# probabilists/zuko

Measured on AMD Instinct MI355X. Metric: log_prob samples/sec, NSF d=64 K=8 bins=8 batch=2^20, higher is better.
Workload: dtype f32; 1 GPU; NSF(features=64, context=0, transforms=8, bins=8, hidden=[256]*3) log_prob, batch=2^20 per GPU, x~N(0,1), seed-0 init; batch_per_gpu=1048576, global_batch=1048576, parallelism=batch-sharded x1, one RCCL all-reduce of the scalar NLL

## Files before the change

include/zuko_amd.h:

```cpp
#ifndef ZUKO_AMD_H
#define ZUKO_AMD_H

#include <stdint.h>

#ifdef __cplusplus
extern "C" {
#endif

#define ZK_DTYPE_F32 0
#define ZK_DTYPE_F64 1
#define ZK_DTYPE_BF16 2

#define ZK_ACT_NONE 0
#define ZK_ACT_RELU 1
#define ZK_ACT_ELU 2
#define ZK_ACT_TANH 3
#define ZK_ACT_SILU 4
#define ZK_ACT_GELU 5
#define ZK_ACT_SIGMOID 6
#define ZK_ACT_LEAKY 7


int zk_rqs_forward(int dtype, int64_t N, int64_t D, int K, double bound, double slope, const void* x,
                   const void* widths, int64_t w_sN, int64_t w_sD, const void* heights, int64_t h_sN, int64_t h_sD,
                   const void* derivs, int64_t d_sN, int64_t d_sD, void* y, void* ladj, int ladj_reduced,
                   int32_t* bin_out, void* stream);

int zk_rqs_inverse(int dtype, int64_t N, int64_t D, int K, double bound, double slope, const void* y,
                   const void* widths, int64_t w_sN, int64_t w_sD, const void* heights, int64_t h_sN, int64_t h_sD,
                   const void* derivs, int64_t d_sN, int64_t d_sD, void* x, int32_t* bin_out, void* stream);

int zk_rqs_from_knots(int dtype, int inverse, int64_t N, int64_t D, int K, const void* in, const void* horizontal,
                      const void* vertical, const void* slopes, int64_t k_sN, int64_t k_sD, void* out, void* ladj,
                      int32_t* bin_out, void* stream);

int zk_rqs_diag(int inverse, int64_t N, int64_t D, int K, double bound, double slope, const void* in, const void* widths,
                int64_t w_sN, int64_t w_sD, const void* heights, int64_t h_sN, int64_t h_sD, const void* derivs, int64_t d_sN,
                int64_t d_sD, void* out, void* ladj, int32_t* bin_out, float* knots_out, void* stream);

int zk_affine_forward(int dtype, int64_t N, int64_t D, double slope, const void* x, const void* shift, int64_t s_sN,
                      int64_t s_sD, const void* scale, int64_t c_sN, int64_t c_sD, void* y, void* ladj, int ladj_reduced,
                      void* stream);
int zk_affine_inverse(int dtype, int64_t N, int64_t D, double slope, const void* y, const void* shift, int64_t s_sN,
                      int64_t s_sD, const void* scale, int64_t c_sN, int64_t c_sD, void* x, void* stream);

int zk_sos_forward(int dtype, int64_t N, int64_t D, int P, int L1, double slope, const double* gl_nodes01,
                   const double* gl_weights01, const void* x, const void* a_coef, int64_t a_sN, int64_t a_sD,
                   const void* constant, int64_t c_sN, int64_t c_sD, void* y, void* ladj, int ladj_reduced, void* stream);
int zk_sos_inverse(int dtype, int64_t N, int64_t D, int P, int L1, double slope, const double* gl_nodes01,
                   const double* gl_weights01, int n_bisect, const void* y, const void* a_coef, int64_t a_sN,
                   int64_t a_sD, const void* constant, int64_t c_sN, int64_t c_sD, void* x, void* stream);

int zk_bernstein_forward(int dtype, int64_t N, int64_t D, int M, int bounded, double bound, double eps, const void* x,
                         const void* theta, int64_t t_sN, int64_t t_sD, void* y, void* ladj, int ladj_reduced, void* stream);
int zk_bernstein_inverse(int dtype, int64_t N, int64_t D, int M, int bounded, double bound, double eps, int n_bisect, const void* y,
                         const void* theta, int64_t t_sN, int64_t t_sD, void* x, void* stream);

int zk_linear(int dtype, int64_t N, int in_features, int out_features, const void* x, int64_t ldx, const void* weight,
              const uint8_t* mask, const void* bias, int act, void* y, int64_t ldy, void* stream);

int zk_linear_bf16(int64_t N, int in_features, int out_features, const void* x, int64_t ldx, const void* weight, const uint64_t* tile_live_mask,
                   const void* bias, int act, void* y, int64_t ldy, void* stream);

int zk_linear_bf16_rqs(int64_t N, int in_features, int panels, const void* h, int64_t ldh, const void* weight_panels, const uint64_t* tile_live_mask,
                       const void* bias_panels, int K, int features, double bound, double slope, const void* x, int64_t ldx, void* y, int64_t ldy,
                       float* partial, float* ladj, void* stream);
int zk_linear_bf16_rqs_lanes(int64_t N, int in_features, int panels, const void* h, int64_t ldh, const void* weight_panels,
                             const uint64_t* tile_live_mask, const void* bias_panels, int K, int features, double bound, double slope, const void* x,
                             int64_t ldx, void* y, int64_t ldy, float* partial, float* ladj, void* stream);

typedef struct zk_ar_args_v1 {
  uint32_t struct_size;
  uint32_t version;
  int32_t uni_kind;
  int32_t D;
  int32_t DIN;
  int32_t n_layers;
  int32_t n_groups;
  int32_t n_chunks;
  int32_t act;
  int32_t bias_floats;
  int32_t accumulate;
  int32_t rev;
  int32_t n_sched;
  int32_t g0;
  int32_t g1;
  int32_t reserved;
  int64_t N;
  int64_t ldx;
  int64_t ldy;
  int64_t ldo;
  int64_t ldphi;
  double bound;
  double slope;
  const void* x;
  void* y;
  void* ladj;
  const void* y_in;
  void* x_out;
  const void* wstream;
  const void* bias;
  const uint32_t* skip;
  const int32_t* featmap;
  int32_t* bin_out;
  float* knots_out;
  const int32_t* sched;
  const int32_t* olim;
  const void* launcher;
  void* h1;
  void* h2;
  void* h3;
  void* phi;
  void* gh1;
  void* gh2;
  void* gh3;
  int32_t phi_packed;
  int32_t pad_;
  const double* gl_nodes01;
  const double* gl_weights01;
  double eps;
  double wdescale0;
  double wdescale1;
  double wdescale2;
  double wdescale3;
  uint32_t* amax0;
  uint32_t* amax1;
  uint32_t* amax2;
  uint32_t* amax3;
} zk_ar_args_v1;

int zk_ar_forward(const zk_ar_args_v1* args, void* stream);
int zk_ar_forward_split(const zk_ar_args_v1* args, void* stream);
int zk_ar_forward_diag(const zk_ar_args_v1* args, void* stream);
int zk_ar_dgrad_chain(const zk_ar_args_v1* args, void* stream);
int zk_ar_dgrad_full(const zk_ar_args_v1* args, void* stream);
int zk_ar_backward_full(const zk_ar_args_v1* args, void* stream);
int zk_ar_inverse_sweep(const zk_ar_args_v1* args, void* stream);
int zk_ar_inverse_partial(const zk_ar_args_v1* args, void* stream);
typedef struct zk_coupling_args_v1 {
  uint32_t struct_size;
  uint32_t version;
  int32_t D;
  int32_t C;
  int32_t nit;
  int32_t n_groups;
  int32_t n_layers;
  int32_t n_chunks;
  int32_t act;
  int32_t bias_floats;
  int32_t accumulate;
  int32_t static_ok;
  int64_t N;
  int64_t ldx;
  int64_t ldc;
  int64_t ldy;
  double slope;
  const void* in;
  const void* ctx;
  void* out;
  void* ladj;
  const void* wstream;
  const void* bias;
  const int32_t* bias_off;
  const int32_t* amap;
  const int32_t* fmap;
  const int32_t* tiles;
  const int32_t* widths;
  double wdescale0;
  double wdescale1;
  double wdescale2;
  double wdescale3;
} zk_coupling_args_v1;
int zk_coupling_forward(const zk_coupling_args_v1* args, void* stream);
int zk_coupling_inverse(const zk_coupling_args_v1* args, void* stream);
typedef struct zk_ar_inc_args_v1 {
  uint32_t struct_size;
  uint32_t version;
  int32_t uni_kind;
  int32_t n_hidden;
  int32_t D;
  int32_t C;
  int32_t n_groups;
  int32_t n_chunks;
  int32_t act;
  int32_t bias_floats;
  int64_t N;
  int64_t ldy;
  int64_t ldc;
  int64_t ldx;
  double bound;
  double slope;
  const void* y;
  const void* ctx;
  void* x;
  void* ladj;
  const void* wstream;
  const void* bias;
  const int32_t* bias_off;
  const int32_t* featmap;
  const int32_t* prog;
  int32_t half;
  int32_t pad_;
  double wdescale1;
  double wdescale2;
  double wdescale3;
  const double* gl_nodes01;
  const double* gl_weights01;
  double eps;
  int32_t n_bisect;
  int32_t pad2_;
} zk_ar_inc_args_v1;
int zk_ar_inverse_incremental(const zk_ar_inc_args_v1* args, void* stream);
int zk_ar_inc_lds_bytes(int bias_floats, int nit);
int zk_ar_lds_bytes(int variant, int bias_floats);
int zk_ar_forward_static(const zk_ar_args_v1* args, void* stream);
int zk_ar_forward_train(const zk_ar_args_v1* args, void* stream);
int zk_gather_f32(const void* src, const uint8_t* mask, const int32_t* idx, int64_t n, void* dst, void* stream);
int zk_gather_split_bf16(const void* src, const uint8_t* mask, const int32_t* idx, int64_t n_blocks, void* dst, void* stream);
int zk_gather_split_f16(const void* src, const uint8_t* mask, const int32_t* idx, int64_t n_blocks, void* dst, double scale, void* stream);
typedef struct zk_gather_desc_v1 {
  uint32_t struct_size;
  int32_t split;
  int64_t count;
  const void* src;
  const uint8_t* mask;
  const int32_t* idx;
  void* dst;
} zk_gather_desc_v1;
int zk_gather_multi(int n, const zk_gather_desc_v1* descs, void* stream);

int zk_univariate_backward(int kind, int64_t N, int64_t D, int K, double bound, double slope, const void* x, const void* phi,
                           const void* gy, const void* gl, int gl_reduced, void* gx, void* gphi, void* stream);
int zk_sos_backward(int64_t N, int64_t D, int P, int L1, double slope, const double* gl_nodes01, const double* gl_weights01,
                    int has_const, const void* x, const void* params, const void* gy, const void* gl, int gl_reduced, void* gx,
                    void* gparams, void* stream);
int zk_bernstein_backward(int64_t N, int64_t D, int M, int bounded, double bound, double eps, const void* x, const void* theta, const void* gy,
                          const void* gl, int gl_reduced, void* gx, void* gtheta, void* stream);
int zk_inverse_seed(int64_t n, const void* gx, const void* ladj, void* gy, void* seed, void* stream);
int zk_diag_normal_backward(int64_t N, int64_t D, const void* z, const void* loc, const void* scale, const void* g, void* gz,
                            void* stream);
int zk_act_backward(int64_t n, const void* y, const void* gout, int act, void* gin, void* stream);

int zk_gemm_f32_skip(int64_t N, int in_features, int out_features, const void* x, int64_t ldx, const void* w, const uint64_t* kskip,
                     const void* bias, int act, const void* gate, int64_t ldg, int gate_act, void* y, int64_t ldy, void* stream);
int zk_wgrad_slices(int64_t N, int npairs);
int zk_wgrad_f32(int64_t N, int out_features, int in_features, const void* g, int64_t ldg, const void* h, int64_t ldh,
                 const int32_t* pairs, int npairs, float* partial, const uint8_t* mask, void* dw, int accumulate, const int32_t* rows,
                 const int32_t* cols, void* stream);
int zk_wgrad_bias_f32(int64_t N, int out_features, int in_features, const void* g, int64_t ldg, const void* h, int64_t ldh,
                      const int32_t* pairs, int npairs, float* partial, const uint8_t* mask, void* dw, int accumulate,
                      const uint8_t* cs_flag, float* cs_partial, void* db, const int32_t* rows, const int32_t* cols, void* stream);
typedef struct zk_wgrad_layer_v1 {
  uint32_t struct_size;
  int32_t out_features;
  int32_t in_features;
  int32_t npairs;
  int64_t ldg;
  int64_t ldh;
  const void* g;
  const void* h;
  const int32_t* pairs;
  void* partial;
  const uint8_t* mask;
  void* dw;
  const uint8_t* cs_flag;
  void* cs_partial;
  void* db;
  const int32_t* rows;
  const int32_t* cols;
  const uint32_t* g_amax;
  const uint32_t* h_amax;
} zk_wgrad_layer_v1;
int zk_wgrad_multi(int n_layers, const zk_wgrad_layer_v1* layers, int64_t N, void* stream);
int zk_colsum_slices(int64_t N);
int zk_colsum_f32(int64_t N, int C, const void* x, int64_t ld, float* workspace, void* out, int accumulate, void* stream);

#define ZK_AMAX_WORDS 2048
typedef struct zk_amax_desc_v1 {
  uint32_t struct_size;
  int32_t cols;
  int64_t rows;
// ... 34 lines not shown
```

zuko_amd/csrc/fused_ar.hip:

```cpp
#include "../../include/zuko_amd.h"
#include "zk_ar_common.h"
#include <type_traits>

#ifndef ZK_AR_TIMING
#define ZK_AR_TIMING 0
#endif

namespace zk {

template <int CH, int NR> struct RingT {
  static constexpr int kChunk = CH, kSlots = NR;
  float* lds;
  const float* stream;
  int n_chunks, pos, slot, load_chunk, load_slot, wave, lane, dbg;
  const int* sched;

  template <int I> __device__ __forceinline__ void dma(const float* g, float* l) {
    if constexpr (I < CH / AR_WAVES) {
#ifndef ZK_AR_NO_RING_DMA
      __builtin_amdgcn_global_load_lds((const __attribute__((address_space(1))) void*)g, (__attribute__((address_space(3))) void*)l, 16, I * AR_TF * 4, 0);
#endif
      dma<I + 1>(g, l);
    }
  }
// ... 227 lines not shown
        printf("wave %d: L1 %llu  L2 %llu  L3 %llu  (+bias/act each)  last layer + 16 epilogues %llu   total %llu cycles\n", wave, tstamp[1] - tstamp[0],
               tstamp[2] - tstamp[1], tstamp[3] - tstamp[2], tstamp[5] - tstamp[3], tstamp[5] - tstamp[0]);
    }
    if (!INVERSE) ar_ladj_store(a, lacc, n, live, q);
  }
  ring.drain();
}

__device__ __forceinline__ float gather_one(const float* __restrict__ src, const uint8_t* __restrict__ mask, int32_t k) { return (k >= 0 && (!mask || mask[k])) ? src[k] : 0.f; }

__device__ __forceinline__ void gather_split_lane(const float* __restrict__ src, const uint8_t* __restrict__ mask, const int32_t* __restrict__ idx, int64_t i, uint4* __restrict__ dst) {
  typedef __bf16 bf16x8 __attribute__((ext_vector_type(8)));
  const int4 k0 = *reinterpret_cast<const int4*>(idx + i * 8), k1 = *reinterpret_cast<const int4*>(idx + i * 8 + 4);
  const int k[8] = {k0.x, k0.y, k0.z, k0.w, k1.x, k1.y, k1.z, k1.w};
  bf16x8 h, m, l;
#pragma unroll
  for (int e = 0; e < 8; ++e) {
    const float v = gather_one(src, mask, k[e]);
    const __bf16 hh = (__bf16)v;
    const float r1 = v - (float)hh;
    const __bf16 mm = (__bf16)r1;
    h[e] = hh; m[e] = mm; l[e] = (__bf16)(r1 - (float)mm);
  }
  const int64_t b = i >> 6;
  const int lane = (int)(i & 63);
  dst[(b * 3 + 0) * 64 + lane] = __builtin_bit_cast(uint4, h);
  dst[(b * 3 + 1) * 64 + lane] = __builtin_bit_cast(uint4, m);
  dst[(b * 3 + 2) * 64 + lane] = __builtin_bit_cast(uint4, l);
}

__global__ __launch_bounds__(256) void gather_kernel(const float* __restrict__ src, const uint8_t* __restrict__ mask, const int32_t* __restrict__ idx, int64_t n, float* __restrict__ dst) {
  for (int64_t i = (int64_t)blockIdx.x * 256 + threadIdx.x; i < n; i += (int64_t)gridDim.x * 256) {
    dst[i] = gather_one(src, mask, idx[i]);
  }
}

__global__ __launch_bounds__(256) void gather_split_kernel(const float* __restrict__ src, const uint8_t* __restrict__ mask, const int32_t* __restrict__ idx, int64_t n_lanes,
                                                           uint4* __restrict__ dst) {
  for (int64_t i = (int64_t)blockIdx.x * 256 + threadIdx.x; i < n_lanes; i += (int64_t)gridDim.x * 256) gather_split_lane(src, mask, idx, i, dst);
}

__global__ __launch_bounds__(256) void gather_split_f16_kernel(const float* __restrict__ src, const uint8_t* __restrict__ mask, const int32_t* __restrict__ idx, int64_t n_lanes,
                                                               uint4* __restrict__ dst, float scale) {
  typedef _Float16 f16x8 __attribute__((ext_vector_type(8)));
  for (int64_t i = (int64_t)blockIdx.x * 256 + threadIdx.x; i < n_lanes; i += (int64_t)gridDim.x * 256) {
    const int4 k0 = *reinterpret_cast<const int4*>(idx + i * 8), k1 = *reinterpret_cast<const int4*>(idx + i * 8 + 4);
    const int k[8] = {k0.x, k0.y, k0.z, k0.w, k1.x, k1.y, k1.z, k1.w};
    f16x8 h, l;
#pragma unroll
    for (int e = 0; e < 8; ++e) {
      const float v = gather_one(src, mask, k[e]) * scale;
      const _Float16 hh = (_Float16)v;
      h[e] = hh; l[e] = (_Float16)(v - (float)hh);
    }
    const int64_t b = i >> 6;
    const int lane = (int)(i & 63);
    dst[(b * 2 + 0) * 64 + lane] = __builtin_bit_cast(uint4, h);
    dst[(b * 2 + 1) * 64 + lane] = __builtin_bit_cast(uint4, l);
  }
}

struct GatherMulti {
  int n;
  int start[9];
  struct One { const float* src; const uint8_t* mask; const int32_t* idx; int64_t count; void* dst; int split; } g[8];
};
__global__ __launch_bounds__(256) void gather_multi_kernel(GatherMulti m) {
  const int b = (int)blockIdx.x;
  GatherMulti::One g = m.g[0];
  int base = 0;
#pragma unroll
  for (int k = 1; k < 8; ++k)
    if (k < m.n && b >= m.start[k]) { g = m.g[k]; base = m.start[k]; }
  const int64_t i = (int64_t)(b - base) * 256 + threadIdx.x;
  if (!g.split) {
    if (i < g.count) reinterpret_cast<float*>(g.dst)[i] = gather_one(g.src, g.mask, g.idx[i]);
  } else if (i < g.count * 64) {
    gather_split_lane(g.src, g.mask, g.idx, i, reinterpret_cast<uint4*>(g.dst));
  }
}

}

using namespace zk;

extern "C" {

int zk_gather_f32(const void* src, const uint8_t* mask, const int32_t* idx, int64_t n, void* dst, void* stream) {
  if (n <= 0) return 0;
  int64_t nb = (n + 255) / 256;
  hipLaunchKernelGGL(gather_kernel, dim3((unsigned)(nb > 2048 ? 2048 : nb)), dim3(256), 0, (hipStream_t)stream, (const float*)src, mask, idx, n, (float*)dst);
  return ZK_LAUNCH_CHECK();
}

int zk_gather_split_bf16(const void* src, const uint8_t* mask, const int32_t* idx, int64_t n_blocks, void* dst, void* stream) {
  if (n_blocks <= 0) return 0;
  if (!src || !idx || !dst || ((uintptr_t)idx % 16) || ((uintptr_t)dst % 16)) return ZK_EINVAL;
  const int64_t n_lanes = n_blocks * 64, nb = (n_lanes + 255) / 256;
  hipLaunchKernelGGL(gather_split_kernel, dim3((unsigned)(nb > 2048 ? 2048 : nb)), dim3(256), 0, (hipStream_t)stream, (const float*)src, mask, idx, n_lanes, (uint4*)dst);
  return ZK_LAUNCH_CHECK();
}

int zk_gather_split_f16(const void* src, const uint8_t* mask, const int32_t* idx, int64_t n_blocks, void* dst, double scale, void* stream) {
  if (n_blocks <= 0) return 0;
  if (!src || !idx || !dst || ((uintptr_t)idx % 16) || ((uintptr_t)dst % 16) || !(scale > 0.0) || !(scale < 1e38)) return ZK_EINVAL;
  const int64_t n_lanes = n_blocks * 64, nb = (n_lanes + 255) / 256;
  hipLaunchKernelGGL(gather_split_f16_kernel, dim3((unsigned)(nb > 2048 ? 2048 : nb)), dim3(256), 0, (hipStream_t)stream, (const float*)src, mask, idx, n_lanes, (uint4*)dst, (float)scale);
  return ZK_LAUNCH_CHECK();
}

int zk_gather_multi(int n, const zk_gather_desc_v1* descs, void* stream) {
  if (n < 1 || n > 8 || !descs) return ZK_EINVAL;
  GatherMulti m{};
  m.n = n;
  int blocks = 0;
  for (int k = 0; k < n; ++k) {
    const zk_gather_desc_v1& d = descs[k];
    if (d.struct_size != sizeof(zk_gather_desc_v1) || d.count < 0 || (d.count > 0 && (!d.src || !d.idx || !d.dst))) return ZK_EINVAL;
    if (d.split && (((uintptr_t)d.idx % 16) || ((uintptr_t)d.dst % 16))) return ZK_EINVAL;
    m.g[k] = {(const float*)d.src, d.mask, d.idx, d.count, d.dst, d.split};
    m.start[k] = blocks;
    const int64_t threads = d.split ? d.count * 64 : d.count;
    if (threads > (int64_t)0x7fffffff) return ZK_EINVAL;
    blocks += (int)((threads + 255) / 256);
  }
  m.start[n] = blocks;
  if (blocks == 0) return 0;
  hipLaunchKernelGGL(gather_multi_kernel, dim3((unsigned)blocks), dim3(256), 0, (hipStream_t)stream, m);
  return ZK_LAUNCH_CHECK();
}

#ifndef AR_CH
#define AR_CH 24
#define AR_NR 3
#endif
typedef RingT<AR_CH, AR_NR> Ring24x3;
static int ar_lds_bytes(int bias_floats, bool xlds, int xs) { return ArLds::bytes(AR_CH * AR_NR * AR_TF, bias_floats, xlds ? AR_WAVES : 0, xs); }
int zk_ar_lds_bytes(int variant, int bias_floats) { return ar_lds_bytes(bias_floats, true, 260); }

struct ArPartial {
  const void* static_fn = nullptr;
  int rev = 0;
  float* act_out[3] = {nullptr, nullptr, nullptr};
  float* phi_out = nullptr;
  int64_t ldphi = 0;
  int phi_packed = 0;
  const double* gl_nodes01 = nullptr;
  const double* gl_weights01 = nullptr;
  double eps = 0.0;
  int32_t* bin_out = nullptr;
  float* knots_out = nullptr;
  double wdescale[4] = {0.0, 0.0, 0.0, 0.0};
  unsigned* amax[4] = {nullptr, nullptr, nullptr, nullptr};
  const int* sched = nullptr;
  int n_sched = 0;
  const int* olim = nullptr;
  int g0 = 0, g1 = -1;
};

static int ar_launch(const ArPartial& part, bool inverse, int uni_kind, int64_t N, int D, int DIN, const void* x, int64_t ldx, const void* yin, int64_t ldyin, void* y, int64_t ldy,
                     void* ladj, int accumulate, const void* wstream, const void* bias, int bias_floats, const uint32_t* skip, const int32_t* featmap,
                     int n_layers, int n_groups, int n_chunks, int act, double bound, double slope, int variant, void* stream) {
  if (N <= 0) return 0;
  if (n_groups * 8 > ArLds::FMAP_WORDS || n_groups > ArLds::SKIP_WORDS) return ZK_EINVAL;
  if (n_layers < 2 || DIN > (part.static_fn ? 512 : 256) || DIN < D || DIN % 4 || ldx % 4 || ((uintptr_t)x % 16) || n_chunks < 1) return ZK_EINVAL;
  ArArgs a{};
  a.N = N; a.D = D; a.DIN = DIN;
  a.x = (const float*)x; a.ldx = ldx;
  a.yin = (const float*)yin; a.ldyin = ldyin;
  a.y = (float*)y; a.ldy = ldy; a.ladj = (float*)ladj; a.accumulate = accumulate;
  a.stream = (const float*)wstream; a.bias = (const float*)bias; a.skip = skip; a.featmap = featmap;
  a.L = n_layers; a.NG = n_groups; a.n_chunks = n_chunks; a.act = act; a.bias_floats = bias_floats;
  a.bound = (float)bound; a.ls = (float)log(slope);
  a.lc = rqs_lean_const(bound, log(slope));
  a.n_tiles = (N + 127) / 128;
  a.g0 = 0; a.g1 = n_groups;
  for (int l = 0; l < 8; ++l) a.olim[l] = 3;
  if (part.sched) {
    if (part.n_sched < 1 || part.g0 < 0 || part.g1 > n_groups || part.g0 >= part.g1 || n_layers - 1 > 8) return ZK_EINVAL;
    a.sched = part.sched; a.n_sched = part.n_sched; a.g0 = part.g0; a.g1 = part.g1;
    for (int l = 0; l < n_layers - 1; ++l) a.olim[l] = part.olim[l];
  }
#if ZK_AR_TIMING
  a.dbg = (variant >> 8) & 0xff;
  if ((variant & 0xff) != 0) return ZK_EINVAL;
#else
  if (variant != 0) return ZK_EINVAL;
#endif
  if (part.static_fn) {
    if (inverse || part.sched || ((part.bin_out != nullptr) != (part.knots_out != nullptr))) return ZK_EINVAL;
    a.bin_out = part.bin_out; a.knots_out = part.knots_out;
    a.l1rev = part.rev;
    for (int l = 0; l < 3; ++l) a.act_out[l] = part.act_out[l];
    a.phi_out = part.phi_out; a.ldphi = part.ldphi; a.phi_packed = part.phi_packed;
    if (uni_kind == 5) {
      const bool conditioner_only = part.phi_out != nullptr && y == nullptr;
      if ((!part.gl_nodes01 || !part.gl_weights01) && !conditioner_only) return ZK_EINVAL;
      a.sos.bound = (float)bound; a.sos.slope = (float)slope; a.sos.P = 3; a.sos.L1 = 5;
      if (part.gl_nodes01 && part.gl_weights01)
        for (int i = 0; i < 5; ++i) { a.sos.node[i] = (float)part.gl_nodes01[i]; a.sos.weight[i] = (float)part.gl_weights01[i]; }
    }
    a.eps = (float)(part.eps > 0.0 ? part.eps : 1e-6);
    for (int l = 0; l < 4; ++l) a.wdescale[l] = (float)part.wdescale[l];
    for (int l = 0; l < 4; ++l) a.amax[l] = part.amax[l];
    return ((ars_launch_fn)part.static_fn)(&a, ARS_ABI, (int)sizeof(ArArgs), part.phi_out != nullptr, stream);
  }
  a.xs = ((D + 3) / 4) * 4 + 4;
  const bool vec_ok = (D % 4 == 0) && (ldy % 4 == 0) && ((uintptr_t)y % 16 == 0) && (!inverse || ((ldyin % 4 == 0) && ((uintptr_t)yin % 16 == 0)));
  a.xlds = vec_ok && ar_lds_bytes(bias_floats, true, a.xs) <= 160 * 1024;
  const int lds = ar_lds_bytes(bias_floats, a.xlds, a.xs);
  if (lds > 160 * 1024) return ZK_EINVAL;
  const void* fn = nullptr;
#define ZK_AR_PICK(UNI)                                                                                                                     \
  (inverse ? (a.xlds ? (const void*)ar_kernel<UNI, true, Ring24x3, true> : (const void*)ar_kernel<UNI, true, Ring24x3, false>)            \
           : (a.xlds ? (const void*)ar_kernel<UNI, false, Ring24x3, true> : (const void*)ar_kernel<UNI, false, Ring24x3, false>))
#define ZK_AR_PICK_X(UNI) (inverse ? (const void*)ar_kernel<UNI, true, Ring24x3, true> : (const void*)ar_kernel<UNI, false, Ring24x3, true>)
  if (uni_kind == 0) fn = ZK_AR_PICK(UniAffine);
  else if (uni_kind == 1) fn = ZK_AR_PICK(UniRqs8);
  else if (uni_kind >= 2 && uni_kind <= 4 && !a.xlds) return ZK_EINVAL;
  else if (uni_kind == 2) fn = ZK_AR_PICK_X(UniRqs4);
  else if (uni_kind == 3) fn = ZK_AR_PICK_X(UniRqs16);
  else if (uni_kind == 4) fn = ZK_AR_PICK_X(UniCircRqs8);
  else return ZK_EINVAL;
  if (part.bin_out || part.knots_out) {
    if (inverse || part.sched || !a.xlds || !part.bin_out || !part.knots_out) return ZK_EINVAL;
    a.bin_out = part.bin_out; a.knots_out = part.knots_out;
    if (uni_kind == 1) fn = (const void*)ar_kernel<UniRqs8, false, Ring24x3, true, true>;
    else if (uni_kind == 2) fn = (const void*)ar_kernel<UniRqs4, false, Ring24x3, true, true>;
    else if (uni_kind == 3) fn = (const void*)ar_kernel<UniRqs16, false, Ring24x3, true, true>;
    else return ZK_EINVAL;
  }
  return ar_launch_dyn_lds(fn, 256, 512, lds, a, stream);
}

#define AR_ARGS_OK(args) (ar_args_norm(args, &args##_norm_) ? ((args) = &args##_norm_, true) : false)

static int ar_launch_v1(const ArPartial& part, bool inverse, const zk_ar_args_v1& p, void* stream) {
  return ar_launch(part, inverse, p.uni_kind, p.N, p.D, p.DIN, p.x, p.ldx, inverse ? p.y_in : nullptr, inverse ? p.ldy : 0, inverse ? p.x_out : p.y, inverse ? p.ldo : p.ldy,
                   inverse ? nullptr : p.ladj, p.accumulate, p.wstream, p.bias, p.bias_floats, p.skip, p.featmap, p.n_layers, p.n_groups, p.n_chunks, p.act, p.bound, p.slope, 0,
                   stream);
}

int zk_ar_forward(const zk_ar_args_v1* args, void* stream) {
  zk_ar_args_v1 args_norm_;
  if (!AR_ARGS_OK(args)) return ZK_EINVAL;
  return ar_launch_v1(ArPartial{}, false, *args, stream);
}

int zk_ar_forward_diag(const zk_ar_args_v1* args, void* stream) {
  zk_ar_args_v1 args_norm_;
  if (!AR_ARGS_OK(args)) return ZK_EINVAL;
  ArPartial part;
  part.bin_out = args->bin_out; part.knots_out = args->knots_out;
  zk_ar_args_v1 p = *args;
  p.accumulate = 0;
  return ar_launch_v1(part, false, p, stream);
}

int zk_ar_forward_static(const zk_ar_args_v1* args, void* stream) {
  zk_ar_args_v1 args_norm_;
  if (!AR_ARGS_OK(args) || !args->launcher) return ZK_EINVAL;
  ArPartial part;
  part.static_fn = args->launcher; part.rev = args->rev;
  part.gl_nodes01 = args->gl_nodes01; part.gl_weights01 = args->gl_weights01; part.eps = args->eps;
  part.bin_out = args->bin_out; part.knots_out = args->knots_out;
  part.wdescale[0] = args->wdescale0; part.wdescale[1] = args->wdescale1; part.wdescale[2] = args->wdescale2; part.wdescale[3] = args->wdescale3;
  zk_ar_args_v1 p = *args;
  p.skip = nullptr;
  return ar_launch_v1(part, false, p, stream);
}

int zk_ar_forward_train(const zk_ar_args_v1* args, void* stream) {
  zk_ar_args_v1 args_norm_;
  if (!AR_ARGS_OK(args) || !args->launcher || !args->phi || !args->h1) return ZK_EINVAL;
  const int n_layers = args->n_layers;
  if (n_layers < 2 || n_layers > 4 || (n_layers > 2 && !args->h2) || (n_layers > 3 && !args->h3)) return ZK_EINVAL;
  if (((uintptr_t)args->h1 % 16) || ((uintptr_t)args->h2 % 16) || ((uintptr_t)args->h3 % 16)) return ZK_EINVAL;
  ArPartial part;
  part.static_fn = args->launcher; part.rev = args->rev;
  part.act_out[0] = (float*)args->h1; part.act_out[1] = (float*)args->h2; part.act_out[2] = (float*)args->h3; part.phi_out = (float*)args->phi; part.ldphi = args->ldphi;
  part.phi_packed = args->phi_packed;
  part.amax[0] = args->amax0; part.amax[1] = args->amax1; part.amax[2] = args->amax2; part.amax[3] = args->amax3;
  zk_ar_args_v1 p = *args;
  p.act = 1; p.skip = nullptr;
  if (!p.y) {
    p.ldy = 0; p.ladj = nullptr; p.accumulate = 0; p.bound = 1.0; p.slope = 1e-3;
  }
  return ar_launch_v1(part, false, p, stream);
}

typedef int (*ars_dgrad_fn)(const ArArgs* a, int abi, int args_bytes, void* stream);
static bool ar_chain_args_ok(const zk_ar_args_v1* args) {
  return args->launcher && args->x && args->y && args->wstream && args->n_layers >= 2 && args->n_layers <= 4 && args->N >= 0 && args->N <= 0x7fffffff;
}
static ArArgs ar_chain_args(const zk_ar_args_v1* args, int chain_layers, int gated) {
  const void* hs[3] = {args->h1, args->h2, args->h3};
  void* gs[3] = {args->gh1, args->gh2, args->gh3};
  ArArgs a{};
  a.x = (const float*)args->x; a.ldx = args->ldx; a.N = args->N; a.D = args->D; a.DIN = args->DIN; a.L = chain_layers; a.n_chunks = args->n_chunks;
  a.stream = (const float*)args->wstream;
  a.phi_out = (float*)args->y; a.ldphi = args->ldy;
  for (int c = 0; c < gated; ++c) {
    a.gate[c] = (const float*)hs[gated - 1 - c];
    a.act_out[c] = (float*)gs[gated - 1 - c];
  }
  return a;
}
static int ar_chain_launch(const zk_ar_args_v1* args, const ArArgs& a, void* stream) { return ((ars_dgrad_fn)args->launcher)(&a, ARS_ABI, (int)sizeof(ArArgs), stream); }

int zk_ar_dgrad_chain(const zk_ar_args_v1* args, void* stream) {
  zk_ar_args_v1 args_norm_;
  if (!AR_ARGS_OK(args) || !ar_chain_args_ok(args)) return ZK_EINVAL;
  if (args->N == 0) return 0;
  return ar_chain_launch(args, ar_chain_args(args, args->n_layers - 1, args->n_layers - 2), stream);
}

int zk_ar_dgrad_full(const zk_ar_args_v1* args, void* stream) {
  zk_ar_args_v1 args_norm_;
  if (!AR_ARGS_OK(args) || !ar_chain_args_ok(args)) return ZK_EINVAL;
  if (args->N == 0) return 0;
  ArArgs a = ar_chain_args(args, args->n_layers, args->n_layers - 1);
  a.accumulate = args->accumulate;
  return ar_chain_launch(args, a, stream);
}

int zk_ar_backward_full(const zk_ar_args_v1* args, void* stream) {
  zk_ar_args_v1 args_norm_;
  if (!AR_ARGS_OK(args) || !ar_chain_args_ok(args) || !args->phi || !args->x_out || !args->y_in || !args->ladj || !args->featmap) return ZK_EINVAL;
  if (args->uni_kind < 0 || args->uni_kind > 1 || args->DIN < args->D || args->D < 1) return ZK_EINVAL;
  if (args->N == 0) return 0;
  ArArgs a = ar_chain_args(args, args->n_layers, args->n_layers - 1);
  a.NG = args->n_groups; a.featmap = args->featmap; a.accumulate = args->accumulate;
  a.gy = (const float*)args->y_in; a.ldgy = args->ldo; a.gl = (const float*)args->ladj;
  a.phi_in = (const float*)args->phi; a.gphi_out = (float*)args->x_out; a.ldpin = args->ldphi; a.phi_packed = 1;
  a.bound = (float)args->bound; a.ls = (float)log(args->slope);
  a.amax[0] = args->amax0; a.amax[1] = args->amax1; a.amax[2] = args->amax2; a.amax[3] = args->amax3;
  return ar_chain_launch(args, a, stream);
}

int zk_ar_inverse_sweep(const zk_ar_args_v1* args, void* stream) {
  zk_ar_args_v1 args_norm_;
  if (!AR_ARGS_OK(args)) return ZK_EINVAL;
  return ar_launch_v1(ArPartial{}, true, *args, stream);
}

int zk_ar_inverse_partial(const zk_ar_args_v1* args, void* stream) {
  zk_ar_args_v1 args_norm_;
  if (!AR_ARGS_OK(args) || !args->sched || !args->olim) return ZK_EINVAL;
  ArPartial part;
  part.sched = args->sched; part.n_sched = args->n_sched; part.olim = args->olim; part.g0 = args->g0; part.g1 = args->g1;
  return ar_launch_v1(part, true, *args, stream);
}

}
```

zuko_amd/csrc/fused_ar_half_impl.h:

```cpp
#pragma once
#include "fused_ar_split_impl.h"

#ifndef ARH_LOOK
#define ARH_LOOK 1
#endif
#ifndef ARH_RELU_INT
#define ARH_RELU_INT 0
#endif
#ifndef ARH_EPI_PINNED
#define ARH_EPI_PINNED 1
#endif
#ifndef ARH_DESCALE_PK
#define ARH_DESCALE_PK 1
#endif
#ifndef ARH_PREFETCH
#define ARH_PREFETCH 1
#endif

namespace zk {

typedef _Float16 f16x8 __attribute__((ext_vector_type(8)));

struct ArhB {
  f16x8 h, l;
// ... 26 lines not shown
  for (int e = 0; e < 4; ++e) asm("v_fma_mixlo_f16 %0, %1, %2, %3" : "=v"(h[e]) : "v"(e < 2 ? lo[2 * e] : hi[2 * e - 4]), "v"(s), "s"(nz));
#pragma unroll
  for (int e = 0; e < 4; ++e) asm("v_fma_mixhi_f16 %0, %1, %2, %3" : "+v"(h[e]) : "v"(e < 2 ? lo[2 * e + 1] : hi[2 * e - 3]), "v"(s), "s"(nz));
#pragma unroll
  for (int e = 0; e < 4; ++e) asm("v_fma_mixlo_f16 %0, %1, %2, -%3 op_sel:[0,0,0] op_sel_hi:[0,0,1]" : "=v"(l[e]) : "v"(e < 2 ? lo[2 * e] : hi[2 * e - 4]), "v"(s), "v"(h[e]));
#pragma unroll
  for (int e = 0; e < 4; ++e) asm("v_fma_mixhi_f16 %0, %1, %2, -%3 op_sel:[0,0,1] op_sel_hi:[0,0,1]" : "+v"(l[e]) : "v"(e < 2 ? lo[2 * e + 1] : hi[2 * e - 3]), "v"(s), "v"(h[e]));
  b.h = __builtin_bit_cast(f16x8, h); b.l = __builtin_bit_cast(f16x8, l);
  return;
#endif
#pragma unroll
  for (int e = 0; e < 8; ++e) {
    const float v = (e < 4 ? lo[e] : hi[e - 4]) * s;
    const _Float16 h = (_Float16)v;
    const float r = v - (float)h;
    b.h[e] = h;
    b.l[e] = (_Float16)r;
  }
}

#define ARH_MFMA(A, B, C) C = __builtin_amdgcn_mfma_f32_16x16x32_f16(__builtin_bit_cast(f16x8, A), B, C, 0, 0, 0)
__device__ __forceinline__ void arh_block(const f32x4 (&a)[2], const ArhB& b, f32x4& c) {
  if (ARX_ABL == 2) {
    asm volatile("" ::"v"(a[0]), "v"(a[1]));
    return;
  }
  ARH_MFMA(a[1], b.h, c);
  ARH_MFMA(a[0], b.l, c);
  ARH_MFMA(a[0], b.h, c);
}

__device__ __forceinline__ void arh_touch(f32x4& v) { asm volatile("" : "+v"(v)); }
template <int N> __device__ __forceinline__ void arh_settle(f32x4& a0, f32x4& a1) { asm volatile("s_waitcnt lgkmcnt(%2)" : "+v"(a0), "+v"(a1) : "n"(N)); }
template <int N> __device__ __forceinline__ void arh_settle(f32x4& a0, f32x4& a1, f32x4& a2) { asm volatile("s_waitcnt lgkmcnt(%3)" : "+v"(a0), "+v"(a1), "+v"(a2) : "n"(N)); }

template <int WAVES, int CH, int NR> struct ArhRing : ArRingS<WAVES, CH, NR> {
  typedef ArRingS<WAVES, CH, NR> B;
  template <int XV> __device__ __forceinline__ void advance_x() {
    asm volatile("s_waitcnt vmcnt(%0) lgkmcnt(0)" ::"n"((NR - 2) * B::PER + XV) : "memory");
    if (ARX_ABL != 4) __builtin_amdgcn_s_barrier();
    asm volatile("" ::: "memory");
    this->issue();
    this->slot = (this->slot + 1 == NR) ? 0 : this->slot + 1;
    this->cur_off = this->lds_off + (unsigned)(this->slot * CH * AR_TF * 4 + this->lane * 16);
  }
  template <int S, int XV = 0> __device__ __forceinline__ f32x4 read() {
    if constexpr (XV != 0 && S % CH == 0) {
      advance_x<XV>();
      f32x4 v;
      if (ARX_ABL == 5) {
        asm volatile("v_mov_b32 %0, %1" : "=v"(v[0]) : "v"(this->cur_off));
        v[1] = v[2] = v[3] = v[0];
        return v;
      }
      asm volatile("ds_read_b128 %0, %1 offset:%2" : "=v"(v) : "v"(this->cur_off), "n"((S % CH) * AR_TF * 4));
      return v;
    } else {
      return B::template read<S>();
    }
  }
};

template <class S, int L, class Ring> __device__ __forceinline__ void arh_hidden(Ring& ring, const float* bias_q, const ArhB (&in)[S::TMAX / 2], f32x4 (&out)[S::TMAX], float d) {
  typedef ArxPat<S> P;
  constexpr int NB = S::NB[L], BASE = S::BASE[L], HTL = S::HT[L];
  ars_for<HTL>([&](auto t_) ARS_ALWAYS_INLINE {
    constexpr int t = t_;
    if constexpr (!P::tile_has_blocks(L, t)) out[t] = *reinterpret_cast<const f32x4*>(bias_q + t * 16);
  });
  if constexpr (NB > 0) {
    constexpr int LOOK = ARH_LOOK < NB ? ARH_LOOK : NB;
    f32x4 a[LOOK + 1][2];
    f32x4 bs;
    f32x4 acc;
    const unsigned bias_addr = arx_lds_addr(bias_q);
    ars_for<LOOK>([&](auto b_) ARS_ALWAYS_INLINE {
      constexpr int b = b_;
      ars_for<2>([&](auto p) ARS_ALWAYS_INLINE { a[b][p] = ring.template read<BASE + 2 * b + decltype(p)::value>(); });
    });
    ars_for<NB>([&](auto s_) ARS_ALWAYS_INLINE {
      constexpr int s = s_, ot = P::ot(L, s), ip = P::ip(L, s), cur = s % (LOOK + 1);
      constexpr bool first_of_tile = (s == 0 || P::ot(L, s - 1) != ot), last_of_tile = (s + 1 == NB || P::ot(L, s + 1) != ot);
      if constexpr (first_of_tile) acc = f32x4{0.f, 0.f, 0.f, 0.f};
      if constexpr (last_of_tile) bs = arx_lds_raw<ot * 64>(bias_addr);
      if constexpr (s + LOOK < NB) {
        constexpr int nx = (s + LOOK) % (LOOK + 1);
        ars_for<2>([&](auto p) ARS_ALWAYS_INLINE { a[nx][p] = ring.template read<BASE + 2 * (s + LOOK) + decltype(p)::value>(); });
      }
      constexpr int ahead = (s + LOOK < NB ? LOOK : NB - 1 - s);
      if constexpr (last_of_tile) arh_settle<(s + LOOK < NB ? 2 : 0)>(a[cur][0], a[cur][1], bs);
      else arh_settle<2 * ahead>(a[cur][0], a[cur][1]);
      if (ARX_FENCE) __builtin_amdgcn_sched_barrier(0);
      arh_block(a[cur], in[ip], acc);
      if (ARX_FENCE) __builtin_amdgcn_sched_barrier(0);
      if constexpr (last_of_tile) {
        if (ARH_DESCALE_PK) {
#pragma unroll
          for (int r = 0; r < 4; r += 2) {
            const arh_f32x2 o = __builtin_elementwise_fma(arh_f32x2{acc[r], acc[r + 1]}, arh_f32x2{d, d}, arh_f32x2{bs[r], bs[r + 1]});
            out[ot][r] = o[0]; out[ot][r + 1] = o[1];
          }
        } else {
#pragma unroll
          for (int r = 0; r < 4; ++r) out[ot][r] = __builtin_fmaf(acc[r], d, bs[r]);
        }
      }
    });
  }
}

template <class S, int L, class Ring> __device__ __forceinline__ void arh_hidden_stack(Ring& ring, const float* bias_lds, int q, ArhB (&in)[S::TMAX / 2], f32x4 (&out)[S::TMAX], const ArArgs& a,
                                                                                       float& inv_s, float& poison) {
  if constexpr (L < S::NH) {
    arh_hidden<S, L>(ring, bias_lds + L * S::BIAS_STRIDE + 4 * q, in, out, a.wdescale[L] * inv_s);
    constexpr int HTL = S::HT[L];
    float amax = 0.f;
    if constexpr (S::ACT == 1 && ARH_EPI_PINNED) {
#pragma unroll
      for (int t = 0; t < HTL; ++t)
#pragma unroll
        for (int r = 0; r < 4; r += 2) {
          asm("v_max_f32 %0, 0, %0" : "+v"(out[t][r]));
          asm("v_max_f32 %0, 0, %0" : "+v"(out[t][r + 1]));
          asm("v_max3_f32 %0, %0, %1, %2" : "+v"(amax) : "v"(out[t][r]), "v"(out[t][r + 1]));
        }
    } else if constexpr (S::ACT == 1) {
#pragma unroll
      for (int t = 0; t < HTL; ++t)
#pragma unroll
        for (int r = 0; r < 4; ++r) {
          if (ARH_RELU_INT) out[t][r] = __builtin_bit_cast(float, max(__builtin_bit_cast(int, out[t][r]), 0));
          else out[t][r] = out[t][r] < 0.f ? 0.f : out[t][r];
          amax = fmaxf(amax, out[t][r]);
        }
    } else {
      ar_activate<S::ACT, HTL>(out, out);
#pragma unroll
      for (int t = 0; t < HTL; ++t)
#pragma unroll
        for (int r = 0; r < 4; ++r) amax = fmaxf(amax, fabsf(out[t][r]));
    }
    float s;
    arh_scale(amax, s, inv_s);
    if constexpr (S::ACT == 1 && ARH_EPI_PINNED) {
      if (!(amax < ARH_AMAX_OVERFLOW)) poison = __builtin_nanf("");
    }
    const f32x4 zero = {0.f, 0.f, 0.f, 0.f};
#pragma unroll
    for (int p = 0; p < (HTL + 1) / 2; ++p) arh_split(out[2 * p], 2 * p + 1 < HTL ? out[2 * p + 1] : zero, s, in[p]);
    arh_hidden_stack<S, L + 1, Ring>(ring, bias_lds, q, in, out, a, inv_s, poison);
  }
}

template <class S, typename Uni, bool DIAG = false> __global__ __launch_bounds__(64 * S::WAVES, S::OCC) void arh_kernel(ArArgs a) {
  typedef ArhRing<S::WAVES, S::CH, S::NR> Ring;
  static_assert(S::WAVES == 8 && S::NR == 3 && S::TMAX <= 16 && S::TMAX % 2 == 0 && S::OCC == 2, "two-part split kernels: widths <= 256, two wavefronts per SIMD");
  constexpr int NT = Uni::NT, FPL = Uni::FPL, TOTAL = Uni::TOTAL, WAVES = S::WAVES;
  constexpr int NG = S::NG;
  constexpr int NSTEP = S::GOFF[NG];
  constexpr bool XLDS = S::XLDS;
  const ArLane ln;
  const int tid = ln.tid, lane = ln.lane, wave = ln.wave, j = ln.j, q = ln.q;

  Ring ring;
  ring.lds = ars_lds; ring.stream = a.stream; ring.n_chunks = a.n_chunks; ring.wave = wave; ring.lane = lane;
  ring.load_chunk = 0; ring.load_slot = 0;
#pragma unroll
  for (int i = 0; i < S::NR - 1; ++i) ring.issue();
  ring.slot = S::NR - 1;
  ring.lds_off = (unsigned)(size_t)((__attribute__((address_space(3))) float*)ars_lds);
  ring.cur_off = ring.lds_off;

  auto x_request = [&](int64_t tile, f32x4 (&xv)[S::NIT]) ARS_ALWAYS_INLINE {
    const int64_t n = tile * (16 * WAVES) + wave * 16 + j;
    const float* row = a.x + (n < a.N ? n : a.N - 1) * a.ldx;
#pragma unroll
    for (int it = 0; it < S::NIT; ++it) {
      const int col = it * 16 + 4 * q;
      xv[it] = *reinterpret_cast<const f32x4*>(row + ((it + 1) * 16 <= S::DIN || col < S::DIN ? col : S::DIN - 4));
    }
  };
  f32x4 xnext[S::NIT];
  if (ARH_PREFETCH) x_request(blockIdx.x, xnext);

  float* const bias_lds = ars_lds + S::NR * S::CH * AR_TF;
  int* const fmap_lds = ArLds::fmap(bias_lds, a.bias_floats);
  float* const xr = ArLds::row(fmap_lds, wave, j, a.xs);
  ArLds::stage<64 * WAVES>(a, tid, bias_lds, fmap_lds, NG * 4 * FPL);
  const float* bias_last = bias_lds + S::NH * S::BIAS_STRIDE;
  const unsigned bias_last_addr = arx_lds_addr(bias_last + 4 * q);
  const ArFids<NG, FPL, (NG * FPL <= 32)> fids(fmap_lds, q);

  for (int64_t tile = blockIdx.x; tile < a.n_tiles; tile += gridDim.x) {
    const int64_t n = tile * (16 * WAVES) + wave * 16 + j;
    const bool live = n < a.N;
    const int64_t nc = live ? n : a.N - 1;
    const float* xrow = a.x + nc * a.ldx;

    ArhB in[S::TMAX / 2];
    f32x4 out[S::TMAX];
    float poison;
    float inv_s;
    {
      f32x4 xin[S::NIT + 1];
#pragma unroll
      for (int it = 0; it < S::NIT; ++it) {
        f32x4 v = {0.f, 0.f, 0.f, 0.f};
        if (ARH_PREFETCH) {
          if ((it + 1) * 16 <= S::DIN || it * 16 + 4 * q < S::DIN) v = xnext[it];
        } else {
          if ((it + 1) * 16 <= S::DIN || it * 16 + 4 * q < S::DIN) v = *reinterpret_cast<const f32x4*>(xrow + it * 16 + 4 * q);
        }
        xin[it] = v;
      }
      xin[S::NIT] = f32x4{0.f, 0.f, 0.f, 0.f};
      poison = ar_poison_of<S::NIT>(xin);
      float amax = 0.f;
#pragma unroll
      for (int it = 0; it < S::NIT; ++it)
#pragma unroll
        for (int r = 0; r < 4; ++r) amax = fmaxf(amax, fabsf(xin[it][r]));
      if constexpr (XLDS) ar_rows_in<S::D>(xr, q, xin);
      float s;
      arh_scale(amax, s, inv_s);
      if constexpr (S::ACT == 1 && ARH_EPI_PINNED) {
        if (!(amax < ARH_AMAX_OVERFLOW)) poison = __builtin_nanf("");
      }
#pragma unroll
      for (int p = 0; p < (S::NIT + 1) / 2; ++p) arh_split(xin[2 * p], xin[2 * p + 1], s, in[p]);
    }

    float ladj_in = 0.f;
    if (ARH_PREFETCH && a.ladj && a.accumulate && live && q == 0) ladj_in = a.ladj[n];

    arh_hidden_stack<S, 0, Ring>(ring, bias_lds, q, in, out, a, inv_s, poison);

    const float dl = a.wdescale[S::NH] * inv_s;
    float lacc = 0.f;
    constexpr int NBL = NSTEP * NT;
    constexpr int LOOKL = ARH_LOOK < NBL ? ARH_LOOK : NBL;
    f32x4 w[LOOKL + 1][2];
    constexpr int XPOS = ARH_PREFETCH ? (S::LAST_BASE + S::CH - 1) / S::CH * S::CH : -1;
    if (ARH_PREFETCH) {
      asm volatile("" ::: "memory");
      x_request(tile + gridDim.x < a.n_tiles ? tile + gridDim.x : tile, xnext);
      asm volatile("" ::: "memory");
    }
#define ARH_READ_LAST(POS) ring.template read<(POS), ((POS) == XPOS ? S::NIT : 0)>()
    ars_for<LOOKL>([&](auto b_) ARS_ALWAYS_INLINE {
      constexpr int b = b_;
      ars_for<2>([&](auto p) ARS_ALWAYS_INLINE { w[b][p] = ARH_READ_LAST(S::LAST_BASE + 2 * b + decltype(p)::value); });
    });
    ars_for<NG>([&](auto g_) ARS_ALWAYS_INLINE {
      constexpr int g = g_, ST0 = S::GOFF[g], GN = S::GOFF[g + 1] - S::GOFF[g];
      int fid[FPL];
      float xin[FPL];
      fids.template fetch<XLDS>(g, xr, xrow, fid, xin);
      f32x4 acc[NT], bs[NT];
      if constexpr (GN == 0) {
        const float* bg = bias_last + (g * NT) * 16 + 4 * q;
        ars_for<NT>([&](auto t) ARS_ALWAYS_INLINE { bs[t] = *reinterpret_cast<const f32x4*>(bg + t * 16); });
      }
      ars_for<NT>([&](auto t) ARS_ALWAYS_INLINE { acc[t] = f32x4{0.f, 0.f, 0.f, 0.f}; });
      ars_for<GN>([&](auto i_) ARS_ALWAYS_INLINE {
        constexpr int st = ST0 + decltype(i_)::value, ip = S::G_IP[st];
        ars_for<NT>([&](auto t_) ARS_ALWAYS_INLINE {
          constexpr int t = t_, blk = st * NT + t, cur = blk % (LOOKL + 1);
          constexpr bool last_of_group = (decltype(i_)::value == GN - 1 && t == NT - 1);
          if constexpr (last_of_group) {
            ars_for<NT>([&](auto u) ARS_ALWAYS_INLINE { bs[u] = arx_lds_raw<(g * NT + decltype(u)::value) * 64>(bias_last_addr); });
          }
          if constexpr (blk + LOOKL < NBL) {
            constexpr int nx = (blk + LOOKL) % (LOOKL + 1);
            ars_for<2>([&](auto p) ARS_ALWAYS_INLINE { w[nx][p] = ARH_READ_LAST(S::LAST_BASE + 2 * (blk + LOOKL) + decltype(p)::value); });
          }
          constexpr int ahead = (blk + LOOKL < NBL ? LOOKL : NBL - 1 - blk);
          if constexpr (last_of_group) arh_settle<(blk + LOOKL < NBL ? 2 : 0)>(w[cur][0], w[cur][1]);
          else arh_settle<2 * ahead>(w[cur][0], w[cur][1]);
          if constexpr (last_of_group) {
#pragma unroll
            for (int u = 0; u < NT; ++u) arh_touch(bs[u]);
          }
          if (ARX_FENCE) __builtin_amdgcn_sched_barrier(0);
          arh_block(w[cur], in[ip], acc[t]);
          if (ARX_FENCE) __builtin_amdgcn_sched_barrier(0);
        });
      });
      float p[4 * NT];
      ars_for<NT>([&](auto t) ARS_ALWAYS_INLINE {
#pragma unroll
        for (int r = 0; r < 4; ++r) {
          p[4 * t + r] = __builtin_fmaf(acc[t][r], dl, bs[t][r]);
          if (ARH_POISON_ONE) asm("" : "+v"(p[4 * t + r]));
        }
      });
      ar_uni_epilogue<Uni, DIAG, XLDS>(p, a, fid, xin, poison, xr, n, live, S::D, lacc);
    });
#undef ARH_READ_LAST
    if (ARH_PREFETCH) ar_ladj_store<true>(a, lacc, n, live, q, ladj_in);
    if constexpr (XLDS) ar_rows_out<S::D>(xr, q, a.y + n * a.ldy, live);
    if (!ARH_PREFETCH) ar_ladj_store(a, lacc, n, live, q);
  }
  asm volatile("s_waitcnt vmcnt(0)" ::: "memory");
}

template <class S, typename Uni> static int arh_launch(const ArArgs* in, int abi, int args_bytes, int train, void* stream) {
  if (abi != ARS_ABI || args_bytes != (int)sizeof(ArArgs)) return ZK_EINVAL;
  ArArgs a = *in;
  if (train || a.D != S::D || a.DIN != S::DIN || a.L != S::NH + 1 || a.act != S::ACT || a.sched || a.NG != S::NG || a.n_chunks != S::NCHUNK || a.l1rev) return ZK_EINVAL;
  for (int l = 0; l <= S::NH; ++l)
    if (!(a.wdescale[l] > 0.f) || !(a.wdescale[l] < __builtin_inff())) return ZK_EINVAL;
  a.n_tiles = (a.N + 16 * S::WAVES - 1) / (16 * S::WAVES);
  a.xs = ((S::D + 3) / 4) * 4 + 4;
  const bool vec_ok = (S::D % 4 == 0) && (a.ldy % 4 == 0) && ((uintptr_t)a.y % 16 == 0);
  if (S::XLDS != 0 && !vec_ok) return ZK_EINVAL;
  a.xlds = S::XLDS;
  const int lds = ArLds::bytes(S::NR * S::CH * AR_TF, a.bias_floats, S::XLDS ? S::WAVES : 0, a.xs);
  if (lds > 160 * 1024) return ZK_EINVAL;
  const void* fn = nullptr;
  if ((a.bin_out != nullptr) != (a.knots_out != nullptr)) return ZK_EINVAL;
  if (a.bin_out) {
    if constexpr (Uni::NKNOT > 1) fn = (const void*)arh_kernel<S, Uni, true>;
  } else {
    fn = (const void*)arh_kernel<S, Uni, false>;
  }
  if (!fn) return ZK_EINVAL;
  return ar_launch_dyn_lds(fn, 256, 64 * S::WAVES, lds, a, stream);
}

}
```

zuko_amd/csrc/fused_ar_split_impl.h:

```cpp
#pragma once
#include "fused_ar_static_impl.h"
#include "zk_half.h"
#include "zk_univariate_bwd.h"

#ifndef ARX_LOOK
#define ARX_LOOK 1
#endif
#ifndef ARX_FENCE
#define ARX_FENCE 1
#endif

namespace zk {

typedef __bf16 bf16x8 __attribute__((ext_vector_type(8)));

struct ArxB {
  bf16x8 h, m, l;
};

__device__ __forceinline__ void arx_split(const f32x4& lo, const f32x4& hi, ArxB& b) {
  if (ARX_ABL == 6) {
    b.h = __builtin_bit_cast(bf16x8, lo); b.m = __builtin_bit_cast(bf16x8, hi); b.l = b.h;
    return;
  }
#pragma unroll
  for (int e = 0; e < 8; ++e) {
    const float v = e < 4 ? lo[e] : hi[e - 4];
    const __bf16 h = (__bf16)v;
    const float r1 = v - (float)h;
    const __bf16 m = (__bf16)r1;
    const float r2 = r1 - (float)m;
    b.h[e] = h;
    b.m[e] = m;
    b.l[e] = (__bf16)r2;
  }
}

#define ARX_MFMA(A, B, C) C = __builtin_amdgcn_mfma_f32_16x16x32_bf16(__builtin_bit_cast(bf16x8, A), B, C, 0, 0, 0)
__device__ __forceinline__ void arx_block(const f32x4 (&a)[3], const ArxB& b, f32x4& c) {
  if (ARX_ABL == 2) {
    asm volatile("" ::"v"(a[0]), "v"(a[1]), "v"(a[2]));
    return;
  }
  ARX_MFMA(a[2], b.h, c);
  ARX_MFMA(a[0], b.l, c);
  ARX_MFMA(a[1], b.m, c);
  ARX_MFMA(a[1], b.h, c);
  ARX_MFMA(a[0], b.m, c);
  ARX_MFMA(a[0], b.h, c);
}

template <int OFF> __device__ __forceinline__ f32x4 arx_lds_raw(unsigned addr) {
  f32x4 v;
  asm volatile("ds_read_b128 %0, %1 offset:%2" : "=v"(v) : "v"(addr), "n"(OFF));
  return v;
}
__device__ __forceinline__ unsigned arx_lds_addr(const float* p) { return (unsigned)(size_t)((const __attribute__((address_space(3))) float*)p); }

template <bool ON> __device__ __forceinline__ void arx_mfma_guard(f32x4& acc) {
  if constexpr (ON) asm volatile("s_nop 15" : "+v"(acc));
}
template <class S, class = void> struct ArxOneWave : std::false_type {};
template <class S> struct ArxOneWave<S, std::void_t<decltype(S::OCC)>> : std::integral_constant<bool, S::OCC == 1> {};

template <class S> struct ArxPat {
  static constexpr int ot(int l, int s) { return S::B_OT[S::BOFF[l] + s]; }
  static constexpr int ip(int l, int s) { return S::B_IP[S::BOFF[l] + s]; }
  static constexpr bool tile_has_blocks(int l, int t) {
    for (int s = 0; s < S::NB[l]; ++s)
      if (ot(l, s) == t) return true;
    return false;
  }
};

template <class S, int L, class Ring> __device__ __forceinline__ void arx_hidden(Ring& ring, const float* bias_q, const ArxB (&in)[S::TMAX / 2], f32x4 (&out)[S::TMAX]) {
  typedef ArxPat<S> P;
  constexpr int NB = S::NB[L], BASE = S::BASE[L], HTL = S::HT[L];
  ars_for<HTL>([&](auto t_) ARS_ALWAYS_INLINE {
    constexpr int t = t_;
    if constexpr (!P::tile_has_blocks(L, t)) out[t] = *reinterpret_cast<const f32x4*>(bias_q + t * 16);
  });
  if constexpr (NB > 0) {
    constexpr int LOOK = ARX_LOOK < NB ? ARX_LOOK : NB;
    f32x4 a[LOOK + 1][3];
    const unsigned bias_addr = arx_lds_addr(bias_q);
    ars_for<LOOK>([&](auto b_) ARS_ALWAYS_INLINE {
      constexpr int b = b_;
      ars_for<3>([&](auto p) ARS_ALWAYS_INLINE { a[b][p] = ring.template read<BASE + 3 * b + decltype(p)::value>(); });
    });
    ars_for<NB>([&](auto s_) ARS_ALWAYS_INLINE {
      constexpr int s = s_, ot = P::ot(L, s), ip = P::ip(L, s), cur = s % (LOOK + 1);
      constexpr bool first_of_tile = (s == 0 || P::ot(L, s - 1) != ot);
      if constexpr (first_of_tile) out[ot] = arx_lds_raw<ot * 64>(bias_addr);
      if constexpr (s + LOOK < NB) {
        constexpr int nx = (s + LOOK) % (LOOK + 1);
        ars_for<3>([&](auto p) ARS_ALWAYS_INLINE { a[nx][p] = ring.template read<BASE + 3 * (s + LOOK) + decltype(p)::value>(); });
      }
      constexpr int ahead = (s + LOOK < NB ? LOOK : NB - 1 - s);
      if constexpr (first_of_tile) ars_settle<(s + LOOK < NB ? 3 : 0)>(a[cur][0], a[cur][1], a[cur][2], out[ot]);
      else ars_settle<3 * ahead>(a[cur][0], a[cur][1], a[cur][2]);
      if (ARX_FENCE) __builtin_amdgcn_sched_barrier(0);
      arx_block(a[cur], in[ip], out[ot]);
      if (ARX_FENCE) __builtin_amdgcn_sched_barrier(0);
    });
    arx_mfma_guard<ArxOneWave<S>::value>(out[P::ot(L, NB - 1)]);
  }
}

__device__ __forceinline__ void arx_amax_flush(const ArArgs& a, const float (&mx)[4], unsigned which, int lane) {
#pragma unroll
  for (int l = 0; l < 4; ++l)
    if (a.amax[l]) {
      const float m = gh_wave_max(mx[l]);
      if (lane == 0) gh_amax_put(a.amax[l], which, m);
    }
}
template <class S, int L, class Ring, bool TRAIN> __device__ __forceinline__ void arx_hidden_stack(Ring& ring, const float* bias_lds, int q, ArxB (&in)[S::TMAX / 2], f32x4 (&out)[S::TMAX],
                                                                                                 const ArArgs& a, int64_t n, bool live, float (&mx)[4]) {
  if constexpr (L < S::NH) {
    arx_hidden<S, L>(ring, bias_lds + L * S::BIAS_STRIDE + 4 * q, in, out);
    constexpr int HTL = S::HT[L];
    ar_activate<S::ACT, HTL>(out, out);
    if constexpr (TRAIN) {
      if (live) {
#pragma unroll
        for (int t = 0; t < HTL; ++t) *reinterpret_cast<f32x4*>(a.act_out[L < 3 ? L : 2] + n * (HTL * 16) + t * 16 + 4 * q) = out[t];
        if (a.amax[L < 3 ? L : 2]) {
#pragma unroll
          for (int t = 0; t < HTL; ++t)
#pragma unroll
            for (int r = 0; r < 4; ++r) mx[L < 3 ? L : 2] = fmaxf(mx[L < 3 ? L : 2], fabsf(out[t][r]));
        }
      }
    }
    const f32x4 zero = {0.f, 0.f, 0.f, 0.f};
#pragma unroll
    for (int p = 0; p < (HTL + 1) / 2; ++p) arx_split(out[2 * p], 2 * p + 1 < HTL ? out[2 * p + 1] : zero, in[p]);
    arx_hidden_stack<S, L + 1, Ring, TRAIN>(ring, bias_lds, q, in, out, a, n, live, mx);
  }
}

template <class S, typename Uni, bool TRAIN, bool DIAG = false> __global__ __launch_bounds__(64 * S::WAVES, S::OCC) void arx_kernel(ArArgs a) {
  typedef ArRingS<S::WAVES, S::CH, S::NR> Ring;
  static_assert((S::WAVES == 8 || S::WAVES == 4) && (S::NR == 2 || S::NR == 3) && (S::TMAX <= 16 || (S::TMAX <= 32 && S::OCC == 1 && S::WAVES == 4)) && S::TMAX % 2 == 0,
                "operand-split kernels: widths <= 256 with two wavefronts per SIMD, <= 512 with one");
  constexpr int NT = Uni::NT, FPL = Uni::FPL, TOTAL = Uni::TOTAL, WAVES = S::WAVES;
  constexpr int NG = S::NG;
  constexpr int NSTEP = S::GOFF[NG];
  constexpr bool XLDS = S::XLDS;
  const ArLane ln;
  const int tid = ln.tid, lane = ln.lane, wave = ln.wave, j = ln.j, q = ln.q;

  Ring ring;
  ring.start(ars_lds, a.stream, a.n_chunks, wave, lane);
  float* const bias_lds = ars_lds + S::NR * S::CH * AR_TF;
  int* const fmap_lds = ArLds::fmap(bias_lds, a.bias_floats);
  float* const xr = ArLds::row(fmap_lds, wave, j, a.xs);
  ArLds::stage<64 * WAVES>(a, tid, bias_lds, fmap_lds, NG * 4 * FPL);
  const float* bias_last = bias_lds + S::NH * S::BIAS_STRIDE;
  const unsigned bias_last_addr = arx_lds_addr(bias_last + 4 * q);
  const ArFids<NG, FPL, (NG * FPL <= 32 && !TRAIN)> fids(fmap_lds, q);

  const bool uni_on = !TRAIN || a.y != nullptr;
  float mx[4] = {0.f, 0.f, 0.f, 0.f};
  for (int64_t tile = blockIdx.x; tile < a.n_tiles; tile += gridDim.x) {
    const int64_t n = tile * (16 * WAVES) + wave * 16 + j;
    const bool live = n < a.N;
    const int64_t nc = live ? n : a.N - 1;
    const float* xrow = a.x + nc * a.ldx;

    ArxB in[S::TMAX / 2];
    f32x4 out[S::TMAX];
    float poison;
    {
      f32x4 xin[S::NIT + 1];
#pragma unroll
      for (int it = 0; it < S::NIT; ++it) {
        f32x4 v = {0.f, 0.f, 0.f, 0.f};
        if ((it + 1) * 16 <= S::DIN || it * 16 + 4 * q < S::DIN) v = *reinterpret_cast<const f32x4*>(xrow + it * 16 + 4 * q);
        xin[it] = v;
        if constexpr (TRAIN) {
          if (live && a.amax[3]) {
#pragma unroll
            for (int r = 0; r < 4; ++r) mx[3] = fmaxf(mx[3], fabsf(v[r]));
          }
        }
      }
      xin[S::NIT] = f32x4{0.f, 0.f, 0.f, 0.f};
      poison = 0.f;
      int bad = 0;
#pragma unroll
      for (int it = 0; it < S::NIT; ++it)
#pragma unroll
        for (int r = 0; r < 4; ++r) bad |= !(fabsf(xin[it][r]) < __builtin_inff());
      bad |= __shfl_xor(bad, 16, 64);
      bad |= __shfl_xor(bad, 32, 64);
      if (bad) poison = __builtin_nanf("");
      if constexpr (XLDS) ar_rows_in<S::D>(xr, q, xin);
#pragma unroll
      for (int p = 0; p < (S::NIT + 1) / 2; ++p) arx_split(xin[2 * p], xin[2 * p + 1], in[p]);
    }

    arx_hidden_stack<S, 0, Ring, TRAIN>(ring, bias_lds, q, in, out, a, n, live, mx);

    float lacc = 0.f;
    constexpr int NBL = NSTEP * NT;
    constexpr int LOOKL = ARX_LOOK < NBL ? ARX_LOOK : NBL;
    f32x4 w[LOOKL + 1][3];
    ars_for<LOOKL>([&](auto b_) ARS_ALWAYS_INLINE {
      constexpr int b = b_;
      ars_for<3>([&](auto p) ARS_ALWAYS_INLINE { w[b][p] = ring.template read<S::LAST_BASE + 3 * b + decltype(p)::value>(); });
    });
    ars_for<NG>([&](auto g_) ARS_ALWAYS_INLINE {
      constexpr int g = g_, ST0 = S::GOFF[g], GN = S::GOFF[g + 1] - S::GOFF[g];
      int fid[FPL];
      float xin[FPL];
      fids.template fetch<XLDS>(g, xr, xrow, fid, xin);
      f32x4 acc[NT];
      if constexpr (GN > 0) {
        ars_for<NT>([&](auto t) ARS_ALWAYS_INLINE { acc[t] = arx_lds_raw<(g * NT + decltype(t)::value) * 64>(bias_last_addr); });
      } else {
        const float* bg = bias_last + (g * NT) * 16 + 4 * q;
        ars_for<NT>([&](auto t) ARS_ALWAYS_INLINE { acc[t] = *reinterpret_cast<const f32x4*>(bg + t * 16); });
      }
      ars_for<GN>([&](auto i_) ARS_ALWAYS_INLINE {
        constexpr int st = ST0 + decltype(i_)::value, ip = S::G_IP[st];
        ars_for<NT>([&](auto t_) ARS_ALWAYS_INLINE {
          constexpr int t = t_, blk = st * NT + t, cur = blk % (LOOKL + 1);
          if constexpr (blk + LOOKL < NBL) {
            constexpr int nx = (blk + LOOKL) % (LOOKL + 1);
            ars_for<3>([&](auto p) ARS_ALWAYS_INLINE { w[nx][p] = ring.template read<S::LAST_BASE + 3 * (blk + LOOKL) + decltype(p)::value>(); });
          }
          constexpr int ahead = (blk + LOOKL < NBL ? LOOKL : NBL - 1 - blk);
          if constexpr (decltype(i_)::value == 0 && t == 0) ars_settle<(blk + LOOKL < NBL ? 3 : 0)>(w[cur][0], w[cur][1], w[cur][2], acc[t]);
          else if constexpr (decltype(i_)::value == 0) ars_settle<3 * ahead>(w[cur][0], w[cur][1], w[cur][2], acc[t]);
          else ars_settle<3 * ahead>(w[cur][0], w[cur][1], w[cur][2]);
          if (ARX_FENCE) __builtin_amdgcn_sched_barrier(0);
          arx_block(w[cur], in[ip], acc[t]);
          if (ARX_FENCE) __builtin_amdgcn_sched_barrier(0);
        });
      });
      float p[4 * NT];
      if constexpr (GN > 0) arx_mfma_guard<ArxOneWave<S>::value>(acc[NT - 1]);
      ars_for<NT>([&](auto t) ARS_ALWAYS_INLINE {
#pragma unroll
        for (int r = 0; r < 4; ++r) p[4 * t + r] = acc[t][r];
      });
      if constexpr (TRAIN) {
        if (a.phi_packed) {
          if (live) {
            float* dst = a.phi_out + n * a.ldphi + (g * NT) * 16 + 4 * q;
            ars_for<NT>([&](auto t) ARS_ALWAYS_INLINE {
              *reinterpret_cast<f32x4*>(dst + decltype(t)::value * 16) = f32x4{p[4 * t] + poison, p[4 * t + 1] + poison, p[4 * t + 2] + poison, p[4 * t + 3] + poison};
            });
          }
        } else {
#pragma unroll
          for (int fi = 0; fi < FPL; ++fi) {
            const int f = fid[fi];
            if (f >= 0 && live) {
              float* dst = a.phi_out + n * a.ldphi + f * TOTAL;
#pragma unroll
              for (int i = 0; i < TOTAL; ++i) dst[i] = p[fi * TOTAL + i] + poison;
            }
          }
        }
      }
      if (uni_on) ar_uni_epilogue<Uni, DIAG, XLDS>(p, a, fid, xin, poison, xr, n, live, S::D, lacc);
    });
    if constexpr (XLDS) ar_rows_out<S::D>(xr, q, a.y + n * a.ldy, live && uni_on);
    if (uni_on) ar_ladj_store(a, lacc, n, live, q);
  }
  if constexpr (TRAIN) arx_amax_flush(a, mx, blockIdx.x * WAVES + wave, lane);
  asm volatile("s_waitcnt vmcnt(0)" ::: "memory");
}

#ifndef ARXB_AHEAD
#define ARXB_AHEAD 1
#endif
#ifndef ARXB_ABL
#define ARXB_ABL 0
#endif
template <class S> struct ArxdPat {
  static constexpr int pair_index(int s) {
    int n = 0;
    for (int i = 1; i <= s; ++i) n += S::B_IP[i] != S::B_IP[i - 1];
    return n;
  }
};

template <class S, class Ring> __device__ __forceinline__ void arxd_first(Ring& ring, const float* grow_q, int q, f32x4 (&out)[S::TMAX]) {
  typedef ArxdPat<S> P;
  constexpr int NB = S::NB[0], BASE = S::BASE[0], HTL = S::HT[0], NP = S::NP0, DEPTH = NP < 6 ? NP : 6;
  const f32x4 zero = {0.f, 0.f, 0.f, 0.f};
#pragma unroll
  for (int t = 0; t < HTL; ++t) out[t] = zero;
  f32x4 pf[DEPTH][2];
  auto fetch = [&](auto j_) ARS_ALWAYS_INLINE {
    constexpr int j = decltype(j_)::value, ip = S::P0[j];
    ars_for<2>([&](auto h_) ARS_ALWAYS_INLINE {
      constexpr int it = 2 * ip + decltype(h_)::value;
      f32x4 v = zero;
      if constexpr ((it + 1) * 16 <= S::DIN0) v = *reinterpret_cast<const f32x4*>(grow_q + it * 16);
      else if constexpr (it * 16 < S::DIN0) {
        if (it * 16 + 4 * q < S::DIN0) v = *reinterpret_cast<const f32x4*>(grow_q + it * 16);
      }
      pf[j % DEPTH][h_] = v;
    });
  };
  ars_for<DEPTH>([&](auto j_) ARS_ALWAYS_INLINE { fetch(j_); });
  ArxB b;
  f32x4 a[2][3];
  ars_for<3>([&](auto p) ARS_ALWAYS_INLINE { a[0][p] = ring.template read<BASE + decltype(p)::value>(); });
  ars_for<NB>([&](auto s_) ARS_ALWAYS_INLINE {
    constexpr int s = s_, ot = S::B_OT[s], j = P::pair_index(s);
    if constexpr (s == 0 || S::B_IP[s - 1] != S::B_IP[s]) {
      arx_split(pf[j % DEPTH][0], pf[j % DEPTH][1], b);
      if constexpr (j + DEPTH < NP) fetch(std::integral_constant<int, j + DEPTH>{});
    }
    if constexpr (s + 1 < NB) {
      ars_for<3>([&](auto p) ARS_ALWAYS_INLINE { a[(s + 1) & 1][p] = ring.template read<BASE + 3 * (s + 1) + decltype(p)::value>(); });
      ars_settle<3>(a[s & 1][0], a[s & 1][1], a[s & 1][2]);
    } else {
      ars_settle<0>(a[s & 1][0], a[s & 1][1], a[s & 1][2]);
    }
    __builtin_amdgcn_sched_barrier(0);
    arx_block(a[s & 1], b, out[ot]);
    __builtin_amdgcn_sched_barrier(0);
  });
}

template <class S, int L, class Ring> __device__ __forceinline__ void arxd_stack(Ring& ring, const float* zero_q, int q, ArxB (&in)[S::TMAX / 2], f32x4 (&out)[S::TMAX], const ArArgs& a,
                                                                                 int64_t n, int64_t nc, bool live, float (&mx)[4], const float* xadd_q = nullptr) {
  if constexpr (L < S::NH) {
    if constexpr (L > 0) arx_hidden<S, L>(ring, zero_q, in, out);
    constexpr int HTL = S::HT[L];
    if constexpr (L + 1 < S::NH) {
      const float* grow = a.gate[L] + nc * (HTL * 16) + 4 * q;
#pragma unroll
      for (int t = 0; t < HTL; ++t) {
        const f32x4 h = (ARXB_ABL == 6 || ARXB_ABL == 7 || ARXB_ABL == 8) ? f32x4{1.f, -1.f, 1.f, 1.f} : *reinterpret_cast<const f32x4*>(grow + t * 16);
#pragma unroll
        for (int r = 0; r < 4; ++r) out[t][r] = out[t][r] * (h[r] > 0.f ? 1.f : 0.f);
      }
      if (live && ARXB_ABL != 5 && ARXB_ABL != 7 && ARXB_ABL != 8) {
#pragma unroll
        for (int t = 0; t < HTL; ++t) *reinterpret_cast<f32x4*>(a.act_out[L] + n * (HTL * 16) + t * 16 + 4 * q) = out[t];
        if (a.amax[L < 3 ? L : 2]) {
#pragma unroll
          for (int t = 0; t < HTL; ++t)
#pragma unroll
            for (int r = 0; r < 4; ++r) mx[L < 3 ? L : 2] = fmaxf(mx[L < 3 ? L : 2], fabsf(out[t][r]));
        }
      }
      const f32x4 zero = {0.f, 0.f, 0.f, 0.f};
#pragma unroll
      for (int p = 0; p < (HTL + 1) / 2; ++p) arx_split(out[2 * p], 2 * p + 1 < HTL ? out[2 * p + 1] : zero, in[p]);
      arxd_stack<S, L + 1, Ring>(ring, zero_q, q, in, out, a, n, nc, live, mx, xadd_q);
    } else if (live) {
#pragma unroll
      for (int t = 0; t < HTL; ++t)
        if ((t + 1) * 16 <= S::DOUT || t * 16 + 4 * q < S::DOUT) {
          f32x4* dst = reinterpret_cast<f32x4*>(a.phi_out + n * a.ldphi + t * 16 + 4 * q);
          if (xadd_q) out[t] += *reinterpret_cast<const f32x4*>(xadd_q + t * 16);
          *dst = a.accumulate ? *dst + out[t] : out[t];
        }
    }
  }
}

template <class S> __global__ __launch_bounds__(512, 2) void arxd_kernel(ArArgs a) {
  typedef ArRingS<8, S::CH> Ring;
  static_assert(S::NH >= 2 && S::NH <= 4 && S::TMAX <= 16 && S::TMAX % 2 == 0 && S::WAVES == 8, "dgrad chain: the last layer + up to three gated layers, widths <= 256");
  const ArLane ln;
  const int lane = ln.lane, wave = ln.wave, j = ln.j, q = ln.q;
  Ring ring;
  ring.start(ars_lds, a.stream, a.n_chunks, wave, lane);
  float* zero_lds = ArChainLds<S::CH, S::TMAX>::template zero_fill<512>(ars_lds, ln.tid);
  __syncthreads();
  float mx[4] = {0.f, 0.f, 0.f, 0.f};
  for (int64_t tile = blockIdx.x; tile < a.n_tiles; tile += gridDim.x) {
    const int64_t n = tile * 128 + wave * 16 + j;
    const bool live = n < a.N;
    const int64_t nc = live ? n : a.N - 1;
    ArxB in[S::TMAX / 2];
    f32x4 out[S::TMAX];
    arxd_first<S>(ring, a.x + nc * a.ldx + 4 * q, q, out);
    arxd_stack<S, 0, Ring>(ring, zero_lds + 4 * q, q, in, out, a, n, nc, live, mx);
  }
  arx_amax_flush(a, mx, blockIdx.x * 8 + wave, lane);
  asm volatile("s_waitcnt vmcnt(0)" ::: "memory");
}

template <typename Uni, typename A> __device__ __forceinline__ void arxb_adjoint(const float* p, const A& a, float x, float gy, float gl, float& gx, float* g) {
  if constexpr (Uni::TOTAL == 2) affine_backward_element(p, x, gy, gl, a.ls, gx, g);
  else rqs_backward_element<(Uni::TOTAL + 1) / 3>(p, x, gy, gl, a.bound, a.ls, gx, g);
}

template <class S, typename Uni, class Ring>
__device__ __forceinline__ void arxb_first(Ring& ring, const ArArgs& a, const int* fmap_lds, float* xr, int q, int64_t n, int64_t nc, bool live, f32x4 (&out)[S::TMAX], float (&mx)[4]) {
  constexpr int NT = Uni::NT, FPL = Uni::FPL, TOTAL = Uni::TOTAL;
  constexpr int SG = (NT % 2) ? 2 : 1;
  constexpr int NSTEP = S::NG / SG, PPS = SG * NT / 2, NF = SG * FPL;
  constexpr int NB = S::NB[0], BASE = S::BASE[0], HTL = S::HT[0];
  static_assert(S::NG % SG == 0 && FPL * TOTAL <= 4 * NT, "packed order: whole pairs per step");
  const f32x4 zero = {0.f, 0.f, 0.f, 0.f};
#pragma unroll
  for (int t = 0; t < HTL; ++t) out[t] = zero;
  const float glv = a.gl[nc];
  const float* phirow = a.phi_in + nc * a.ldpin + 4 * q;
  float* gphirow = a.gphi_out + n * a.ldpin + 4 * q;
  const float* xrow = a.x + nc * a.ldx;
  const float* gyrow = a.gy + nc * a.ldgy;
  f32x4 ph4[ARXB_AHEAD][SG * NT];
  float xv[ARXB_AHEAD][NF], gyv[ARXB_AHEAD][NF];
  int fid[ARXB_AHEAD][NF];
  auto fetch = [&](auto s_) ARS_ALWAYS_INLINE {
    constexpr int s = decltype(s_)::value, bf = s % ARXB_AHEAD;
#pragma unroll
    for (int t = 0; t < SG * NT; ++t)
      ph4[bf][t] = (ARXB_ABL == 2 || ARXB_ABL == 3 || ARXB_ABL == 8) ? f32x4{0.01f, 0.02f, 0.03f, 0.04f} : *reinterpret_cast<const f32x4*>(phirow + (s * SG * NT + t) * 16);
#pragma unroll
    for (int i = 0; i < NF; ++i) {
      const int f = fmap_lds[((s * SG + i / FPL) * 4 + q) * FPL + i % FPL];
      const int fc = f < 0 ? 0 : f;
      fid[bf][i] = f;
      xv[bf][i] = xrow[fc];
      gyv[bf][i] = gyrow[fc];
    }
  };
  ars_for<(ARXB_AHEAD < NSTEP ? ARXB_AHEAD : NSTEP)>([&](auto s_) ARS_ALWAYS_INLINE { fetch(s_); });
  f32x4 w[2][3];
  if constexpr (NB > 0) {
    ars_for<3>([&](auto p) ARS_ALWAYS_INLINE { w[0][p] = ring.template read<BASE + decltype(p)::value>(); });
  }
  ars_for<NSTEP>([&](auto s_) ARS_ALWAYS_INLINE {
    constexpr int s = s_, bf = s % ARXB_AHEAD;
    float gq[SG * NT * 4];
#pragma unroll
    for (int i = 0; i < SG * NT * 4; ++i) gq[i] = 0.f;
#pragma unroll
    for (int i = 0; i < NF; ++i) {
      const int f = fid[bf][i];
      float ph[TOTAL], g[TOTAL], gxv;
#pragma unroll
      for (int k = 0; k < TOTAL; ++k) ph[k] = ph4[bf][(i / FPL) * NT + ((i % FPL) * TOTAL + k) / 4][((i % FPL) * TOTAL + k) % 4];
      if (ARXB_ABL == 4) {
        gxv = xv[bf][i] + gyv[bf][i];
#pragma unroll
        for (int k = 0; k < TOTAL; ++k) g[k] = ph[k] + glv;
      } else
      arxb_adjoint<Uni>(ph, a, xv[bf][i], gyv[bf][i], glv, gxv, g);
      if (f >= 0) xr[f] = gxv;
#pragma unroll
      for (int k = 0; k < TOTAL; ++k) gq[(i / FPL) * NT * 4 + (i % FPL) * TOTAL + k] = f >= 0 ? g[k] : 0.f;
    }
    if constexpr (s + ARXB_AHEAD < NSTEP) fetch(std::integral_constant<int, s + ARXB_AHEAD>{});
    if (live && ARXB_ABL != 1 && ARXB_ABL != 3 && ARXB_ABL != 8) {
#pragma unroll
      for (int t = 0; t < SG * NT; ++t) *reinterpret_cast<f32x4*>(gphirow + (s * SG * NT + t) * 16) = f32x4{gq[4 * t], gq[4 * t + 1], gq[4 * t + 2], gq[4 * t + 3]};
      if (a.amax[3]) {
#pragma unroll
        for (int t = 0; t < 4 * SG * NT; ++t) mx[3] = fmaxf(mx[3], fabsf(gq[t]));
      }
    }
    ars_for<PPS>([&](auto pl_) ARS_ALWAYS_INLINE {
      constexpr int pl = pl_, pp = s * PPS + pl, B0 = S::PB[pp], B1 = S::PB[pp + 1];
      if constexpr (B1 > B0) {
        ArxB b;
        arx_split(f32x4{gq[8 * pl], gq[8 * pl + 1], gq[8 * pl + 2], gq[8 * pl + 3]}, f32x4{gq[8 * pl + 4], gq[8 * pl + 5], gq[8 * pl + 6], gq[8 * pl + 7]}, b);
        ars_for<B1 - B0>([&](auto i_) ARS_ALWAYS_INLINE {
          constexpr int blk = B0 + decltype(i_)::value, ot = S::B_OT[blk];
          if constexpr (blk + 1 < NB) {
            ars_for<3>([&](auto p) ARS_ALWAYS_INLINE { w[(blk + 1) & 1][p] = ring.template read<BASE + 3 * (blk + 1) + decltype(p)::value>(); });
            ars_settle<3>(w[blk & 1][0], w[blk & 1][1], w[blk & 1][2]);
          } else {
            ars_settle<0>(w[blk & 1][0], w[blk & 1][1], w[blk & 1][2]);
          }
          __builtin_amdgcn_sched_barrier(0);
          arx_block(w[blk & 1], b, out[ot]);
          __builtin_amdgcn_sched_barrier(0);
        });
      }
    });
  });
}

template <class S, typename Uni> using ArxbLds = ArChainLds<S::CH, S::TMAX, ((S::NG * 4 * Uni::FPL + 3) / 4) * 4>;

template <class S, typename Uni> __global__ __launch_bounds__(512, 2) void arxb_kernel(ArArgs a) {
  typedef ArRingS<8, S::CH> Ring;
  static_assert(S::NH >= 2 && S::NH <= 4 && S::TMAX <= 16 && S::TMAX % 2 == 0 && S::WAVES == 8, "dgrad chain: the last layer + up to three gated layers, widths <= 256");
  typedef ArxbLds<S, Uni> Lds;
  const ArLane ln;
  const int tid = ln.tid, lane = ln.lane, wave = ln.wave, j = ln.j, q = ln.q;
  Ring ring;
  ring.start(ars_lds, a.stream, a.n_chunks, wave, lane);
  int* fmap_lds = Lds::fmap(ars_lds);
  float* xr = Lds::rows(ars_lds) + (wave * 16 + j) * a.xs;
  float* zero_lds = Lds::template zero_fill<512>(ars_lds, tid);
  for (int i = tid; i < S::NG * 4 * Uni::FPL; i += 512) fmap_lds[i] = a.featmap[i];
  __syncthreads();
  float mx[4] = {0.f, 0.f, 0.f, 0.f};
  for (int64_t tile = blockIdx.x; tile < a.n_tiles; tile += gridDim.x) {
    const int64_t n = tile * 128 + wave * 16 + j;
    const bool live = n < a.N;
    const int64_t nc = live ? n : a.N - 1;
    ArxB in[S::TMAX / 2];
    f32x4 out[S::TMAX];
    if (a.D < S::DOUT) {
#pragma unroll 1
      for (int i = a.D + q; i < a.xs - 4; i += 4) xr[i] = 0.f;
    }
    arxb_first<S, Uni>(ring, a, fmap_lds, xr, q, n, nc, live, out, mx);
    asm volatile("" ::: "memory");
    __builtin_amdgcn_wave_barrier();
    arxd_stack<S, 0, Ring>(ring, zero_lds + 4 * q, q, in, out, a, n, nc, live, mx, xr + 4 * q);
    asm volatile("" ::: "memory");
    __builtin_amdgcn_wave_barrier();
  }
  arx_amax_flush(a, mx, blockIdx.x * 8 + wave, lane);
  asm volatile("s_waitcnt vmcnt(0)" ::: "memory");
}

template <class S, typename Uni> static int arxb_launch(const ArArgs* in, int abi, int args_bytes, void* stream) {
  if (abi != ARS_ABI || args_bytes != (int)sizeof(ArArgs)) return ZK_EINVAL;
  ArArgs a = *in;
  if (a.DIN != S::DOUT || a.D < 1 || a.D > S::DOUT || a.D > S::NG * 4 * Uni::FPL || a.L != S::NH || a.NG != S::NG || a.n_chunks != S::NCHUNK || !a.x || !a.phi_out || !a.phi_in || !a.gphi_out || !a.gy || !a.gl || !a.featmap ||
      a.ldx % 4 || a.ldphi % 4 || a.ldpin < (int64_t)S::NG * Uni::NT * 16 || ((uintptr_t)a.x % 16) || ((uintptr_t)a.phi_out % 16))
    return ZK_EINVAL;
  for (int l = 0; l + 1 < S::NH; ++l)
    if (!a.gate[l] || !a.act_out[l] || ((uintptr_t)a.gate[l] % 16) || ((uintptr_t)a.act_out[l] % 16)) return ZK_EINVAL;
  a.n_tiles = (a.N + 127) / 128;
  a.xs = ((S::DOUT + 3) / 4) * 4 + 4;
  const int lds = ArxbLds<S, Uni>::bytes(8 * 16 * a.xs);
  if (lds > 160 * 1024 || a.ldpin % 4 || ((uintptr_t)a.phi_in % 16) || ((uintptr_t)a.gphi_out % 16)) return ZK_EINVAL;
  return ar_launch_dyn_lds((const void*)arxb_kernel<S, Uni>, 256, 512, lds, a, stream);
}

template <class S> static int arxd_launch(const ArArgs* in, int abi, int args_bytes, void* stream) {
  if (abi != ARS_ABI || args_bytes != (int)sizeof(ArArgs)) return ZK_EINVAL;
  ArArgs a = *in;
  if (a.DIN != S::DIN0 || a.D != S::DOUT || a.L != S::NH || a.n_chunks != S::NCHUNK || !a.x || !a.phi_out || a.ldx % 4 || a.ldphi % 4 || ((uintptr_t)a.x % 16) ||
      ((uintptr_t)a.phi_out % 16))
    return ZK_EINVAL;
  for (int l = 0; l + 1 < S::NH; ++l)
    if (!a.gate[l] || !a.act_out[l] || ((uintptr_t)a.gate[l] % 16) || ((uintptr_t)a.act_out[l] % 16)) return ZK_EINVAL;
  a.n_tiles = (a.N + 127) / 128;
  return ar_launch_dyn_lds((const void*)arxd_kernel<S>, 256, 512, ArChainLds<S::CH, S::TMAX>::bytes(0), a, stream);
}

template <class S, typename Uni> static int arx_launch(const ArArgs* in, int abi, int args_bytes, int train, void* stream) {
  if (abi != ARS_ABI || args_bytes != (int)sizeof(ArArgs)) return ZK_EINVAL;
  ArArgs a = *in;
  if (a.D != S::D || a.DIN != S::DIN || a.L != S::NH + 1 || a.act != S::ACT || a.sched || a.NG != S::NG || a.n_chunks != S::NCHUNK || a.l1rev) return ZK_EINVAL;
  if (train && (!S::TRAIN_OK || !a.phi_out || (a.phi_packed && (a.ldphi % 4 || a.ldphi < (int64_t)S::NG * Uni::NT * 16 || ((uintptr_t)a.phi_out % 16))))) return ZK_EINVAL;
  a.n_tiles = (a.N + 16 * S::WAVES - 1) / (16 * S::WAVES);
  a.xs = ((S::D + 3) / 4) * 4 + 4;
  const bool vec_ok = (S::D % 4 == 0) && ((train && !a.y) || ((a.ldy % 4 == 0) && ((uintptr_t)a.y % 16 == 0)));
  if (S::XLDS != 0 && !vec_ok) return ZK_EINVAL;
  a.xlds = S::XLDS;
  const int lds = ArLds::bytes(S::NR * S::CH * AR_TF, a.bias_floats, S::XLDS ? S::WAVES : 0, a.xs);
  if (lds > 160 * 1024) return ZK_EINVAL;
  const void* fn = nullptr;
  if ((a.bin_out != nullptr) != (a.knots_out != nullptr) || (a.bin_out && train)) return ZK_EINVAL;
  if (train) {
    if constexpr (S::TRAIN_OK) fn = (const void*)arx_kernel<S, Uni, true>;
  } else if (a.bin_out) {
    if constexpr (Uni::NKNOT > 1) fn = (const void*)arx_kernel<S, Uni, false, true>;
  } else {
    fn = (const void*)arx_kernel<S, Uni, false>;
  }
  if (!fn) return ZK_EINVAL;
  constexpr int MAXG = (S::WAVES == 4 && S::OCC == 2) ? 512 : 256;
  return ar_launch_dyn_lds(fn, MAXG, 64 * S::WAVES, lds, a, stream);
}

}
```

zuko_amd/csrc/fused_ar_static_impl.h:

```cpp
#pragma once
#include "zk_ar_common.h"
#include <type_traits>
#include <utility>

namespace zk {

#define ARS_CH 24
#define ARS_NR 3
#define ARS_ALWAYS_INLINE __attribute__((always_inline))

template <class F, int... I> __device__ __forceinline__ void ars_for_impl(F&& f, std::integer_sequence<int, I...>) { (f(std::integral_constant<int, I>{}), ...); }
template <int N, class F> __device__ __forceinline__ void ars_for(F&& f) {
  if constexpr (N > 0) ars_for_impl(f, std::make_integer_sequence<int, N>{});
}

__host__ __device__ constexpr int ars_popc(unsigned m) { return (int)((m & 1u) + ((m >> 1) & 1u) + ((m >> 2) & 1u) + ((m >> 3) & 1u)); }

template <class S> struct ArsPat {
  static constexpr int otg(int l, int s) { return S::S_OTG[S::SOFF[l] + s]; }
  static constexpr int it(int l, int s) { return S::S_IT[S::SOFF[l] + s]; }
  static constexpr int alt(int l, int s) { return S::S_ALT[S::SOFF[l] + s]; }
  static constexpr unsigned mask(int l, int s) { return S::S_MASK[S::SOFF[l] + s]; }
  static constexpr bool first_of_group(int l, int s) { return s == 0 || otg(l, s - 1) != otg(l, s); }
  static constexpr bool group_has_steps(int l, int g) {
// ... 188 lines not shown
  if constexpr (FID_REGS) {
#pragma unroll
    for (int i = 0; i < NG; ++i)
#pragma unroll
      for (int fi = 0; fi < FPL; ++fi) fids[i * FPL + fi] = fmap_lds[(i * 4 + q) * FPL + fi];
  }

  for (int64_t tile = blockIdx.x; tile < a.n_tiles; tile += gridDim.x) {
    const int64_t n = tile * (16 * WAVES) + wave * 16 + j;
    const bool live = n < a.N;
    const int64_t nc = live ? n : a.N - 1;
    const float* xrow = a.x + nc * a.ldx;

    f32x4 in[S::TMAX], out[S::TMAX];
#pragma unroll
    for (int it = 0; it < S::NIT; ++it) {
      f32x4 v = {0.f, 0.f, 0.f, 0.f};
      if ((it + 1) * 16 <= S::DIN || it * 16 + 4 * q < S::DIN) v = *reinterpret_cast<const f32x4*>(xrow + it * 16 + 4 * q);
      in[it] = v;
    }
    const float poison = ar_poison_of<S::NIT>(in);
    if constexpr (XLDS) ar_rows_in<S::D>(xr, q, in);

    ars_hidden_stack<S, 0, Ring, TRAIN>(ring, bias_lds, q, in, out, rev, a, n, live);

    float lacc = 0.f;
    f32x4 w[2][NT];
    if constexpr (NSTEP > 0) {
      ars_for<NT>([&](auto t) ARS_ALWAYS_INLINE { w[0][t] = ring.template read<S::LAST_BASE + decltype(t)::value>(); });
    }
    ars_for<NG>([&](auto g_) ARS_ALWAYS_INLINE {
      constexpr int g = g_, ST0 = S::GOFF[g], GN = S::GOFF[g + 1] - S::GOFF[g];
      int fid[FPL];
      float xin[FPL];
#pragma unroll
      for (int fi = 0; fi < FPL; ++fi) {
        if constexpr (FID_REGS) fid[fi] = fids[g * FPL + fi];
        else fid[fi] = fmap_lds[(g * 4 + q) * FPL + fi];
        const int fc = fid[fi] < 0 ? 0 : fid[fi];
        if constexpr (XLDS) xin[fi] = xr[fc];
        else xin[fi] = xrow[fc];
      }
      f32x4 acc[NT];
      {
        const float* bg = bias_last + (g * NT) * 16 + 4 * q;
        ars_for<NT>([&](auto t) ARS_ALWAYS_INLINE { acc[t] = *reinterpret_cast<const f32x4*>(bg + t * 16); });
      }
      ars_for<GN>([&](auto i_) ARS_ALWAYS_INLINE {
        constexpr int st = ST0 + decltype(i_)::value, it = S::G_IT[st];
        if constexpr (st + 1 < NSTEP) {
          ars_for<NT>([&](auto t) ARS_ALWAYS_INLINE { w[(st + 1) & 1][t] = ring.template read<S::LAST_BASE + (st + 1) * NT + decltype(t)::value>(); });
          ars_settle_tiles<NT, NT>(w[st & 1]);
        } else {
          ars_settle_tiles<0, NT>(w[st & 1]);
        }
        __builtin_amdgcn_sched_barrier(0);
        ars_for<4>([&](auto r) ARS_ALWAYS_INLINE {
          ars_for<NT>([&](auto t) ARS_ALWAYS_INLINE { acc[t] = __builtin_amdgcn_mfma_f32_16x16x4f32(w[st & 1][t][(int)r], in[it][(int)r], acc[t], 0, 0, 0); });
        });
        __builtin_amdgcn_sched_barrier(0);
      });
      float p[4 * NT];
      ars_for<NT>([&](auto t) ARS_ALWAYS_INLINE {
#pragma unroll
        for (int r = 0; r < 4; ++r) p[4 * t + r] = acc[t][r];
      });
      if constexpr (TRAIN) {
#pragma unroll
        for (int fi = 0; fi < FPL; ++fi) {
          const int f = fid[fi];
          if (f >= 0 && live) {
            float* dst = a.phi_out + n * a.ldphi + f * TOTAL;
#pragma unroll
            for (int i = 0; i < TOTAL; ++i) dst[i] = p[fi * TOTAL + i] + poison;
          }
        }
      } else {
        ar_uni_epilogue<Uni, false, XLDS, false>(p, a, fid, xin, poison, xr, n, live, S::D, lacc);
      }
    });
    if constexpr (XLDS && !TRAIN) ar_rows_out<S::D>(xr, q, a.y + n * a.ldy, live);
    if constexpr (!TRAIN) ar_ladj_store(a, lacc, n, live, q);
  }
  asm volatile("s_waitcnt vmcnt(0)" ::: "memory");
}

template <class S, int L, class Ring> __device__ __forceinline__ void ars_dgrad_stack(Ring& ring, const float* zero_q, int q, f32x4 (&in)[S::TMAX], f32x4 (&out)[S::TMAX], const ArArgs& a,
                                                                                      int64_t n, int64_t nc, bool live) {
  if constexpr (L < S::NH) {
    ars_hidden<S, L>(ring, zero_q, in, out, false);
    constexpr int HTL = S::HT[L];
    if constexpr (L + 1 < S::NH) {
      const float* grow = a.gate[L] + nc * (HTL * 16) + 4 * q;
#pragma unroll
      for (int t = 0; t < HTL; ++t) {
        const f32x4 h = *reinterpret_cast<const f32x4*>(grow + t * 16);
#pragma unroll
        for (int r = 0; r < 4; ++r) in[t][r] = out[t][r] * (h[r] > 0.f ? 1.f : 0.f);
      }
      if (live) {
#pragma unroll
        for (int t = 0; t < HTL; ++t) *reinterpret_cast<f32x4*>(a.act_out[L] + n * (HTL * 16) + t * 16 + 4 * q) = in[t];
      }
      ars_dgrad_stack<S, L + 1, Ring>(ring, zero_q, q, in, out, a, n, nc, live);
    } else if (live) {
#pragma unroll
      for (int t = 0; t < HTL; ++t)
        if ((t + 1) * 16 <= S::DOUT || t * 16 + 4 * q < S::DOUT) *reinterpret_cast<f32x4*>(a.phi_out + n * a.ldphi + t * 16 + 4 * q) = out[t];
    }
  }
}

template <class S> __global__ __launch_bounds__(512, 2) void ars_dgrad_kernel(ArArgs a) {
  typedef ArRingS<8> Ring;
  static_assert(S::NH >= 1 && S::NH <= 4 && S::TMAX <= 16, "dgrad chain: up to three gated layers + the input layer, widths <= 256");
  typedef ArChainLds<ARS_CH, S::TMAX> Lds;
  const ArLane ln;
  const int wave = ln.wave, j = ln.j, q = ln.q;
  Ring ring;
  ring.start(ars_lds, a.stream, a.n_chunks, wave, ln.lane);
  float* zero_lds = Lds::template zero_fill<512>(ars_lds, ln.tid);
  __syncthreads();
  for (int64_t tile = blockIdx.x; tile < a.n_tiles; tile += gridDim.x) {
    const int64_t n = tile * 128 + wave * 16 + j;
    const bool live = n < a.N;
    const int64_t nc = live ? n : a.N - 1;
    const float* grow = a.x + nc * a.ldx;
    f32x4 in[S::TMAX], out[S::TMAX];
#pragma unroll
    for (int it = 0; it < S::NIT; ++it) in[it] = *reinterpret_cast<const f32x4*>(grow + it * 16 + 4 * q);
    ars_dgrad_stack<S, 0, Ring>(ring, zero_lds + 4 * q, q, in, out, a, n, nc, live);
  }
  asm volatile("s_waitcnt vmcnt(0)" ::: "memory");
}

template <class S> static int ars_dgrad_launch(const ArArgs* in, int abi, int args_bytes, void* stream) {
  if (abi != ARS_ABI || args_bytes != (int)sizeof(ArArgs)) return ZK_EINVAL;
  ArArgs a = *in;
  if (a.DIN != S::DIN || a.D != S::DOUT || a.L != S::NH || a.n_chunks != S::NCHUNK || !a.x || !a.phi_out || a.ldx % 4 || a.ldphi % 4 || ((uintptr_t)a.x % 16) ||
      ((uintptr_t)a.phi_out % 16))
    return ZK_EINVAL;
  for (int l = 0; l + 1 < S::NH; ++l)
    if (!a.gate[l] || !a.act_out[l] || ((uintptr_t)a.gate[l] % 16) || ((uintptr_t)a.act_out[l] % 16)) return ZK_EINVAL;
  a.n_tiles = (a.N + 127) / 128;
  return ar_launch_dyn_lds((const void*)ars_dgrad_kernel<S>, 256, 512, ArChainLds<ARS_CH, S::TMAX>::bytes(0), a, stream);
}

template <class S, typename Uni> static int ars_launch(const ArArgs* in, int abi, int args_bytes, int train, void* stream) {
  if (abi != ARS_ABI || args_bytes != (int)sizeof(ArArgs)) return ZK_EINVAL;
  ArArgs a = *in;
  if (a.D != S::D || a.DIN != S::DIN || a.L != S::NH + 1 || a.act != S::ACT || a.sched || a.NG != S::NG || a.n_chunks != S::NCHUNK) return ZK_EINVAL;
  if (a.l1rev && !S::HAS_ALT) return ZK_EINVAL;
  if (a.bin_out || a.knots_out) return ZK_EINVAL;
  if (train && (!S::TRAIN_OK || !a.phi_out)) return ZK_EINVAL;
  a.n_tiles = (a.N + 16 * S::WAVES - 1) / (16 * S::WAVES);
  a.xs = ((S::D + 3) / 4) * 4 + 4;
  const bool vec_ok = (S::D % 4 == 0) && (train || ((a.ldy % 4 == 0) && ((uintptr_t)a.y % 16 == 0)));
  if (S::XLDS != 0 && !vec_ok) return ZK_EINVAL;
  a.xlds = S::XLDS;
  const int lds = ArLds::bytes(ARS_NR * ARS_CH * AR_TF, a.bias_floats, S::XLDS ? S::WAVES : 0, a.xs);
  if (lds > 160 * 1024) return ZK_EINVAL;
  const void* fn = nullptr;
  if (train) {
    if constexpr (S::TRAIN_OK) fn = (const void*)ars_kernel<S, Uni, true>;
  } else {
    fn = (const void*)ars_kernel<S, Uni, false>;
  }
  if (!fn) return ZK_EINVAL;
  return ar_launch_dyn_lds(fn, 256, 64 * S::WAVES, lds, a, stream);
}

}
```

zuko_amd/csrc/zk_ar_common.h:

```cpp
#pragma once
#include "zk_univariate.h"
#include <cstddef>
#include <cstring>
#include <mutex>
#include <unordered_map>

namespace zk {

typedef float f32x4 __attribute__((ext_vector_type(4)));

#define AR_TF 256
#define AR_WAVES 8
#define AR_T 16
#define ARS_ABI 9
#ifndef ARX_ABL
#define ARX_ABL 0
#endif
#ifndef ARH_POISON_ONE
#define ARH_POISON_ONE 1
#endif

struct ArArgs {
  int64_t N;
  int D, DIN;
  const float* x; int64_t ldx;
  float* y; int64_t ldy;
  const float* yin; int64_t ldyin;
  float* ladj; int accumulate;
  const float* stream;
  const float* bias;
  const uint32_t* skip;
  const int32_t* featmap;
  int L, NG, n_chunks, act, bias_floats, dbg;
  const int* sched;
  int n_sched;
  int olim[8];
  int g0, g1;
  int xlds;
  int xs;
  float bound, ls;
  RqsLeanConst lc;
  int64_t n_tiles;
  int32_t* bin_out;
  float* knots_out;
  int l1rev;
  float* act_out[3];
  float* phi_out;
  int64_t ldphi;
  const float* gate[3];
  const float* phi_in;
  float* gphi_out;
  int64_t ldpin;
  const float* gy; int64_t ldgy;
  const float* gl;
  int phi_packed;
  SosConst<float> sos;
  float eps;
  float wdescale[4];
  unsigned* amax[4];
};

__device__ __forceinline__ float act_f32(float v, int act) {
  switch (act) {
    case 1: return v < 0.f ? 0.f : v;
    case 2: return v > 0.f ? v : expm1f(v);
    case 3: return tanhf(v);
    case 4: return v / (1.f + expf(-v));
    case 5: return 0.5f * v * (1.f + erff(v * 0.70710678118654752440f));
    case 6: return 1.f / (1.f + expf(-v));
    case 7: return v > 0.f ? v : 0.01f * v;
    default: return v;
  }
}


struct UniAffine {
  static constexpr int TOTAL = 2, FPL = 2, NT = 1;
  template <bool INV> static __device__ __forceinline__ void poison(float* p, int base, float nan_or_zero) {
    p[base + 0] += nan_or_zero;
    p[base + 1] += nan_or_zero;
  }
  static constexpr int NKNOT = 1;
  template <typename P, typename A> static __device__ __forceinline__ void fwd(const P& p, int base, const A& a, float x, float& y, float& lj, int* k = nullptr, float* ks = nullptr) {
    affine_fwd<float, MathFast>(p(base + 0), p(base + 1), a.ls, x, y, lj);
  }
  template <typename P, typename A> static __device__ __forceinline__ float inv(const P& p, int base, const A& a, float y) {
    return affine_inv<float, MathFast>(p(base + 0), p(base + 1), a.ls, y);
  }
};

template <int K, bool CIRC> struct UniRqs {
  static constexpr int TOTAL = 3 * K - 1, FPL = 1, NT = (TOTAL + 3) / 4;
  static __device__ __forceinline__ float shift(float v, float bound) {
    const float period = 2.f * bound;
    float r = fmodf(v, period);
    r = (r < 0.f) ? r + period : r;
    return r - bound;
  }
  template <bool INV> static __device__ __forceinline__ void poison(float* p, int base, float nan_or_zero) {
#if ARH_POISON_ONE
    p[base + (INV ? K : 0)] += nan_or_zero;
#else
#pragma unroll
    for (int j = 0; j < K; ++j) p[base + (INV ? K : 0) + j] += nan_or_zero;
#endif
  }
  static constexpr int NKNOT = K + 1;
  template <typename P, typename A> static __device__ __forceinline__ void fwd(const P& p, int base, const A& a, float x, float& y, float& lj, int* k = nullptr, float* ks = nullptr) {
    int kk;
    rqs_lean<K, false>([&](int j) { return p(base + j); }, [&](int j) { return p(base + K + j); }, [&](int j) { return p(base + 2 * K + j); }, a.lc,
                       CIRC ? shift(x, a.bound) : x, y, lj, kk, ks);
    if (k) *k = kk;
  }
  template <typename P, typename A> static __device__ __forceinline__ float inv(const P& p, int base, const A& a, float y) {
    float x, lj;
    rqs_lean<K, true>([&](int j) { return p(base + j); }, [&](int j) { return p(base + K + j); }, [&](int j) { return p(base + 2 * K + j); }, a.lc, y, x, lj);
    return CIRC ? shift(x, a.bound) : x;
  }
};
template <int P, int L1> struct UniSos {
  static constexpr int TOTAL = P * L1 + 1, FPL = 1, NT = (TOTAL + 3) / 4, NKNOT = 1;
  template <bool INV> static __device__ __forceinline__ void poison(float* p, int base, float nan_or_zero) {
    p[base] += nan_or_zero;
    p[base + P * L1] += nan_or_zero;
  }
  template <typename Pa, typename A> static __device__ __forceinline__ void fwd(const Pa& p, int base, const A& a, float x, float& y, float& lj, int* k = nullptr, float* ks = nullptr) {
    auto ld = [&](int j) { return p(base + j); };
    y = sos_f_static<float, P, L1>(a.sos, ld, x) + p(base + P * L1);
    lj = t_log(sos_g_static<float, P, L1>(a.sos, ld, x));
  }
};
template <int NC> struct UniBernBounded {
  static constexpr int TOTAL = NC - 5, FPL = 1, NT = (TOTAL + 3) / 4, NKNOT = 1;
  template <bool INV> static __device__ __forceinline__ void poison(float* p, int base, float nan_or_zero) { p[base] += nan_or_zero; }
  template <typename Pa, typename A> static __device__ __forceinline__ void fwd(const Pa& p, int base, const A& a, float x, float& y, float& lj, int* k = nullptr, float* ks = nullptr) {
    float th[NC];
    bern_theta_bounded<float, NC>([&](int j) { return p(base + j); }, a.bound, th);
    const BernTails<float> t = bern_tails<float, NC>(th, true, a.bound, a.eps);
    float d;
    bern_fwd<float, NC>(th, t, a.bound, x, y, d, a.eps);
    lj = t_log(d);
  }
};
typedef UniSos<3, 5> UniSos3x5;
typedef UniBernBounded<22> UniBern17;
typedef UniRqs<8, false> UniRqs8;
typedef UniRqs<4, false> UniRqs4;
typedef UniRqs<16, false> UniRqs16;
typedef UniRqs<8, true> UniCircRqs8;


struct ArLds {
  static constexpr int FMAP_WORDS = 1024, SKIP_WORDS = 256;
  static constexpr int bytes(int ring_floats, int bias_floats, int row_waves, int xs) {
    return (ring_floats + bias_floats + FMAP_WORDS + SKIP_WORDS + row_waves * 16 * xs) * (int)sizeof(float);
  }
  static __device__ __forceinline__ int* fmap(float* bias, int bias_floats) { return reinterpret_cast<int*>(bias + bias_floats); }
  static __device__ __forceinline__ int* skip(int* fmap_) { return fmap_ + FMAP_WORDS; }
  static __device__ __forceinline__ float* row(int* fmap_, int wave, int j, int xs) {
    return reinterpret_cast<float*>(fmap_ + FMAP_WORDS + SKIP_WORDS) + wave * 16 * xs + j * xs;
  }
  template <int THREADS> static __device__ __forceinline__ void stage(const ArArgs& a, int tid, float* bias, int* fmap_, int n_fmap, int skip0 = 0, int n_skip = 0) {
    for (int i = tid; i < a.bias_floats; i += THREADS) bias[i] = a.bias[i];
    for (int i = tid; i < n_fmap; i += THREADS) fmap_[i] = a.featmap[i];
    for (int i = tid; i < n_skip; i += THREADS) skip(fmap_)[i] = (int)a.skip[skip0 + i];
    __syncthreads();
  }
};

struct ArLane {
  int tid, lane, wave, j, q;
  __device__ __forceinline__ ArLane() : tid(threadIdx.x), lane(tid & 63), wave(__builtin_amdgcn_readfirstlane(tid >> 6)), j(lane & 15), q(lane >> 4) {}
};

template <int NIT, int M> __device__ __forceinline__ float ar_poison_of(const f32x4 (&v)[M]) {
  int bad = 0;
#pragma unroll
  for (int it = 0; it < NIT; ++it)
#pragma unroll
    for (int r = 0; r < 4; ++r) bad |= !(fabsf(v[it][r]) < __builtin_inff());
  bad |= __shfl_xor(bad, 16, 64);
  bad |= __shfl_xor(bad, 32, 64);
  return bad ? __builtin_nanf("") : 0.f;
}

template <int D, int M> __device__ __forceinline__ void ar_rows_in(float* xr, int q, const f32x4 (&v)[M]) {
#pragma unroll
  for (int it = 0; it < (D + 15) / 16; ++it)
    if ((it + 1) * 16 <= D || it * 16 + 4 * q < D) *reinterpret_cast<f32x4*>(xr + it * 16 + 4 * q) = v[it];
  asm volatile("" ::: "memory");
  __builtin_amdgcn_wave_barrier();
}
template <int D> __device__ __forceinline__ void ar_rows_out(const float* xr, int q, float* yrow, bool live) {
  asm volatile("" ::: "memory");
  __builtin_amdgcn_wave_barrier();
  if (live) {
#pragma unroll
    for (int it = 0; it < (D + 15) / 16; ++it)
      if ((it + 1) * 16 <= D || it * 16 + 4 * q < D) *reinterpret_cast<f32x4*>(yrow + it * 16 + 4 * q) = *reinterpret_cast<const f32x4*>(xr + it * 16 + 4 * q);
  }
}
template <int ACT, int N, int M> __device__ __forceinline__ void ar_activate(f32x4 (&dst)[M], const f32x4 (&src)[M]) {
  if constexpr (ACT == 1) {
#pragma unroll
    for (int t = 0; t < N; ++t)
#pragma unroll
      for (int r = 0; r < 4; ++r) dst[t][r] = src[t][r] < 0.f ? 0.f : src[t][r];
  } else if constexpr (ACT == 0) {
#pragma unroll
    for (int t = 0; t < N; ++t) dst[t] = src[t];
  } else {
#pragma unroll 1
    for (int rep = 0; rep < 1; ++rep) {
#pragma unroll
      for (int t = 0; t < N; ++t)
#pragma unroll
        for (int r = 0; r < 4; ++r) dst[t][r] = act_f32(src[t][r], ACT);
    }
  }
}
template <int NG, int FPL, bool REGS> struct ArFids {
  int r[REGS ? NG * FPL : 1];
  const int* fmap;
  int q;
  __device__ __forceinline__ ArFids(const int* fmap_lds, int q_) : fmap(fmap_lds), q(q_) {
    if constexpr (REGS) {
#pragma unroll
      for (int i = 0; i < NG; ++i)
#pragma unroll
        for (int fi = 0; fi < FPL; ++fi) r[i * FPL + fi] = fmap[(i * 4 + q) * FPL + fi];
    }
  }
  template <bool XLDS> __device__ __forceinline__ void fetch(int g, const float* xr, const float* xrow, int (&fid)[FPL], float (&xin)[FPL]) const {
#pragma unroll
    for (int fi = 0; fi < FPL; ++fi) {
      if constexpr (REGS) fid[fi] = r[g * FPL + fi];
      else fid[fi] = fmap[(g * 4 + q) * FPL + fi];
      const int fc = fid[fi] < 0 ? 0 : fid[fi];
      if constexpr (XLDS) xin[fi] = xr[fc];
      else xin[fi] = xrow[fc];
    }
  }
};

template <typename Uni, bool DIAG, bool XLDS, bool ABL = true>
__device__ __forceinline__ void ar_uni_epilogue(float (&p)[4 * Uni::NT], const ArArgs& a, const int (&fid)[Uni::FPL], const float (&xin)[Uni::FPL], float poison, float* xr, int64_t n,
                                                bool live, int D, float& lacc) {
  constexpr int FPL = Uni::FPL, TOTAL = Uni::TOTAL;
#pragma unroll
  for (int fi = 0; fi < FPL; ++fi) Uni::template poison<false>(p, fi * TOTAL, poison);
  auto ld = [&](int i) { return p[i]; };
#pragma unroll
  for (int fi = 0; fi < FPL; ++fi) {
    const int f = fid[fi];
    if (f >= 0) {
      float yv, lj;
      if (ABL && ARX_ABL == 3) {
        yv = p[fi * TOTAL] + xin[fi]; lj = p[fi * TOTAL + 1];
#pragma unroll
        for (int i = 2; i < TOTAL; ++i) lj += p[fi * TOTAL + i];
      } else if constexpr (DIAG) {
        int kb = 0;
        float ks[Uni::NKNOT];
        Uni::fwd(ld, fi * TOTAL, a, xin[fi], yv, lj, &kb, ks);
        if (live) {
          a.bin_out[n * D + f] = kb;
#pragma unroll
          for (int jj = 0; jj < Uni::NKNOT; ++jj) a.knots_out[(n * D + f) * Uni::NKNOT + jj] = ks[jj];
        }
      } else Uni::fwd(ld, fi * TOTAL, a, xin[fi], yv, lj);
      if constexpr (XLDS) xr[f] = yv;
      else if (live) a.y[n * a.ldy + f] = yv;
      lacc += lj;
    }
  }
}

template <bool PREFETCHED = false> __device__ __forceinline__ void ar_ladj_store(const ArArgs& a, float lacc, int64_t n, bool live, int q, float ladj_in = 0.f) {
  if (a.ladj) {
    lacc += __shfl_xor(lacc, 16, 64);
    lacc += __shfl_xor(lacc, 32, 64);
    if (live && q == 0) a.ladj[n] = a.accumulate ? (PREFETCHED ? ladj_in : a.ladj[n]) + lacc : lacc;
  }
}

static inline int ar_launch_dyn_lds(const void* fn, int max_grid, int block, int lds_bytes, ArArgs& a, void* stream) {
  hipError_t e = hipSuccess;
  {
    static std::mutex mu;
    static std::unordered_map<const void*, int> granted;
    std::lock_guard<std::mutex> lock(mu);
    int& g = granted[fn];
    if (g < lds_bytes) {
      e = hipFuncSetAttribute(fn, hipFuncAttributeMaxDynamicSharedMemorySize, lds_bytes);
      if (e != hipSuccess) return (int)e;
      g = lds_bytes;
    }
  }
  const unsigned grid = (unsigned)(a.n_tiles < max_grid ? a.n_tiles : max_grid);
  void* kargs[] = {&a};
  e = hipLaunchKernel(fn, dim3(grid), dim3((unsigned)block), kargs, lds_bytes, (hipStream_t)stream);
  if (e != hipSuccess) return (int)e;
  return ZK_LAUNCH_CHECK();
}

template <class Args> static inline bool ar_args_norm(const Args* p, Args* out) {
  if (!p || p->version != 1 || p->struct_size < offsetof(Args, phi_packed) || p->struct_size > sizeof(Args)) return false;
  std::memset(out, 0, sizeof(*out));
  std::memcpy(out, p, p->struct_size);
  out->struct_size = sizeof(Args);
  return true;
}

}
```

zuko_amd/distributions.py:

```python

from __future__ import annotations

import torch
from torch import Size, Tensor
from torch.distributions import Distribution, Independent, Normal, Transform, Uniform
from torch.distributions.utils import _sum_rightmost

from . import ops

__all__ = ["BoxUniform", "DiagNormal", "NormalizingFlow"]

Distribution._validate_args = False
Distribution.arg_constraints = {}


class DiagNormal(Independent):

    def __init__(self, loc: Tensor, scale: Tensor, ndims: int = 1) -> None:
        super().__init__(Normal(torch.as_tensor(loc), torch.as_tensor(scale)), ndims)

    def __repr__(self) -> str:
        return "Diag" + repr(self.base_dist)

    def expand(self, batch_shape: Size, new: Distribution | None = None) -> Distribution:
        new = self._get_checked_instance(DiagNormal, new)
        return super().expand(batch_shape, new)


class BoxUniform(Independent):

    def __init__(self, lower: Tensor, upper: Tensor, ndims: int = 1) -> None:
        super().__init__(Uniform(torch.as_tensor(lower), torch.as_tensor(upper)), ndims)

    def __repr__(self) -> str:
        return "Box" + repr(self.base_dist)

    def expand(self, batch_shape: Size, new: Distribution | None = None) -> Distribution:
        new = self._get_checked_instance(BoxUniform, new)
        return super().expand(batch_shape, new)


class NormalizingFlow(Distribution):

    has_rsample = True

    def __init__(self, transform: Transform, base: Distribution) -> None:
        super().__init__()
        extra = transform.codomain.event_dim - len(base.event_shape)
        if extra > 0:
            base = Independent(base, extra)
        self.transform = transform
        self.base = base
        self.reinterpreted = max(-extra, 0)

    def __repr__(self) -> str:
        inner = f"(transform): {self.transform}\n(base): {self.base}".replace("\n", "\n  ")
        return f"{type(self).__name__}(\n  {inner}\n)"

    @property
    def batch_shape(self) -> Size:
        return self.base.batch_shape

    @property
    def event_shape(self) -> Size:
        return self.transform.inverse_shape(self.base.event_shape)

    def expand(self, batch_shape: Size, new: Distribution | None = None) -> Distribution:
        new = self._get_checked_instance(NormalizingFlow, new)
        new.transform = self.transform
        new.base = self.base.expand(batch_shape)
        new.reinterpreted = self.reinterpreted
        Distribution.__init__(new, validate_args=False)
        return new

    def _fusable_base(self):
        b = self.base
        if isinstance(b, DiagNormal) and b.reinterpreted_batch_ndims == 1 and self.reinterpreted == 0:
            n = b.base_dist
            loc, scale = n.loc, n.scale
            D = loc.shape[-1]
            if loc.dim() > 1:
                if any(s != 0 for s in loc.stride()[:-1]) or any(s != 0 for s in scale.stride()[:-1]):
                    return None
                loc = loc.as_strided((D,), (loc.stride(-1),))
                scale = scale.as_strided((D,), (scale.stride(-1),))
            return loc, scale
        return None

    def log_prob(self, x: Tensor) -> Tensor:
        z, ladj = self.transform.call_and_ladj(x)
        ladj = _sum_rightmost(ladj, self.reinterpreted)
        fused = self._fusable_base()
        if fused is not None and torch.is_grad_enabled() and (fused[0].requires_grad or fused[1].requires_grad):
            fused = None
        if fused is not None and z.is_cuda and torch.is_tensor(ladj) and ladj.shape == z.shape[:-1]:
            return ops.diag_normal_log_prob(z, fused[0], fused[1], ladj)
        return self.base.log_prob(z) + ladj

    def rsample(self, shape: Size = ()) -> Tensor:
        z = self.base.rsample(shape) if self.base.has_rsample else self.base.sample(shape)
        return self.transform.inv(z)

    def rsample_and_log_prob(self, shape: Size = ()):
        z = self.base.rsample(shape) if self.base.has_rsample else self.base.sample(shape)
        x, ladj = self.transform.inv.call_and_ladj(z)
        ladj = _sum_rightmost(ladj, self.reinterpreted)
        return x, self.base.log_prob(z) - ladj
```

zuko_amd/flows/autoregressive.py:

```python

from __future__ import annotations

from functools import partial
import math
import os
from math import ceil, prod
from typing import Callable, Sequence

import torch
from torch import BoolTensor, LongTensor, Size, Tensor
from torch.distributions import Transform

import weakref

import torch.nn as nn

from .. import fused
from ..distributions import DiagNormal
from ..lazy import Flow, LazyTransform, UnconditionalDistribution
from ..nn import MaskedLinear, MaskedMLP, _act_code
from ..transforms import AutoregressiveTransform, DependentTransform, MonotonicAffineTransform, MonotonicRQSTransform
from ..utils import broadcast, unpack
from .elementwise import ElementWiseTransform

# ... 228 lines not shown
            del cache[key]
        if key not in cache:
            state = None
            lay = self._fusable_layout()
            mods = list(self.hyper)
            simple = all(isinstance(a, MaskedLinear) != (i % 2 == 1) for i, a in enumerate(mods))
            codes = {_act_code(a) for a in mods if not isinstance(a, MaskedLinear)}
            if lay is not None and lay[0].kind in (0, 1, 2, 3, 5, 6) and simple and len(codes) == 1 and None not in codes and all(l.weight.dtype == torch.float32 for l in lins):
                layout = fused.UniLayout(lay[0].kind, lay[0].total, 1, (lay[0].total + 3) // 4, lay[0].bins)
                plan = inc.build_inc_plan([l.mask for l in lins], self.features, self.order.cpu().numpy(), layout)
                if plan is not None:
                    state = inc.IncAR(plan, lins, device, codes.pop(), lay[1], 1e-3 if lay[0].kind == 6 else lay[2], eps=lay[2] if lay[0].kind == 6 else None)
            cache[key] = (structure, state)
        return cache[key][1]

    def fused_state(self, device: torch.device, inverse: bool = False):
        cache = _FUSED_CACHE.setdefault(self, {})
        key = str(device) + ("/inv" if inverse else "")
        if inverse and self.order is None:
            return None
        lins_all = [m for m in self.hyper if isinstance(m, MaskedLinear)]
        structure = tuple((l.mask._version, l.mask.data_ptr()) for l in lins_all) + ((self.order._version, self.order.data_ptr()) if self.order is not None else ())
        if key in cache and cache[key][0] != structure:
            del cache[key]
        if key not in cache:
            state = None
            lay = self._fusable_layout()
            mods = list(self.hyper)
            lins = [m for m in mods if isinstance(m, MaskedLinear)]
            acts = [m for m in mods if not isinstance(m, MaskedLinear)]
            simple = all(isinstance(a, MaskedLinear) != (i % 2 == 1) for i, a in enumerate(mods))
            codes = {_act_code(a) for a in acts}
            if lay is not None and simple and len(codes) == 1 and None not in codes and all(l.weight.dtype == torch.float32 for l in lins):
                variant = fused.default_variant()
                wide = max([l.weight.shape[0] for l in lins[:-1]] + [lins[0].weight.shape[1]]) > fused.MAX_WIDTH
                poly = lay[0].kind in (5, 6)
                plan = None if ((wide or poly) and inverse) else fused.build_plan([l.mask for l in lins], self.features, lay[0], fused.chunk_of(variant), align_groups=inverse,
                                                                        max_width=fused.MAX_WIDTH_WIDE if wide else fused.MAX_WIDTH)
                if plan is not None:
                    state = fused.FusedAR(plan, device, codes.pop(), lay[1], 1e-3 if lay[0].kind == 6 else lay[2], variant)
                    if lay[0].kind == 6:
                        state.eps = lay[2]
                    if inverse:
                        state.set_sweeps(self.order.cpu().numpy(), self.passes)
            cache[key] = (structure, state)
        return cache[key][1]


_FUSED_CACHE: "weakref.WeakKeyDictionary" = weakref.WeakKeyDictionary()


def _incremental_enabled() -> bool:
    return os.environ.get("ZUKO_AMD_NO_INCREMENTAL", "0") != "1"


def _partial_inverse_enabled() -> bool:
    import os

    return os.environ.get("ZUKO_AMD_FULL_SWEEPS", "0") != "1"


class FusedAutoregressiveTransform(AutoregressiveTransform):

    def __init__(self, lazy: MaskedAutoregressiveTransform, c: Tensor | None) -> None:
        super().__init__(partial(lazy.meta, c), lazy.passes)
        self.lazy = lazy
        self.c = c

    def _fused(self, x: Tensor, need_generic: bool = False):
        if not (x.is_cuda and x.dtype == torch.float32 and x.dim() >= 1):
            return None
        if torch.is_grad_enabled() and (x.requires_grad or (self.c is not None and self.c.requires_grad) or any(p.requires_grad for p in self.lazy.hyper.parameters())):
            return None
        st = self.lazy.fused_state(x.device)
        if st is None:
            return None
        rows = x.numel() // max(x.shape[-1], 1)
        if self.c is not None and self.c.dim() > 1:
            rows = max(rows, self.c.numel() // max(self.c.shape[-1], 1))
        if not st.ready(rows) or (need_generic and not st.generic_ok):
            return None
        return st

    def _check_widths(self, x: Tensor, st) -> None:
        D = self.lazy.features
        C = 0 if self.c is None else self.c.shape[-1]
        din = getattr(getattr(st, "plan", None), "din", None)
        if x.shape[-1] != D or (din is not None and D + C != din):
            raise RuntimeError(f"zuko_amd: input of {x.shape[-1]} features + {C} context columns given to a conditioner built for "
                               f"{D} features + {(din - D) if din is not None else '?'} context columns")

    def _bf16_spline(self, x: Tensor):
        lazy = self.lazy
        if not (x.is_cuda and x.dtype == torch.bfloat16 and x.dim() >= 1) or os.environ.get("ZUKO_AMD_BF16_UNFUSED", "0") == "1":
            return None
        if torch.is_grad_enabled() and (x.requires_grad or any(p.requires_grad for p in lazy.hyper.parameters())):
            return None
        spec = lazy._rqs_spec()
        if spec is None or spec[0] not in (8, 16) or not hasattr(lazy.hyper, "bf16_rqs"):
            return None
        c = self.c
        if c is not None:
            xb, cb = broadcast(x, c, ignore=1)
            inp = torch.cat((xb, cb), dim=-1)
        else:
            xb, inp = x, x
        D = lazy.features
        batch = xb.shape[:-1]
        out = lazy.hyper.bf16_rqs(inp.reshape(-1, inp.shape[-1]), xb.reshape(-1, D), *spec)
        if out is None:
            return None
        return out[0].reshape(batch + (D,)), out[1].reshape(batch)

    def call_and_ladj(self, x: Tensor):
        st = self._fused(x)
        if st is None:
            out = self._bf16_spline(x)
            if out is None:
                out = self._train_fused(x)
            return out if out is not None else super().call_and_ladj(x)
        return self._run_fused(st, x, None)

    def _train_fused(self, x: Tensor):
        lazy, c = self.lazy, self.c
        D = lazy.features
        if not (torch.is_grad_enabled() and x.is_cuda and x.dtype == torch.float32 and x.dim() >= 1 and x.shape[-1] == D):
            return None
        if c is not None and not (c.is_cuda and c.dtype == torch.float32 and (D + c.shape[-1]) % 4 == 0):
            return None
        lay = lazy._fusable_layout()
        if lay is None or lay[0].kind not in (0, 1):
            return None
        from .. import train

        sizes = (1, 1) if lay[0].kind == 0 else (lay[0].bins, lay[0].bins, lay[0].bins - 1)
        if c is not None:
            xb, cb = broadcast(x, c, ignore=1)
            inp = torch.cat((xb, cb), dim=-1)
        else:
            xb, inp = x, x
        batch = xb.shape[:-1]
        out = train.autoregressive(lazy.hyper, (lay[0].kind, float(lay[1]), float(lay[2]), sizes), inp.reshape(-1, inp.shape[-1]), features=D)
        return None if out is None else (out[0].reshape(batch + (D,)), out[1].reshape(batch))

    def call_and_accumulate_ladj(self, x: Tensor, total: Tensor):
        if torch.is_grad_enabled() and (x.requires_grad or total.requires_grad):
            return None
        st = self._fused(x)
        batch = x.shape[:-1] if self.c is None else torch.broadcast_shapes(x.shape[:-1], self.c.shape[:-1])
        if st is None or total.dtype != x.dtype or total.device != x.device or tuple(total.shape) != tuple(batch) or not total.is_contiguous():
            return None
        return self._run_fused(st, x, total)[0]

    def _run_fused(self, st, x: Tensor, total):
        self._check_widths(x, st)
        lazy, c = self.lazy, self.c
        D = lazy.features
        if c is not None:
            xb, cb = broadcast(x, c, ignore=1)
        else:
            xb, cb = x, None
        batch = xb.shape[:-1]
        x2 = xb.reshape(-1, D)
        din = D + (0 if cb is None else cb.shape[-1])
        dinp = -(-din // 4) * 4
        if cb is None and dinp == D and x2.stride(-1) == 1 and x2.stride(0) % 4 == 0 and x2.data_ptr() % 16 == 0:
            inp = x2
        else:
            inp = x2.new_zeros((x2.shape[0], dinp))
            inp[:, :D] = x2
            if cb is not None:
                inp[:, D:din] = cb.reshape(-1, cb.shape[-1])
        y = torch.empty((x2.shape[0], D), dtype=x.dtype, device=x.device)
        ladj = torch.empty(x2.shape[0], dtype=x.dtype, device=x.device) if total is None else total.view(-1)
        st.refresh([m for m in lazy.hyper if isinstance(m, MaskedLinear)])
        st.run(inp, y, ladj, total is not None)
        return y.reshape(batch + (D,)), ladj.reshape(batch)

    def _call(self, x: Tensor) -> Tensor:
        return self.call_and_ladj(x)[0]

    def log_abs_det_jacobian(self, x: Tensor, y: Tensor) -> Tensor:
        return self.call_and_ladj(x)[1]

    @property
    def inv(self) -> Transform:
        return _FusedInverse(self)

    def inverse_and_ladj(self, y: Tensor):
        out = self._inverse_impl(y, True)
        if isinstance(out, tuple):
            return out
        return out, self.log_abs_det_jacobian(out, y)

    def _inverse(self, y: Tensor) -> Tensor:
        return self._inverse_impl(y, False)

    def _inverse_impl(self, y: Tensor, want_ladj: bool):
        st = self._fused(y, need_generic=True)
        if st is None:
            out = self._poly_incremental(y, want_ladj)
            return out if out is not None else self._ordered_inverse(y)
        self._check_widths(y, st)
        lazy, c = self.lazy, self.c
        D = lazy.features
        if c is not None:
            yb, cb = broadcast(y, c, ignore=1)
        else:
            yb, cb = y, None
        batch = yb.shape[:-1]
        y2 = yb.reshape(-1, D).contiguous()
        inc_state = lazy.incremental_state(y.device) if _incremental_enabled() and _partial_inverse_enabled() else None
        if inc_state is not None:
            inc_state.refresh([m for m in lazy.hyper if isinstance(m, MaskedLinear)])
            c2 = None if cb is None else cb.reshape(-1, cb.shape[-1]).contiguous()
            x2, l2 = inc_state.run(y2, c2, want_ladj)
            return (x2.reshape(batch + (D,)), l2.reshape(batch)) if want_ladj else x2.reshape(batch + (D,))
        din = D + (0 if cb is None else cb.shape[-1])
        buf = y2.new_zeros((y2.shape[0], -(-din // 4) * 4))
        if cb is not None:
            buf[:, D:din] = cb.reshape(-1, cb.shape[-1])
        lins = [m for m in lazy.hyper if isinstance(m, MaskedLinear)]
        part = lazy.fused_state(y.device, inverse=True) if _partial_inverse_enabled() else None
        if part is not None:
            part.refresh(lins)
            for s_ in range(self.passes):
                part.run_inverse_partial(buf, y2, s_)
        else:
            st.refresh(lins)
            for _ in range(self.passes):
                st.run_inverse_sweep(buf, y2)
        return buf[:, :D].reshape(batch + (D,)).contiguous() if buf.shape[1] != D else buf.reshape(batch + (D,))


    def _poly_incremental(self, y: Tensor, want_ladj: bool):
        lazy, c = self.lazy, self.c
        if not (y.is_cuda and y.dtype == torch.float32 and y.dim() >= 1 and _incremental_enabled() and _partial_inverse_enabled()) or want_ladj:
            return None
        if torch.is_grad_enabled() and (y.requires_grad or (c is not None and c.requires_grad) or any(p.requires_grad for p in lazy.hyper.parameters())):
            return None
        lay = lazy._fusable_layout()
        if lay is None or lay[0].kind not in (5, 6) or os.environ.get("ZUKO_AMD_FULL_SWEEPS", "0") == "1":
            return None
        inc_state = lazy.incremental_state(y.device)
        if inc_state is None:
            return None
        D = lazy.features
        if y.shape[-1] != D:
            return None
        if c is not None:
            yb, cb = broadcast(y, c, ignore=1)
        else:
            yb, cb = y, None
        batch = yb.shape[:-1]
        inc_state.refresh([m for m in lazy.hyper if isinstance(m, MaskedLinear)])
        c2 = None if cb is None else cb.reshape(-1, cb.shape[-1]).contiguous()
        x2, _ = inc_state.run(yb.reshape(-1, D).contiguous(), c2, False)
        return x2.reshape(batch + (D,))

    def _ordered_inverse(self, y: Tensor) -> Tensor:
        lazy, c = self.lazy, self.c
        mods = list(lazy.hyper) if isinstance(lazy.hyper, torch.nn.Sequential) else []
        grad = torch.is_grad_enabled() and (y.requires_grad or (c is not None and c.requires_grad) or any(p.requires_grad for p in lazy.hyper.parameters()))
        if lazy.order is None or grad or not mods or type(mods[-1]) is not MaskedLinear or not y.is_cuda or y.dtype not in (torch.float32, torch.float64) or os.environ.get("ZUKO_AMD_FULL_SWEEPS", "0") == "1":
            return super()._inverse(y)
        from .. import ops

        if c is not None:
            yb, cb = broadcast(y, c, ignore=1)
        else:
            yb, cb = y, None
        batch = yb.shape[:-1]
        y2 = yb.reshape(-1, lazy.features)
        c2 = None if cb is None else cb.reshape(-1, cb.shape[-1])

        def linear(h, w, b, m, act_module):
            code = None if act_module is None else _act_code(act_module)
            if act_module is None or code is not None:
                return ops.linear(h, w, b, m, code or 0)
            return act_module(ops.linear(h, w, b, m))

        x2 = wavefront_inverse(lazy, y2, c2, self.passes, linear, lambda phi, ys: lazy.univariate(*unpack(phi, lazy.shapes)).inv(ys))
        return x2.reshape(batch + (lazy.features,))


def wavefront_inverse(lazy: "MaskedAutoregressiveTransform", y2: Tensor, c2: Tensor | None, passes: int, linear, inverse_of, stack=None) -> Tensor:
    from ..nn import apply_stack

    stack = apply_stack if stack is None else stack

    mods = list(lazy.hyper)
    D, total, last = lazy.features, lazy.total, mods[-1]
    dev = y2.device
    x2 = torch.zeros_like(y2)
    units = lazy._sweep_units(dev, passes)
    if units is not None:
        hbuf = [y2.new_zeros((y2.shape[0], m.weight.shape[0])) for m in mods[0:-1:2]]
        urows = lazy._sweep_unit_rows(dev, passes) if y2.dtype == mods[0].weight.dtype else None
    sweep_no = {}
    for s_, idx in lazy._sweep_features(dev, passes):
        if units is None:
            h = stack(mods[:-1], x2 if c2 is None else torch.cat((x2, c2), dim=-1))
        else:
            h = x2 if c2 is None else torch.cat((x2, c2), dim=-1)
            for l, lin in enumerate(mods[0:-1:2]):
                first_t = sweep_no.get(l, 0)
                todo = [units[l][t] for t in range(first_t, s_ + 1) if units[l][t] is not None]
                sweep_no[l] = s_ + 1
                if todo:
                    u_ = todo[0] if len(todo) == 1 else torch.cat(todo)
                    if urows is not None:
                        wr, mr, br, starts = urows[l]
                        r0, r1 = starts[first_t], starts[s_ + 1]
                        w_, m_, bias = wr[r0:r1], mr[r0:r1], None if br is None else br[r0:r1]
                    else:
                        w_, m_, bias = lin.weight.index_select(0, u_), lin.mask.index_select(0, u_), None if lin.bias is None else lin.bias.index_select(0, u_)
                    hbuf[l].index_copy_(1, u_, linear(h, w_, bias, m_, mods[2 * l + 1]))
                h = hbuf[l]
        if isinstance(idx, tuple):
            lo, hi = idx
            rows, k = slice(lo * total, hi * total), hi - lo
            w, b, m, ys = last.weight[rows], None if last.bias is None else last.bias[rows], last.mask[rows], y2[:, lo:hi]
        else:
            rows, k = (idx[:, None] * total + torch.arange(total, device=dev)[None, :]).reshape(-1), idx.numel()
            w, b, m, ys = last.weight.index_select(0, rows), None if last.bias is None else last.bias.index_select(0, rows), last.mask.index_select(0, rows), y2.index_select(1, idx)
        xs = inverse_of(linear(h, w, b, m, None).unflatten(-1, (k, total)), ys)
        if isinstance(idx, tuple):
            x2[:, idx[0] : idx[1]] = xs
# ... 50 lines not shown
```

zuko_amd/fused.py:

```python

from __future__ import annotations

from dataclasses import dataclass

import ctypes
import math
import os

import numpy as np
import torch
from torch import Tensor

TILE = 16
CHUNK = 24
GROUP_HIDDEN = 4
MAX_WIDTH = 256
MAX_WIDTH_WIDE = 512


@dataclass
class UniLayout:

    kind: int
    total: int
# ... 349 lines not shown
        raise ValueError(f"zuko_amd.set_matmul_precision: unknown mode '{mode}' (one of {sorted(_PRECISIONS)})")
    _precision = _PRECISIONS[mode.lower()]


HALF_SPREAD_LOG2 = 14
HALF_SMALL_FRACTION = 0.01
HALF_ROW_LOG2 = 12
HALF_MIN_LOG2, HALF_MAX_LOG2 = -20, 40


def half_scales(linears):
    stats = []
    for m in linears:
        w = m.weight.detach()
        a = (w * m.mask).abs() if getattr(m, "mask", None) is not None else w.abs()
        big = a.amax()
        nz = a > 0
        small = (nz & (a < big * 2.0 ** -HALF_SPREAD_LOG2)).sum() / nz.sum().clamp_min(1)
        rowmax = a.amax(dim=1)
        minrow = torch.where(rowmax > 0, rowmax, big).amin()
        bias = getattr(m, "bias", None)
        bfin = torch.isfinite(bias.detach()).all() if bias is not None else torch.ones((), dtype=torch.bool, device=w.device)
        stats.append(torch.stack([big.float(), small.float(), minrow.float(), bfin.float()]))
    out = []
    for big, small, minrow, bfin in torch.stack(stats).tolist():
        if big == 0.0:
            out.append((bfin == 1.0, 0))
            continue
        ok = bfin == 1.0 and math.isfinite(big) and 2.0 ** HALF_MIN_LOG2 <= big <= 2.0 ** HALF_MAX_LOG2 and small <= HALF_SMALL_FRACTION and minrow >= big * 2.0 ** -HALF_ROW_LOG2
        out.append((bool(ok), 15 - math.frexp(big)[1] if math.isfinite(big) else 0))
    return out


def chunk_of(variant: int = 0) -> int:
    return CHUNK


def default_variant() -> int:
    return 0


class FusedAR:

    def __init__(self, plan: ArPlan, device: torch.device, act: int, bound: float, slope: float, variant: int = 0) -> None:
        self.plan = plan
        self.variant = variant
        self.device = device
        self.act = act
        self.bound = bound
        self.slope = slope
        self.skip = torch.from_numpy(plan.skip.view(np.int32).copy()).to(device)
        self.featmap = torch.from_numpy(plan.featmap.copy()).to(device)
        self.gather = [torch.from_numpy(g).to(device) for g in plan.gather]
        self.bias_gather = [torch.from_numpy(g).to(device) for g in plan.bias_gather]
        self.stream = torch.empty(plan.n_blocks * 256, dtype=torch.float32, device=device)
        self.bias_floats = plan.bias_off[-1] + len(plan.bias_gather[-1])
        self.bias = torch.empty(self.bias_floats, dtype=torch.float32, device=device)
        self._stamp = None
        self._fine_stamp = None
        self.generic_ok = plan.max_width <= MAX_WIDTH and plan.layout.kind <= 4
        self.eps = 1e-6
        self._gl = None
        self.static = None
        self._static_tried_rows = -1
        self.fine_gather = self.fine_stream = self.fine_offsets = None
        self.fine_n_chunks = 0
        self.half = None
        self.half_gather = self.half_stream = self.half_offsets = None
        self.half_n_chunks = 0
        self.half_ok = False
        self.half_descale = None
        self._half_stamp = None
        self._acquire_static(None)
        self.gs_mode = os.environ.get("ZUKO_AMD_GSPLIT", "1")
        self.gs = None
        self._gs_stamp = self._seen_stamp = None

    @property
    def static_variant(self) -> int:
        return 0 if self.static is None else 1 + self.static[1]

    def _acquire_static(self, rows) -> None:
        from . import static_ar

        upgradable = self.static is not None and not self.static[0].meta.get("split") and static_ar.split_enabled() and rows is not None
        self._acquire_half(rows)
        if (self.static is not None and not upgradable) or self.plan.fine_gather is None or (rows is not None and rows <= self._static_tried_rows):
            return
        if rows is not None:
            self._static_tried_rows = rows if rows < static_ar.jit_min_rows() else 1 << 62
        found = static_ar.lookup(self.plan, self.plan.layout.kind, self.act, rows)
        if found is not None and (self.static is None or found[0] is not self.static[0]):
            self.static = found
            if found[0].meta.get("split"):
                t, gathers = static_ar.split_tables(self.plan, self.plan.layout.kind, self.act)
                self.fine_gather = [torch.from_numpy(g).to(self.device) for g in gathers]
                self.fine_offsets = [b * 256 for b in t["BASE"]] + [t["LAST_BASE"] * 256]
                self.fine_n_chunks = t["NCHUNK"]
                stream_images = t["STREAM_IMAGES"]
            else:
                self.fine_gather = [torch.from_numpy(g).to(self.device) for g in self.plan.fine_gather]
                self.fine_offsets = [b * 256 for b in self.plan.fine_layer_block0]
                self.fine_n_chunks = self.plan.fine_n_chunks
                stream_images = self.fine_n_chunks * 24
            self.fine_stream = torch.zeros(stream_images * 256, dtype=torch.float32, device=self.device)
            self._fine_stamp = None

    def _acquire_half(self, rows) -> None:
        from . import static_ar

        if self.half is not None or self.plan.fine_gather is None or not static_ar.half_enabled() or (rows is not None and rows <= getattr(self, "_half_tried_rows", -1)):
            return
        if rows is not None:
            self._half_tried_rows = rows if rows < static_ar.jit_min_rows() else 1 << 62
        kern = static_ar.lookup_half(self.plan, self.plan.layout.kind, self.act, rows)
        if kern is not None:
            t, gathers = static_ar.half_tables(self.plan, self.plan.layout.kind, self.act)
            self.half = kern
            self.half_gather = [torch.from_numpy(g).to(self.device) for g in gathers]
            self.half_offsets = [b * 256 for b in t["BASE"]] + [t["LAST_BASE"] * 256]
            self.half_n_chunks = t["NCHUNK"]
            self.half_stream = torch.zeros(t["STREAM_IMAGES"] * 256, dtype=torch.float32, device=self.device)
            self._half_stamp = None

    def _refresh_half(self, linears, stamp) -> None:
        from . import _C
        from .ops import _ptr, _stream

        scales = half_scales(linears)
        self._half_stamp = stamp
        self.half_ok = all(ok for ok, _ in scales)
        if not self.half_ok:
            return
        self.half_descale = [2.0 ** -e for _, e in scales]
        for l, (m, (_, e)) in enumerate(zip(linears, scales)):
            w = m.weight.detach()
            if not w.is_contiguous():
                w = w.contiguous()
            nb = self.half_gather[l].numel() // 512
            if nb:
                _C.check(_C.lib().zk_gather_split_f16(_ptr(w), _ptr(m.mask.contiguous().view(torch.uint8)), _ptr(self.half_gather[l]), nb, _ptr(self.half_stream[self.half_offsets[l] :]), 2.0 ** e,
                                                      _stream()), "zk_gather_split_f16")

    def _half_args(self, **io):
        p = self.plan
        from . import _C
        from .ops import _ptr

        d = list(self.half_descale) + [1.0] * (4 - len(self.half_descale))
        return _C.args("zk_ar_args_v1", launcher=self.half.launcher, rev=0, uni_kind=p.layout.kind, D=p.features, wstream=_ptr(self.half_stream), bias=_ptr(self.bias),
                       bias_floats=self.bias_floats, featmap=_ptr(self.featmap), n_layers=p.n_layers, n_groups=p.n_groups, n_chunks=self.half_n_chunks, act=self.act,
                       bound=self.bound, slope=self.slope, wdescale0=d[0], wdescale1=d[1], wdescale2=d[2], wdescale3=d[3], **io)

    def _half_serves(self, y: Tensor) -> bool:
        return (self.half is not None and self.half_ok and self._half_stamp is not None and self._half_stamp == self._seen_stamp and matmul_precision() == "f16x2"
                and self.gs_mode != "force" and (not self.half.meta["XLDS"] or (y.stride(0) % 4 == 0 and y.data_ptr() % 16 == 0)))

    def ready(self, rows: int) -> bool:
        from . import static_ar

        self._acquire_static(static_ar.effective_rows(self, rows))
        return self.generic_ok or self.static is not None

    def _gsplit(self):
        from . import static_ar

        if self.gs_mode == "0" or (self.static is not None and self.gs_mode != "force") or not self.generic_ok or not static_ar.split_enabled():
            return None
        if self.gs is None:
            t = gsplit_gather(self.plan)
            if t is None:
                self.gs = False
            else:
                gathers, offsets, n_chunks = t
                self.gs = ([torch.from_numpy(g).to(self.device) for g in gathers], offsets, n_chunks,
                           torch.zeros(n_chunks * GS_BLOCKS_PER_CHUNK * 768, dtype=torch.float32, device=self.device))
        return self.gs or None

    def refresh(self, linears, fine_only: bool = False) -> None:
        from . import _C
        from .ops import _ptr, _stream

        from .nn import _param_stamp

        stamp = _param_stamp(linears)
        self._seen_stamp = stamp
        want_generic = self.generic_ok and not (fine_only and self.static is not None) and stamp != self._stamp
        want_fine = self.static is not None and stamp != self._fine_stamp
        gs = self._gsplit()
        want_gs = gs is not None and stamp != self._gs_stamp
        if self.half is not None and not fine_only and stamp != self._half_stamp and matmul_precision() == "f16x2":
            self._refresh_half(linears, stamp)
        if not (want_generic or want_fine or want_gs):
            return
        items = []
        for l, m in enumerate(linears):
            w = m.weight.detach()
            if not w.is_contiguous():
                w = w.contiguous()
            mask = m.mask.contiguous().view(torch.uint8)
            if want_generic:
                items.append((w, mask, self.gather[l], self.gather[l].numel(), self.stream[self.plan.layer_block0[l] * 256 :], 0))
            if want_fine:
                fdst = self.fine_stream[self.fine_offsets[l] :]
                if self.static[0].meta.get("split"):
                    items.append((w, mask, self.fine_gather[l], self.fine_gather[l].numel() // 512, fdst, 1))
                else:
                    items.append((w, mask, self.fine_gather[l], self.fine_gather[l].numel(), fdst, 0))
            if want_gs and gs[0][l].numel():
                items.append((w, mask, gs[0][l], gs[0][l].numel() // 512, gs[3][gs[1][l] :], 1))
            nb = self.bias_gather[l].numel()
            bdst = self.bias[self.plan.bias_off[l] :]
            if m.bias is None:
                bdst[:nb].zero_()
            else:
                items.append((m.bias.detach().contiguous(), None, self.bias_gather[l], nb, bdst, 0))
        _C.gather_multi(items, _stream())
        if want_generic:
            self._stamp = stamp
        if want_fine:
            self._fine_stamp = stamp
        if want_gs:
            self._gs_stamp = stamp

    def run(self, inp: Tensor, y: Tensor, ladj: Tensor | None, accumulate: bool) -> None:
        from . import _C
        from .ops import _ptr, _stream

        p = self.plan
        N = inp.shape[0]
        if self._half_serves(y):
            a = self._half_args(N=N, DIN=inp.shape[1], x=_ptr(inp), ldx=inp.stride(0), y=_ptr(y), ldy=y.stride(0), ladj=_ptr(ladj), accumulate=int(accumulate))
            _C.check(_C.lib().zk_ar_forward_static(a, _stream()), "zk_ar_forward_static")
            return
        gs = self._gsplit()
        if gs is not None and self._gs_stamp is not None and self._gs_stamp == self._seen_stamp and (p.layout.kind <= 1 or (p.features % 4 == 0 and y.stride(0) % 4 == 0 and y.data_ptr() % 16 == 0)):
            a = self._generic_args(N=N, DIN=inp.shape[1], x=_ptr(inp), ldx=inp.stride(0), y=_ptr(y), ldy=y.stride(0), ladj=_ptr(ladj), accumulate=int(accumulate))
            a.wstream, a.n_chunks = gs[3].data_ptr(), gs[2]
            _C.check(_C.lib().zk_ar_forward_split(a, _stream()), "zk_ar_forward_split")
            return
        if self.static is not None:
            kern, rev = self.static
            if not kern.meta["XLDS"] or (y.stride(0) % 4 == 0 and y.data_ptr() % 16 == 0):
                extra = {}
                if p.layout.kind == 5:
                    if self._gl is None:
                        from .ops import _leggauss01

                        self._gl = _leggauss01(5)
                    extra = dict(gl_nodes01=ctypes.cast(self._gl[0], ctypes.c_void_p), gl_weights01=ctypes.cast(self._gl[1], ctypes.c_void_p))
                elif p.layout.kind == 6:
                    extra = dict(eps=float(self.eps))
                a = _C.args("zk_ar_args_v1", launcher=kern.launcher, rev=rev, uni_kind=p.layout.kind, N=N, D=p.features, DIN=inp.shape[1], x=_ptr(inp), ldx=inp.stride(0),
                            y=_ptr(y), ldy=y.stride(0), ladj=_ptr(ladj), accumulate=int(accumulate), wstream=_ptr(self.fine_stream), bias=_ptr(self.bias),
                            bias_floats=self.bias_floats, featmap=_ptr(self.featmap), n_layers=p.n_layers, n_groups=p.n_groups, n_chunks=self.fine_n_chunks, act=self.act,
                            bound=self.bound, slope=self.slope, **extra)
                _C.check(_C.lib().zk_ar_forward_static(a, _stream()), "zk_ar_forward_static")
                return
        if not self.generic_ok:
            raise RuntimeError("zuko_amd: this conditioner is wider than the generic fused kernel covers and has no static-shape kernel (FusedAR.ready() was not consulted)")
        a = self._generic_args(N=N, DIN=inp.shape[1], x=_ptr(inp), ldx=inp.stride(0), y=_ptr(y), ldy=y.stride(0), ladj=_ptr(ladj), accumulate=int(accumulate))
        _C.check(_C.lib().zk_ar_forward(a, _stream()), "zk_ar_forward")

    def _generic_args(self, **io):
        from . import _C
        from .ops import _ptr

        p = self.plan
        return _C.args("zk_ar_args_v1", uni_kind=p.layout.kind, D=p.features, wstream=_ptr(self.stream), bias=_ptr(self.bias), bias_floats=self.bias_floats, skip=_ptr(self.skip),
                       featmap=_ptr(self.featmap), n_layers=p.n_layers, n_groups=p.n_groups, n_chunks=p.n_chunks, act=self.act, bound=self.bound, slope=self.slope, **io)

    def run_diag(self, inp: Tensor, y: Tensor, ladj: Tensor, bins: Tensor, knots: Tensor) -> None:
        from . import _C
        from .ops import _ptr, _stream

        p = self.plan
        if self._half_serves(y) and p.layout.kind in (1, 2, 3) and y.stride(0) % 4 == 0 and y.data_ptr() % 16 == 0:
            a = self._half_args(N=inp.shape[0], DIN=inp.shape[1], x=_ptr(inp), ldx=inp.stride(0), y=_ptr(y), ldy=y.stride(0), ladj=_ptr(ladj), accumulate=0, bin_out=_ptr(bins), knots_out=_ptr(knots))
            _C.check(_C.lib().zk_ar_forward_static(a, _stream()), "zk_ar_forward_static")
            return
        if self.static is not None and self.static[0].meta.get("split") and y.stride(0) % 4 == 0 and y.data_ptr() % 16 == 0:
            kern, rev = self.static
            a = _C.args("zk_ar_args_v1", launcher=kern.launcher, rev=rev, uni_kind=p.layout.kind, N=inp.shape[0], D=p.features, DIN=inp.shape[1], x=_ptr(inp), ldx=inp.stride(0),
                        y=_ptr(y), ldy=y.stride(0), ladj=_ptr(ladj), accumulate=0, wstream=_ptr(self.fine_stream), bias=_ptr(self.bias), bias_floats=self.bias_floats,
                        featmap=_ptr(self.featmap), n_layers=p.n_layers, n_groups=p.n_groups, n_chunks=self.fine_n_chunks, act=self.act, bound=self.bound, slope=self.slope,
                        bin_out=_ptr(bins), knots_out=_ptr(knots))
            _C.check(_C.lib().zk_ar_forward_static(a, _stream()), "zk_ar_forward_static")
            return
        a = self._generic_args(N=inp.shape[0], DIN=inp.shape[1], x=_ptr(inp), ldx=inp.stride(0), y=_ptr(y), ldy=y.stride(0), ladj=_ptr(ladj), bin_out=_ptr(bins), knots_out=_ptr(knots))
        gs = self._gsplit()
        if gs is not None and self._gs_stamp is not None and self._gs_stamp == self._seen_stamp and p.features % 4 == 0 and y.stride(0) % 4 == 0 and y.data_ptr() % 16 == 0:
            a.wstream, a.n_chunks = gs[3].data_ptr(), gs[2]
            _C.check(_C.lib().zk_ar_forward_split(a, _stream()), "zk_ar_forward_split")
            return
        err = _C.lib().zk_ar_forward_diag(a, _stream())
        _C.check(err, "zk_ar_forward_diag")

    def run_inverse_sweep(self, buf: Tensor, y: Tensor) -> None:
        from . import _C
        from .ops import _ptr, _stream

        a = self._generic_args(N=buf.shape[0], DIN=buf.shape[1], x=_ptr(buf), ldx=buf.stride(0), y_in=_ptr(y), ldy=y.stride(0), x_out=_ptr(buf), ldo=buf.stride(0))
        err = _C.lib().zk_ar_inverse_sweep(a, _stream())
        _C.check(err, "zk_ar_inverse_sweep")


    def set_sweeps(self, order: np.ndarray, passes: int) -> None:
        import ctypes

        p = self.plan
        per_group = 4 * p.layout.fpl
        slot_order = np.where(p.featmap >= 0, order[np.maximum(p.featmap, 0)], -1)
        self.sweeps = []
        flat: list[int] = []
        for s_ in range(passes):
            slots = np.nonzero(slot_order == s_)[0]
            if slots.size == 0:
                self.sweeps.append(None)
                continue
            g0, g1 = int(slots.min() // per_group), int(slots.max() // per_group) + 1
            sched, olim = partial_schedule(p, g0, g1)
            if not sched:
                sched = [0]
            self.sweeps.append((len(flat), len(sched), (ctypes.c_int * len(olim))(*olim), g0, g1))
            flat += sched
        self.sched_dev = torch.tensor(flat, dtype=torch.int32, device=self.device)

    def run_inverse_partial(self, buf: Tensor, y: Tensor, sweep: int) -> None:
        from . import _C
        from .ops import _ptr, _stream
        import ctypes

        entry = self.sweeps[sweep]
        if entry is None:
            return
        off, n_sched, olim, g0, g1 = entry
        sched_ptr = ctypes.c_void_p(self.sched_dev.data_ptr() + 4 * off)
        a = self._generic_args(N=buf.shape[0], DIN=buf.shape[1], x=_ptr(buf), ldx=buf.stride(0), y_in=_ptr(y), ldy=y.stride(0), x_out=_ptr(buf), ldo=buf.stride(0),
                               sched=sched_ptr, n_sched=n_sched, olim=olim, g0=g0, g1=g1)
        err = _C.lib().zk_ar_inverse_partial(a, _stream())
        _C.check(err, "zk_ar_inverse_partial")
```

zuko_amd/static_ar.py:

```python

from __future__ import annotations

import ctypes
import fcntl
import hashlib
import json
import math
import os
import shutil
import subprocess
import sys
import threading

import numpy as np

HERE = os.path.dirname(os.path.abspath(__file__))
CSRC = os.path.join(HERE, "csrc")
ARS_DIR = os.path.join(HERE, "lib", "ars")
ARS_ABI = 9
UNI_TYPES = {0: "zk::UniAffine", 1: "zk::UniRqs8", 2: "zk::UniRqs4", 3: "zk::UniRqs16", 4: "zk::UniCircRqs8", 5: "zk::UniSos3x5", 6: "zk::UniBern17"}
SPLIT_ONLY_KINDS = {3, 5, 6}
_HEADERS = ("fused_ar_static_impl.h", "fused_ar_split_impl.h", "zk_ar_common.h", "zk_univariate.h", "zk_univariate_bwd.h", "zk_common.h", "zk_half.h")


def _hipcc() -> str | None:
    for cand in (os.environ.get("HIPCC"), "/opt/rocm/bin/hipcc", shutil.which("hipcc")):
        if cand and os.path.exists(cand):
            return cand
    return None


def _arch() -> str:
    from . import _build

    return _build.ARCH


def _jit_dir() -> str:
    d = os.environ.get("ZUKO_AMD_CACHE_DIR")
    return os.path.join(d, "ars") if d else ARS_DIR


def _dirs() -> list[str]:
    d = _jit_dir()
    return [ARS_DIR] if d == ARS_DIR else [d, ARS_DIR]


def _find(name: str) -> str | None:
    for d in _dirs():
        path = os.path.join(d, name)
        if os.path.exists(path):
            return path
    return None


_WARNED: set = set()


def _warn_once(key: str, msg: str) -> None:
    if key not in _WARNED:
        _WARNED.add(key)
        sys.stderr.write(f"[zuko_amd static_ar] {msg}\n")


def _build_so(stem: str, source, meta: dict | None, verbose: bool, out_dir: str | None = None) -> str | None:
    have = _find(stem + ".so")
    if have is not None and (meta is None or os.path.exists(have[: -len(".so")] + ".json")):
        return have
    hipcc = _hipcc()
    if hipcc is None:
        _warn_once("nohipcc", f"no hipcc on this machine: the static-shape kernel {stem} cannot be compiled; this conditioner runs on the generic operand-split kernel "
                              "(same results; 1.1-1.6x the generated kernel's time; conditioners wider than 256 run layer by layer).  Build it where a ROCm compiler is installed (zuko_amd.static_ar.prebuild, or one call at the "
                              "target batch size) and ship zuko_amd/lib/ars/ or ZUKO_AMD_CACHE_DIR with the package.")
        return None
    d = out_dir or _jit_dir()
    try:
        os.makedirs(d, exist_ok=True)
        so = os.path.join(d, stem + ".so")
        with open(os.path.join(d, f".lock_{stem}"), "w") as lock:
            fcntl.flock(lock, fcntl.LOCK_EX)
            if os.path.exists(so) and (meta is None or os.path.exists(os.path.join(d, stem + ".json"))):
                return so
            src = os.path.join(d, stem + ".hip")
            with open(src, "w") as f:
                f.write(source())
            tmp = os.path.join(d, f".{stem}.so.{os.getpid()}")
            cmd = [hipcc, "-O3", "-std=c++17", "-fPIC", f"--offload-arch={_arch()}", "-Wno-unused-result", "-Wno-uninitialized", "-ffp-contract=off", f"-I{CSRC}", "-shared", "-no-hip-rt",
                   *os.environ.get("ZUKO_AMD_STATIC_CXXFLAGS", "").split(),
                   src, f"-L{_torch_lib_dir()}", "-l:libamdhip64.so", "-o", tmp]
            if verbose:
                print("[zuko_amd static_ar]", " ".join(cmd), flush=True)
            elif out_dir is None:
                _warn_once("jit", f"compiling a static-shape kernel for this conditioner on first use ({stem}, 10-25 s; ZUKO_AMD_JIT=0 disables, ZUKO_AMD_CACHE_DIR redirects)")
            r = subprocess.run(cmd, stdout=subprocess.PIPE, stderr=subprocess.STDOUT, text=True)
            if r.returncode != 0:
                sys.stderr.write(f"[zuko_amd static_ar] hipcc failed for {src}:\n{r.stdout[-2000:]}\n")
                try:
                    os.remove(tmp)
                except OSError:
                    pass
                return None
            os.replace(tmp, so)
            if meta is not None:
                with open(os.path.join(d, stem + ".json"), "w") as f:
                    json.dump(meta, f)
        return so
    except OSError as exc:
        _warn_once("oserror:" + d, f"cannot build kernels in {d} ({exc}); staying on the generic kernels (set ZUKO_AMD_CACHE_DIR to a writable directory)")
        return None


_HEADER_DIGEST: str | None = None


def _header_digest() -> str:
    global _HEADER_DIGEST
    if _HEADER_DIGEST is None:
        h = hashlib.sha256(str(ARS_ABI).encode())
        for name in _HEADERS:
            with open(os.path.join(CSRC, name), "rb") as f:
                h.update(f.read())
        _HEADER_DIGEST = h.hexdigest()[:12]
    return _HEADER_DIGEST


_HALF_DIGEST = None


def _half_digest() -> str:
    global _HALF_DIGEST
    if _HALF_DIGEST is None:
        h = hashlib.sha256(_header_digest().encode())
        with open(os.path.join(CSRC, "fused_ar_half_impl.h"), "rb") as f:
            h.update(f.read())
        _HALF_DIGEST = h.hexdigest()[:12]
    return _HALF_DIGEST


def _stamp_of(meta: dict) -> str:
    return _half_digest() if meta.get("half") else _header_digest()




def tables(plan, uni_kind: int, act: int = 1) -> dict | None:
    if plan.fine_gather is None or uni_kind not in UNI_TYPES or act not in range(8):
        return None
    L = plan.n_layers
    NH = L - 1
    if NH < 1 or NH > 6:
        return None
    tm = plan.fine_tilemask
    n_otg = tm.shape[1]
    widths = list(plan.widths)
    HT = [-(-w // 16) for w in widths]
    din4 = -(-plan.din // 4) * 4
    NIT = -(-plan.din // 16)
    TMAX = 4 * -(-max([NIT] + HT) // 4)
    if TMAX > 32:
        return None
    S_OTG, S_IT, S_MASK, NS = [], [], [], []
    for l in range(NH):
        n = 0
        for otg in range(n_otg):
            for it in range(tm.shape[2]):
                m = int(tm[l, otg, it])
                if m:
                    S_OTG.append(otg)
                    S_IT.append(it)
                    S_MASK.append(m)
                    n += 1
        NS.append(n)
# ... 765 lines not shown
```

zuko_amd/transforms.py:

```python

from __future__ import annotations

from typing import Callable, Sequence

import torch
from torch import Tensor
from torch.distributions import Transform, constraints
from torch.distributions.utils import _sum_rightmost

from . import ops

__all__ = [
    "AdditiveTransform",
    "AutoregressiveTransform",
    "BernsteinTransform",
    "BoundedBernsteinTransform",
    "CircularShiftTransform",
    "ComposedTransform",
    "CouplingTransform",
    "DependentTransform",
    "MonotonicAffineTransform",
    "MonotonicRQSTransform",
    "SOSPolynomialTransform",
    "ShiftedSOSPolynomialTransform",
# ... 154 lines not shown

    bijective = True

    def __init__(self, bound: float = 1.0, **kwargs) -> None:
        super().__init__(**kwargs)
        self.bound = bound
        self.domain = constraints.interval(-bound, bound)
        self.codomain = constraints.interval(-bound, bound)

    def __repr__(self) -> str:
        return f"{self.__class__.__name__}(bound={self.bound})"

    def _call(self, x):
        return torch.remainder(x, 2 * self.bound) - self.bound

    def _inverse(self, y):
        return torch.remainder(y, 2 * self.bound) - self.bound

    def log_abs_det_jacobian(self, x, y):
        return torch.zeros_like(x)


class AdditiveTransform(Transform):

    domain = constraints.real
    codomain = constraints.real
    bijective = True
    sign = +1

    def __init__(self, shift: Tensor, **kwargs) -> None:
        super().__init__(**kwargs)
        self.shift = shift

    def _call(self, x):
        return x + self.shift

    def _inverse(self, y):
        return y - self.shift

    def log_abs_det_jacobian(self, x, y):
        return torch.zeros_like(x)




class DependentTransform(Transform):

    def __init__(self, base: Transform, reinterpreted: int, **kwargs) -> None:
        super().__init__(**kwargs)
        self.base = base
        self.reinterpreted = reinterpreted

    def __repr__(self) -> str:
        return f"{self.__class__.__name__}({self.base}, {self.reinterpreted})"

    @property
    def domain(self):
        return constraints.independent(self.base.domain, self.reinterpreted)

    @property
    def codomain(self):
        return constraints.independent(self.base.codomain, self.reinterpreted)

    @property
    def bijective(self) -> bool:
        return self.base.bijective

    def _call(self, x):
        return self.base(x)

    @property
    def inv(self) -> Transform:
        return DependentTransform(self.base.inv, self.reinterpreted)

    def _inverse(self, y):
        return self.base.inv(y)

    def log_abs_det_jacobian(self, x, y):
        return self.call_and_ladj(x)[1] if hasattr(self.base, "call_and_ladj_reduced") and self.reinterpreted == 1 else _sum_rightmost(
            self.base.log_abs_det_jacobian(x, y), self.reinterpreted
        )

    def call_and_ladj(self, x):
        if self.reinterpreted == 1 and hasattr(self.base, "call_and_ladj_reduced") and x.dim() >= 1:
            return self.base.call_and_ladj_reduced(x)
        y, ladj = self.base.call_and_ladj(x)
        return y, _sum_rightmost(ladj, self.reinterpreted)

    def forward_shape(self, shape):
        return self.base.forward_shape(shape)

    def inverse_shape(self, shape):
        return self.base.inverse_shape(shape)


class ComposedTransform(Transform):

    def __init__(self, *transforms: Transform, **kwargs) -> None:
        super().__init__(**kwargs)
        if not transforms:
            raise AssertionError("'transforms' cannot be empty")
        self.transforms = list(transforms)
        dim = 0
        for t in reversed(self.transforms):
            dim = t.domain.event_dim + max(dim - t.codomain.event_dim, 0)
        self.domain_dim = dim
        for t in self.transforms:
            dim += t.codomain.event_dim - t.domain.event_dim
        self.codomain_dim = dim

    def __repr__(self) -> str:
        body = "\n".join(f"  ({i}): " + repr(t).replace("\n", "\n  ") for i, t in enumerate(self.transforms))
        return f"{self.__class__.__name__}(\n{body}\n)"

    @staticmethod
    def _lift(c, extra: int):
        return constraints.independent(c, extra) if extra > 0 else c

    @property
    def domain(self):
        d = self.transforms[0].domain
        return self._lift(d, self.domain_dim - d.event_dim)

    @property
    def codomain(self):
        c = self.transforms[-1].codomain
        return self._lift(c, self.codomain_dim - c.event_dim)

    @property
    def bijective(self) -> bool:
        return all(t.bijective for t in self.transforms)

    def _call(self, x):
        for t in self.transforms:
            x = t(x)
        return x

    @property
    def inv(self) -> Transform:
        rev = ComposedTransform.__new__(ComposedTransform)
        Transform.__init__(rev)
        rev.transforms = [t.inv for t in reversed(self.transforms)]
        rev.domain_dim, rev.codomain_dim = self.codomain_dim, self.domain_dim
        return rev

    def _inverse(self, y):
        for t in reversed(self.transforms):
            y = t.inv(y)
        return y

    def log_abs_det_jacobian(self, x, y):
        return self.call_and_ladj(x)[1]

    def call_and_ladj(self, x):
        dim = self.domain_dim
        total = None
        owned = False
        for t in self.transforms:
            acc = getattr(t, "call_and_accumulate_ladj", None)
            y = acc(x, total) if (acc is not None and owned and dim == t.domain.event_dim) else None
            if y is not None:
                x = y
            else:
                x, ladj = t.call_and_ladj(x)
                ladj = _sum_rightmost(ladj, dim - t.domain.event_dim)
                owned = acc is not None if total is None else True
                total = ladj if total is None else total + ladj
            dim += t.codomain.event_dim - t.domain.event_dim
        return x, total

    def forward_shape(self, shape):
        for t in self.transforms:
            shape = t.forward_shape(shape)
        return shape

    def inverse_shape(self, shape):
        for t in reversed(self.transforms):
            shape = t.inverse_shape(shape)
        return shape


class AutoregressiveTransform(Transform):

    domain = constraints.real_vector
    codomain = constraints.real_vector
    bijective = True

    def __init__(self, meta: Callable[[Tensor], Transform], passes: int, **kwargs) -> None:
        super().__init__(**kwargs)
        self.meta = meta
        self.passes = passes

    def _call(self, x):
        return self.meta(x)(x)

    def _inverse(self, y):
        x = torch.zeros_like(y)
        for _ in range(self.passes):
            x = self.meta(x).inv(y)
        return x

    def log_abs_det_jacobian(self, x, y):
        return self.meta(x).log_abs_det_jacobian(x, y)

    def call_and_ladj(self, x):
        return self.meta(x).call_and_ladj(x)


class CouplingTransform(Transform):

    domain = constraints.real_vector
    codomain = constraints.real_vector
    bijective = True

    def __init__(self, meta: Callable[[Tensor], Transform], mask: Tensor, **kwargs) -> None:
        super().__init__(**kwargs)
        self.meta = meta
        self.idx_a = mask.nonzero().squeeze(-1)
        self.idx_b = (~mask).nonzero().squeeze(-1)

    def split(self, x):
        return x[..., self.idx_a], x[..., self.idx_b]

    def merge(self, a, b, shape):
        out = a.new_empty(shape)
        out[..., self.idx_a] = a
        out[..., self.idx_b] = b
        return out

    def _call(self, x):
        a, b = self.split(x)
        return self.merge(a, self.meta(a)(b), x.shape)

    def _inverse(self, y):
        a, b = self.split(y)
        return self.merge(a, self.meta(a).inv(b), y.shape)

    def log_abs_det_jacobian(self, x, y):
        a, b = self.split(x)
        return self.meta(a).log_abs_det_jacobian(b, self.split(y)[1])

    def call_and_ladj(self, x):
        a, b = self.split(x)
        yb, ladj = self.meta(a).call_and_ladj(b)
        return self.merge(a, yb, x.shape), ladj
```

Measured before the change: 74.24 million samples/s.

## Fuse diagonal-normal base log-prob into last autoregressive transform kernel

Adds a terminal variant of the split and half static AR kernels that evaluates the diagonal Normal base log-density in the epilogue. Per-feature loc, inverse variance and log-normaliser are staged in LDS, and the result is accumulated into ladj instead of writing z. This removes the final transform's y write and the separate base log_prob kernel that re-reads z. It bumps the ABI, adds an env switch to disable it, and falls back when shapes or kernels don't qualify.

After: 75.19 million samples/s (median of 6 runs). +1.3%, better.

```diff
diff --git a/include/zuko_amd.h b/include/zuko_amd.h
--- a/include/zuko_amd.h
+++ b/include/zuko_amd.h
@@ -127,6 +127,8 @@
   uint32_t* amax1;
   uint32_t* amax2;
   uint32_t* amax3;
+  const void* base_loc;
+  const void* base_scale;
 } zk_ar_args_v1;
 
 int zk_ar_forward(const zk_ar_args_v1* args, void* stream);
diff --git a/zuko_amd/csrc/fused_ar.hip b/zuko_amd/csrc/fused_ar.hip
--- a/zuko_amd/csrc/fused_ar.hip
+++ b/zuko_amd/csrc/fused_ar.hip
@@ -403,6 +403,8 @@
   float* knots_out = nullptr;
   double wdescale[4] = {0.0, 0.0, 0.0, 0.0};
   unsigned* amax[4] = {nullptr, nullptr, nullptr, nullptr};
+  const float* base_loc = nullptr;
+  const float* base_scale = nullptr;
   const int* sched = nullptr;
   int n_sched = 0;
   const int* olim = nullptr;
@@ -454,6 +456,8 @@
     a.eps = (float)(part.eps > 0.0 ? part.eps : 1e-6);
     for (int l = 0; l < 4; ++l) a.wdescale[l] = (float)part.wdescale[l];
     for (int l = 0; l < 4; ++l) a.amax[l] = part.amax[l];
+    if ((part.base_loc != nullptr) != (part.base_scale != nullptr) || (part.base_loc && (!ladj || part.phi_out || part.bin_out))) return ZK_EINVAL;
+    a.base_loc = part.base_loc; a.base_scale = part.base_scale;
     return ((ars_launch_fn)part.static_fn)(&a, ARS_ABI, (int)sizeof(ArArgs), part.phi_out != nullptr, stream);
   }
   a.xs = ((D + 3) / 4) * 4 + 4;
@@ -516,6 +520,7 @@
   part.gl_nodes01 = args->gl_nodes01; part.gl_weights01 = args->gl_weights01; part.eps = args->eps;
   part.bin_out = args->bin_out; part.knots_out = args->knots_out;
   part.wdescale[0] = args->wdescale0; part.wdescale[1] = args->wdescale1; part.wdescale[2] = args->wdescale2; part.wdescale[3] = args->wdescale3;
+  part.base_loc = (const float*)args->base_loc; part.base_scale = (const float*)args->base_scale;
   zk_ar_args_v1 p = *args;
   p.skip = nullptr;
   return ar_launch_v1(part, false, p, stream);
diff --git a/zuko_amd/csrc/fused_ar_half_impl.h b/zuko_amd/csrc/fused_ar_half_impl.h
--- a/zuko_amd/csrc/fused_ar_half_impl.h
+++ b/zuko_amd/csrc/fused_ar_half_impl.h
@@ -202,7 +202,7 @@
   }
 }
 
-template <class S, typename Uni, bool DIAG = false> __global__ __launch_bounds__(64 * S::WAVES, S::OCC) void arh_kernel(ArArgs a) {
+template <class S, typename Uni, bool DIAG, bool TERM> __device__ __forceinline__ void arh_body(const ArArgs& a) {
   typedef ArhRing<S::WAVES, S::CH, S::NR> Ring;
   static_assert(S::WAVES == 8 && S::NR == 3 && S::TMAX <= 16 && S::TMAX % 2 == 0 && S::OCC == 2, "two-part split kernels: widths <= 256, two wavefronts per SIMD");
   constexpr int NT = Uni::NT, FPL = Uni::FPL, TOTAL = Uni::TOTAL, WAVES = S::WAVES;
@@ -236,6 +236,8 @@
   float* const bias_lds = ars_lds + S::NR * S::CH * AR_TF;
   int* const fmap_lds = ArLds::fmap(bias_lds, a.bias_floats);
   float* const xr = ArLds::row(fmap_lds, wave, j, a.xs);
+  float* const base = ArLds::base(fmap_lds, NG * 4 * FPL);
+  if constexpr (TERM) ArLds::stage_base<64 * WAVES>(a, tid, base, S::D);
   ArLds::stage<64 * WAVES>(a, tid, bias_lds, fmap_lds, NG * 4 * FPL);
   const float* bias_last = bias_lds + S::NH * S::BIAS_STRIDE;
   const unsigned bias_last_addr = arx_lds_addr(bias_last + 4 * q);
@@ -306,6 +308,8 @@
       int fid[FPL];
       float xin[FPL];
       fids.template fetch<XLDS>(g, xr, xrow, fid, xin);
+      float bv[3 * FPL];
+      if constexpr (TERM) fids.fetch_base(fid, base, S::D, bv);
       f32x4 acc[NT], bs[NT];
       if constexpr (GN == 0) {
         const float* bg = bias_last + (g * NT) * 16 + 4 * q;
@@ -344,15 +348,18 @@
           if (ARH_POISON_ONE) asm("" : "+v"(p[4 * t + r]));
         }
       });
-      ar_uni_epilogue<Uni, DIAG, XLDS>(p, a, fid, xin, poison, xr, n, live, S::D, lacc);
+      ar_uni_epilogue<Uni, DIAG, XLDS, true, TERM>(p, a, fid, xin, poison, xr, n, live, S::D, lacc, bv);
     });
 #undef ARH_READ_LAST
     if (ARH_PREFETCH) ar_ladj_store<true>(a, lacc, n, live, q, ladj_in);
-    if constexpr (XLDS) ar_rows_out<S::D>(xr, q, a.y + n * a.ldy, live);
+    if constexpr (XLDS && !TERM) ar_rows_out<S::D>(xr, q, a.y + n * a.ldy, live);
     if (!ARH_PREFETCH) ar_ladj_store(a, lacc, n, live, q);
   }
   asm volatile("s_waitcnt vmcnt(0)" ::: "memory");
 }
+
+template <class S, typename Uni, bool DIAG = false> __global__ __launch_bounds__(64 * S::WAVES, S::OCC) void arh_kernel(ArArgs a) { arh_body<S, Uni, DIAG, false>(a); }
+template <class S, typename Uni> __global__ __launch_bounds__(64 * S::WAVES, S::OCC) void arht_kernel(ArArgs a) { arh_body<S, Uni, false, true>(a); }
 
 template <class S, typename Uni> static int arh_launch(const ArArgs* in, int abi, int args_bytes, int train, void* stream) {
   if (abi != ARS_ABI || args_bytes != (int)sizeof(ArArgs)) return ZK_EINVAL;
@@ -362,14 +369,18 @@
     if (!(a.wdescale[l] > 0.f) || !(a.wdescale[l] < __builtin_inff())) return ZK_EINVAL;
   a.n_tiles = (a.N + 16 * S::WAVES - 1) / (16 * S::WAVES);
   a.xs = ((S::D + 3) / 4) * 4 + 4;
-  const bool vec_ok = (S::D % 4 == 0) && (a.ldy % 4 == 0) && ((uintptr_t)a.y % 16 == 0);
+  const bool term = a.base_loc != nullptr;
+  if (term && (!a.base_scale || !a.ladj || a.bin_out || a.knots_out || !ArLds::base_fits(S::NG * 4 * Uni::FPL, S::D))) return ZK_EINVAL;
+  const bool vec_ok = (S::D % 4 == 0) && (term || ((a.ldy % 4 == 0) && ((uintptr_t)a.y % 16 == 0)));
   if (S::XLDS != 0 && !vec_ok) return ZK_EINVAL;
   a.xlds = S::XLDS;
   const int lds = ArLds::bytes(S::NR * S::CH * AR_TF, a.bias_floats, S::XLDS ? S::WAVES : 0, a.xs);
   if (lds > 160 * 1024) return ZK_EINVAL;
   const void* fn = nullptr;
   if ((a.bin_out != nullptr) != (a.knots_out != nullptr)) return ZK_EINVAL;
-  if (a.bin_out) {
+  if (term) {
+    fn = (const void*)arht_kernel<S, Uni>;
+  } else if (a.bin_out) {
     if constexpr (Uni::NKNOT > 1) fn = (const void*)arh_kernel<S, Uni, true>;
   } else {
     fn = (const void*)arh_kernel<S, Uni, false>;
diff --git a/zuko_amd/csrc/fused_ar_split_impl.h b/zuko_amd/csrc/fused_ar_split_impl.h
--- a/zuko_amd/csrc/fused_ar_split_impl.h
+++ b/zuko_amd/csrc/fused_ar_split_impl.h
@@ -140,7 +140,7 @@
   }
 }
 
-template <class S, typename Uni, bool TRAIN, bool DIAG = false> __global__ __launch_bounds__(64 * S::WAVES, S::OCC) void arx_kernel(ArArgs a) {
+template <class S, typename Uni, bool TRAIN, bool DIAG, bool TERM> __device__ __forceinline__ void arx_body(const ArArgs& a) {
   typedef ArRingS<S::WAVES, S::CH, S::NR> Ring;
   static_assert((S::WAVES == 8 || S::WAVES == 4) && (S::NR == 2 || S::NR == 3) && (S::TMAX <= 16 || (S::TMAX <= 32 && S::OCC == 1 && S::WAVES == 4)) && S::TMAX % 2 == 0,
                 "operand-split kernels: widths <= 256 with two wavefronts per SIMD, <= 512 with one");
@@ -156,6 +156,8 @@
   float* const bias_lds = ars_lds + S::NR * S::CH * AR_TF;
   int* const fmap_lds = ArLds::fmap(bias_lds, a.bias_floats);
   float* const xr = ArLds::row(fmap_lds, wave, j, a.xs);
+  float* const base = ArLds::base(fmap_lds, NG * 4 * FPL);
+  if constexpr (TERM) ArLds::stage_base<64 * WAVES>(a, tid, base, S::D);
   ArLds::stage<64 * WAVES>(a, tid, bias_lds, fmap_lds, NG * 4 * FPL);
   const float* bias_last = bias_lds + S::NH * S::BIAS_STRIDE;
   const unsigned bias_last_addr = arx_lds_addr(bias_last + 4 * q);
@@ -216,6 +218,8 @@
       int fid[FPL];
       float xin[FPL];
       fids.template fetch<XLDS>(g, xr, xrow, fid, xin);
+      float bv[3 * FPL];
+      if constexpr (TERM) fids.fetch_base(fid, base, S::D, bv);
       f32x4 acc[NT];
       if constexpr (GN > 0) {
         ars_for<NT>([&](auto t) ARS_ALWAYS_INLINE { acc[t] = arx_lds_raw<(g * NT + decltype(t)::value) * 64>(bias_last_addr); });
@@ -266,14 +270,17 @@
           }
         }
       }
-      if (uni_on) ar_uni_epilogue<Uni, DIAG, XLDS>(p, a, fid, xin, poison, xr, n, live, S::D, lacc);
+      if (uni_on) ar_uni_epilogue<Uni, DIAG, XLDS, true, TERM>(p, a, fid, xin, poison, xr, n, live, S::D, lacc, bv);
     });
-    if constexpr (XLDS) ar_rows_out<S::D>(xr, q, a.y + n * a.ldy, live && uni_on);
+    if constexpr (XLDS && !TERM) ar_rows_out<S::D>(xr, q, a.y + n * a.ldy, live && uni_on);
     if (uni_on) ar_ladj_store(a, lacc, n, live, q);
   }
   if constexpr (TRAIN) arx_amax_flush(a, mx, blockIdx.x * WAVES + wave, lane);
   asm volatile("s_waitcnt vmcnt(0)" ::: "memory");
 }
+
+template <class S, typename Uni, bool TRAIN, bool DIAG = false> __global__ __launch_bounds__(64 * S::WAVES, S::OCC) void arx_kernel(ArArgs a) { arx_body<S, Uni, TRAIN, DIAG, false>(a); }
+template <class S, typename Uni> __global__ __launch_bounds__(64 * S::WAVES, S::OCC) void arxt_kernel(ArArgs a) { arx_body<S, Uni, false, false, true>(a); }
 
 #ifndef ARXB_AHEAD
 #define ARXB_AHEAD 1
@@ -557,7 +564,9 @@
   if (train && (!S::TRAIN_OK || !a.phi_out || (a.phi_packed && (a.ldphi % 4 || a.ldphi < (int64_t)S::NG * Uni::NT * 16 || ((uintptr_t)a.phi_out % 16))))) return ZK_EINVAL;
   a.n_tiles = (a.N + 16 * S::WAVES - 1) / (16 * S::WAVES);
   a.xs = ((S::D + 3) / 4) * 4 + 4;
-  const bool vec_ok = (S::D % 4 == 0) && ((train && !a.y) || ((a.ldy % 4 == 0) && ((uintptr_t)a.y % 16 == 0)));
+  const bool term = a.base_loc != nullptr;
+  if (term && (train || !a.base_scale || !a.ladj || a.bin_out || a.knots_out || !ArLds::base_fits(S::NG * 4 * Uni::FPL, S::D))) return ZK_EINVAL;
+  const bool vec_ok = (S::D % 4 == 0) && ((train && !a.y) || term || ((a.ldy % 4 == 0) && ((uintptr_t)a.y % 16 == 0)));
   if (S::XLDS != 0 && !vec_ok) return ZK_EINVAL;
   a.xlds = S::XLDS;
   const int lds = ArLds::bytes(S::NR * S::CH * AR_TF, a.bias_floats, S::XLDS ? S::WAVES : 0, a.xs);
@@ -566,6 +575,8 @@
   if ((a.bin_out != nullptr) != (a.knots_out != nullptr) || (a.bin_out && train)) return ZK_EINVAL;
   if (train) {
     if constexpr (S::TRAIN_OK) fn = (const void*)arx_kernel<S, Uni, true>;
+  } else if (term) {
+    fn = (const void*)arxt_kernel<S, Uni>;
   } else if (a.bin_out) {
     if constexpr (Uni::NKNOT > 1) fn = (const void*)arx_kernel<S, Uni, false, true>;
   } else {
diff --git a/zuko_amd/csrc/fused_ar_static_impl.h b/zuko_amd/csrc/fused_ar_static_impl.h
--- a/zuko_amd/csrc/fused_ar_static_impl.h
+++ b/zuko_amd/csrc/fused_ar_static_impl.h
@@ -364,6 +364,7 @@
   if (a.D != S::D || a.DIN != S::DIN || a.L != S::NH + 1 || a.act != S::ACT || a.sched || a.NG != S::NG || a.n_chunks != S::NCHUNK) return ZK_EINVAL;
   if (a.l1rev && !S::HAS_ALT) return ZK_EINVAL;
   if (a.bin_out || a.knots_out) return ZK_EINVAL;
+  if (a.base_loc) return ZK_EINVAL;
   if (train && (!S::TRAIN_OK || !a.phi_out)) return ZK_EINVAL;
   a.n_tiles = (a.N + 16 * S::WAVES - 1) / (16 * S::WAVES);
   a.xs = ((S::D + 3) / 4) * 4 + 4;
diff --git a/zuko_amd/csrc/zk_ar_common.h b/zuko_amd/csrc/zk_ar_common.h
--- a/zuko_amd/csrc/zk_ar_common.h
+++ b/zuko_amd/csrc/zk_ar_common.h
@@ -12,7 +12,7 @@
 #define AR_TF 256
 #define AR_WAVES 8
 #define AR_T 16
-#define ARS_ABI 9
+#define ARS_ABI 10
 #ifndef ARX_ABL
 #define ARX_ABL 0
 #endif
@@ -58,6 +58,8 @@
   float eps;
   float wdescale[4];
   unsigned* amax[4];
+  const float* base_loc;
+  const float* base_scale;
 };
 
 __device__ __forceinline__ float act_f32(float v, int act) {
@@ -166,6 +168,16 @@
     for (int i = tid; i < n_skip; i += THREADS) skip(fmap_)[i] = (int)a.skip[skip0 + i];
     __syncthreads();
   }
+  static constexpr bool base_fits(int n_fmap, int D) { return n_fmap + 3 * D <= FMAP_WORDS; }
+  static __device__ __forceinline__ float* base(int* fmap_, int n_fmap) { return reinterpret_cast<float*>(fmap_ + n_fmap); }
+  template <int THREADS> static __device__ __forceinline__ void stage_base(const ArArgs& a, int tid, float* tab, int D) {
+    for (int i = tid; i < D; i += THREADS) {
+      const float s = a.base_scale[i];
+      tab[i] = a.base_loc[i];
+      tab[D + i] = 1.f / (2.f * (s * s));
+      tab[2 * D + i] = -t_log(s) - 0.91893853320467274178f;
+    }
+  }
 };
 
 struct ArLane {
@@ -241,11 +253,19 @@
       else xin[fi] = xrow[fc];
     }
   }
-};
-
-template <typename Uni, bool DIAG, bool XLDS, bool ABL = true>
+  __device__ __forceinline__ void fetch_base(const int (&fid)[FPL], const float* base, int D, float (&bv)[3 * FPL]) const {
+#pragma unroll
+    for (int fi = 0; fi < FPL; ++fi) {
+      const int fc = fid[fi] < 0 ? 0 : fid[fi];
+#pragma unroll
+      for (int k = 0; k < 3; ++k) bv[3 * fi + k] = base[k * D + fc];
+    }
+  }
+};
+
+template <typename Uni, bool DIAG, bool XLDS, bool ABL = true, bool TERM = false>
 __device__ __forceinline__ void ar_uni_epilogue(float (&p)[4 * Uni::NT], const ArArgs& a, const int (&fid)[Uni::FPL], const float (&xin)[Uni::FPL], float poison, float* xr, int64_t n,
-                                                bool live, int D, float& lacc) {
+                                                bool live, int D, float& lacc, const float* bv = nullptr) {
   constexpr int FPL = Uni::FPL, TOTAL = Uni::TOTAL;
 #pragma unroll
   for (int fi = 0; fi < FPL; ++fi) Uni::template poison<false>(p, fi * TOTAL, poison);
@@ -269,9 +289,15 @@
           for (int jj = 0; jj < Uni::NKNOT; ++jj) a.knots_out[(n * D + f) * Uni::NKNOT + jj] = ks[jj];
         }
       } else Uni::fwd(ld, fi * TOTAL, a, xin[fi], yv, lj);
-      if constexpr (XLDS) xr[f] = yv;
-      else if (live) a.y[n * a.ldy + f] = yv;
-      lacc += lj;
+      if constexpr (TERM) {
+        const float df = yv - bv[3 * fi];
+        lacc += lj;
+        lacc += __builtin_fmaf(-(df * df), bv[3 * fi + 1], bv[3 * fi + 2]);
+      } else {
+        if constexpr (XLDS) xr[f] = yv;
+        else if (live) a.y[n * a.ldy + f] = yv;
+        lacc += lj;
+      }
     }
   }
 }
diff --git a/zuko_amd/distributions.py b/zuko_amd/distributions.py
--- a/zuko_amd/distributions.py
+++ b/zuko_amd/distributions.py
@@ -1,5 +1,7 @@
 
 from __future__ import annotations
+
+import os
 
 import torch
 from torch import Size, Tensor
@@ -7,6 +9,7 @@
 from torch.distributions.utils import _sum_rightmost
 
 from . import ops
+from .transforms import ComposedTransform
 
 __all__ = ["BoxUniform", "DiagNormal", "NormalizingFlow"]
 
@@ -88,11 +91,17 @@
         return None
 
     def log_prob(self, x: Tensor) -> Tensor:
-        z, ladj = self.transform.call_and_ladj(x)
-        ladj = _sum_rightmost(ladj, self.reinterpreted)
         fused = self._fusable_base()
         if fused is not None and torch.is_grad_enabled() and (fused[0].requires_grad or fused[1].requires_grad):
             fused = None
+        if (fused is not None and isinstance(self.transform, ComposedTransform) and torch.is_tensor(x) and x.is_cuda and x.dtype == torch.float32
+                and os.environ.get("ZUKO_AMD_NO_FUSED_BASE", "0") != "1"):
+            z, ladj = self.transform.call_and_ladj(x, base=fused)
+            if z is None:
+                return ladj
+        else:
+            z, ladj = self.transform.call_and_ladj(x)
+        ladj = _sum_rightmost(ladj, self.reinterpreted)
         if fused is not None and z.is_cuda and torch.is_tensor(ladj) and ladj.shape == z.shape[:-1]:
             return ops.diag_normal_log_prob(z, fused[0], fused[1], ladj)
         return self.base.log_prob(z) + ladj
diff --git a/zuko_amd/flows/autoregressive.py b/zuko_amd/flows/autoregressive.py
--- a/zuko_amd/flows/autoregressive.py
+++ b/zuko_amd/flows/autoregressive.py
@@ -404,7 +404,21 @@
             return None
         return self._run_fused(st, x, total)[0]
 
-    def _run_fused(self, st, x: Tensor, total):
+    def call_and_log_prob(self, x: Tensor, total: Tensor | None, loc: Tensor, scale: Tensor):
+        if torch.is_grad_enabled() and (x.requires_grad or (total is not None and total.requires_grad)):
+            return None
+        st = self._fused(x)
+        if st is None:
+            return None
+        D = self.lazy.features
+        batch = x.shape[:-1] if self.c is None else torch.broadcast_shapes(x.shape[:-1], self.c.shape[:-1])
+        if total is not None and (total.dtype != x.dtype or total.device != x.device or tuple(total.shape) != tuple(batch) or not total.is_contiguous()):
+            return None
+        if any(v.dtype != torch.float32 or v.device != x.device or tuple(v.shape) != (D,) for v in (loc, scale)):
+            return None
+        return self._run_fused(st, x, total, base=(loc.contiguous(), scale.contiguous()))
+
+    def _run_fused(self, st, x: Tensor, total, base=None):
         self._check_widths(x, st)
         lazy, c = self.lazy, self.c
         D = lazy.features
@@ -423,9 +437,14 @@
             inp[:, :D] = x2
             if cb is not None:
                 inp[:, D:din] = cb.reshape(-1, cb.shape[-1])
+        st.refresh([m for m in lazy.hyper if isinstance(m, MaskedLinear)])
+        if base is not None and not st.serves_terminal():
+            return None
+        ladj = torch.empty(x2.shape[0], dtype=x.dtype, device=x.device) if total is None else total.view(-1)
+        if base is not None:
+            st.run(inp, None, ladj, total is not None, base=base)
+            return ladj.reshape(batch)
         y = torch.empty((x2.shape[0], D), dtype=x.dtype, device=x.device)
-        ladj = torch.empty(x2.shape[0], dtype=x.dtype, device=x.device) if total is None else total.view(-1)
-        st.refresh([m for m in lazy.hyper if isinstance(m, MaskedLinear)])
         st.run(inp, y, ladj, total is not None)
         return y.reshape(batch + (D,)), ladj.reshape(batch)
 
diff --git a/zuko_amd/fused.py b/zuko_amd/fused.py
--- a/zuko_amd/fused.py
+++ b/zuko_amd/fused.py
@@ -525,9 +525,20 @@
                        bias_floats=self.bias_floats, featmap=_ptr(self.featmap), n_layers=p.n_layers, n_groups=p.n_groups, n_chunks=self.half_n_chunks, act=self.act,
                        bound=self.bound, slope=self.slope, wdescale0=d[0], wdescale1=d[1], wdescale2=d[2], wdescale3=d[3], **io)
 
-    def _half_serves(self, y: Tensor) -> bool:
+    def _half_serves(self, y: Tensor | None) -> bool:
         return (self.half is not None and self.half_ok and self._half_stamp is not None and self._half_stamp == self._seen_stamp and matmul_precision() == "f16x2"
-                and self.gs_mode != "force" and (not self.half.meta["XLDS"] or (y.stride(0) % 4 == 0 and y.data_ptr() % 16 == 0)))
+                and self.gs_mode != "force" and (y is None or not self.half.meta["XLDS"] or (y.stride(0) % 4 == 0 and y.data_ptr() % 16 == 0)))
+
+    def serves_terminal(self) -> bool:
+        p = self.plan
+        if p.n_groups * 4 * p.layout.fpl + 3 * p.features > 1024:
+            return False
+        if self._half_serves(None):
+            return True
+        gs = self._gsplit()
+        if gs is not None and self._gs_stamp is not None and self._gs_stamp == self._seen_stamp:
+            return False
+        return self.static is not None and bool(self.static[0].meta.get("split")) and p.layout.kind not in (5, 6)
 
     def ready(self, rows: int) -> bool:
         from . import static_ar
@@ -596,12 +607,25 @@
         if want_gs:
             self._gs_stamp = stamp
 
-    def run(self, inp: Tensor, y: Tensor, ladj: Tensor | None, accumulate: bool) -> None:
+    def run(self, inp: Tensor, y: Tensor | None, ladj: Tensor | None, accumulate: bool, base=None) -> None:
         from . import _C
         from .ops import _ptr, _stream
 
         p = self.plan
         N = inp.shape[0]
+        if base is not None:
+            if y is not None or ladj is None or not self.serves_terminal():
+                raise RuntimeError("zuko_amd: terminal launch requested of a conditioner without an operand-split static-shape kernel (FusedAR.serves_terminal() was not consulted)")
+            io = dict(N=N, DIN=inp.shape[1], x=_ptr(inp), ldx=inp.stride(0), ladj=_ptr(ladj), accumulate=int(accumulate), base_loc=_ptr(base[0]), base_scale=_ptr(base[1]))
+            if self._half_serves(None):
+                a = self._half_args(**io)
+            else:
+                kern, rev = self.static
+                a = _C.args("zk_ar_args_v1", launcher=kern.launcher, rev=rev, uni_kind=p.layout.kind, D=p.features, wstream=_ptr(self.fine_stream), bias=_ptr(self.bias),
+                            bias_floats=self.bias_floats, featmap=_ptr(self.featmap), n_layers=p.n_layers, n_groups=p.n_groups, n_chunks=self.fine_n_chunks, act=self.act,
+                            bound=self.bound, slope=self.slope, **io)
+            _C.check(_C.lib().zk_ar_forward_static(a, _stream()), "zk_ar_forward_static")
+            return
         if self._half_serves(y):
             a = self._half_args(N=N, DIN=inp.shape[1], x=_ptr(inp), ldx=inp.stride(0), y=_ptr(y), ldy=y.stride(0), ladj=_ptr(ladj), accumulate=int(accumulate))
             _C.check(_C.lib().zk_ar_forward_static(a, _stream()), "zk_ar_forward_static")
diff --git a/zuko_amd/static_ar.py b/zuko_amd/static_ar.py
--- a/zuko_amd/static_ar.py
+++ b/zuko_amd/static_ar.py
@@ -17,7 +17,7 @@
 HERE = os.path.dirname(os.path.abspath(__file__))
 CSRC = os.path.join(HERE, "csrc")
 ARS_DIR = os.path.join(HERE, "lib", "ars")
-ARS_ABI = 9
+ARS_ABI = 10
 UNI_TYPES = {0: "zk::UniAffine", 1: "zk::UniRqs8", 2: "zk::UniRqs4", 3: "zk::UniRqs16", 4: "zk::UniCircRqs8", 5: "zk::UniSos3x5", 6: "zk::UniBern17"}
 SPLIT_ONLY_KINDS = {3, 5, 6}
 _HEADERS = ("fused_ar_static_impl.h", "fused_ar_split_impl.h", "zk_ar_common.h", "zk_univariate.h", "zk_univariate_bwd.h", "zk_common.h", "zk_half.h")
diff --git a/zuko_amd/transforms.py b/zuko_amd/transforms.py
--- a/zuko_amd/transforms.py
+++ b/zuko_amd/transforms.py
@@ -330,11 +330,17 @@
     def log_abs_det_jacobian(self, x, y):
         return self.call_and_ladj(x)[1]
 
-    def call_and_ladj(self, x):
+    def call_and_ladj(self, x, base=None):
         dim = self.domain_dim
         total = None
         owned = False
+        last = self.transforms[-1]
         for t in self.transforms:
+            if base is not None and t is last and (owned or total is None) and dim == t.domain.event_dim == t.codomain.event_dim == 1:
+                term = getattr(t, "call_and_log_prob", None)
+                lp = term(x, total, *base) if term is not None else None
+                if lp is not None:
+                    return None, lp
             acc = getattr(t, "call_and_accumulate_ladj", None)
             y = acc(x, total) if (acc is not None and owned and dim == t.domain.event_dim) else None
             if y is not None:
```
